# Zaggy1024/RaytracerCore

Hardware: AMD Instinct MI355X
Metric: Mrays/sec (primary+secondary) and samples/sec at 1080p, Cornell box (higher is better)
Workload: dtype f32; 1 GPU; bounce.txt camera 0 1920x1080 x 256 spp per GPU per step; traversal=brute, recursion=10, kernel_build=scene-specialised (hiprtc)

## Files before the change

include/rtcore.h:

```cpp
#ifndef RTCORE_H
#define RTCORE_H

#ifndef __HIPCC_RTC__
#include <stdint.h>
#include <stddef.h>
#endif

#ifdef __cplusplus
extern "C" {
#endif

#define RTCORE_ABI_VERSION 6

typedef enum rt_status {
    RT_OK = 0,
    RT_ERR_ARG = -1,
    RT_ERR_HIP = -2,
    RT_ERR_OOM = -3,
    RT_ERR_NCCL = -4,
    RT_ERR_PARSE = -5,
    RT_ERR_NODEVICE = -6,
    RT_ERR_STATE = -7
} rt_status;

typedef struct rt_vec4d { double x, y, z, w; } rt_vec4d;

typedef struct rt_color { double r, g, b; } rt_color;

typedef enum rt_prim_kind {
    RT_PRIM_TRIANGLE = 0,
    RT_PRIM_SPHERE = 1,
    RT_PRIM_PLANE = 2
} rt_prim_kind;

typedef enum rt_prim_flags {
    RT_FLAG_MIRROR = 1,
    RT_FLAG_TWOSIDED = 2,
    RT_FLAG_INVERT = 4,
    RT_FLAG_HASNORMALS = 8,
    RT_FLAG_TRANSFORMED = 16
} rt_prim_flags;

typedef struct rt_prim {
    int32_t kind;
    int32_t flags;
    rt_vec4d p[3];
    rt_vec4d n[3];
    double radius;
    double to_obj[16];
    double to_world[16];
    double to_normal[16];
    rt_color emission, diffuse, specular, refraction;
    double shininess;
    double refractive_index;
} rt_prim;

typedef enum rt_camera_kind {
    RT_CAMERA_FRUSTUM = 0,
    RT_CAMERA_ORTHO = 1
} rt_camera_kind;

typedef struct rt_camera {
    int32_t kind;
    int32_t reserved;
    rt_vec4d position, look_at, up;
    double fov_y;
    double size_mult;
    double image_plane, dof_amount, focal_length;
} rt_camera;

typedef struct rt_scene_params {
    int32_t width, height;
    int32_t recursion;
    int32_t debug_geom;
    double air_ior;
    rt_color ambient;
} rt_scene_params;

typedef struct rt_scene rt_scene;

typedef enum rt_traversal {
    RT_TRAVERSAL_AUTO = 0,
    RT_TRAVERSAL_BRUTE = 1,
    RT_TRAVERSAL_BVH = 2,
    RT_TRAVERSAL_BVH2 = 3,
    RT_TRAVERSAL_GROUPED = 4
} rt_traversal;

typedef struct rt_scene_info {
    int32_t n_prims;
    int32_t ref_bvh_nodes;
    int32_t ref_bvh_depth;
    int32_t sah_bvh_nodes;
    int32_t sah_bvh_depth;
    int32_t traversal;
    int32_t device;
    int32_t bvh_builder;
    uint64_t device_bytes;
} rt_scene_info;

typedef enum rt_bvh_builder {
    RT_BVH_BUILDER_AUTO = 0,
    RT_BVH_BUILDER_HOST = 1,
    RT_BVH_BUILDER_GPU = 2
} rt_bvh_builder;

#define RT_BUILD_STATS_COUNT 22

int rt_abi_version(void);
const char* rt_build_info(void);
int rt_device_count(void);
int rt_last_error(char* buf, int32_t cap);

int rt_scene_create(const rt_scene_params* params, const rt_prim* prims, int32_t n_prims,
                    int32_t device, rt_scene** out_scene);
int rt_scene_set_camera(rt_scene* scene, const rt_camera* camera);
int rt_scene_set_traversal(rt_scene* scene, int32_t traversal);
int rt_scene_get_info(const rt_scene* scene, rt_scene_info* info);
void rt_scene_destroy(rt_scene* scene);
int rt_set_bvh_builder(int32_t builder);
int rt_scene_get_build_stats(const rt_scene* scene, double* out, int32_t n);
int rt_set_jit(int32_t on);
int rt_scene_get_jit_error(const rt_scene* scene, char* buf, int32_t cap);
int rt_debug_jit_compile(const char* arch, int32_t grouped, char* log, int32_t cap);
int rt_debug_jit_header(const rt_scene_params* params, const rt_prim* prims, int32_t n_prims, const rt_camera* camera,
                        int32_t grouped, char* buf, int64_t cap);
int rt_scene_check_bvh(rt_scene* scene);
#define RT_LAYOUT_COUNT 10
int rt_debug_brute_layout(const rt_prim* prims, int32_t n_prims, int32_t* out, int32_t n_out);
int rt_debug_item_order(int32_t w, int32_t h, int32_t spp, int32_t chunks, int32_t pool, int32_t band,
                        int32_t band_stride, int32_t band_offset, uint32_t* out, int64_t cap_words, int32_t* info);
int rt_debug_pixels_plan(int32_t kernel, int64_t n, int32_t spp, int32_t* info);
int rt_debug_scene_bound(const rt_prim* prims, int32_t n_prims, float* lo, float* hi, float* info);
int rt_debug_block_cull(const rt_prim* prims, int32_t n_prims, const rt_camera* camera, int32_t width, int32_t height,
                        int32_t x0, int32_t y0, int32_t w, int32_t h, int32_t band, int32_t band_stride,
                        int32_t band_offset, uint8_t* dead, int64_t cap, int32_t* info);
int rt_debug_start_rows(int32_t kernel, const rt_camera* camera, int32_t w, int32_t h, int32_t spp, int32_t chunks,
                        int32_t grid_blocks, int32_t flags, int64_t* info);
int rt_debug_ray_log(rt_scene* scene, void* d_log, uint32_t cap, void* d_count);
int rt_debug_vn_rehit(const double* v0, const double* e01, const double* e02, int32_t mirror, double u, double v,
                      const float* dir, int32_t* inside, double* t, double* origin);
int rt_debug_trace_rays(rt_scene* scene, const void* d_rays, uint32_t n, void* d_hits, int32_t waves_per_simd,
                        void* d_stats, void* stream, float* ms);

int rt_render_tile(rt_scene* scene, int32_t x0, int32_t y0, int32_t w, int32_t h, int32_t spp,
                   uint64_t seed, uint64_t sample_base, rt_color* sum_rgb, uint32_t* samples,
                   uint32_t* misses, uint64_t* rays_out);

int rt_render_tile_1spp(rt_scene* scene, int32_t x0, int32_t y0, int32_t w, int32_t h,
                        uint64_t seed, uint64_t sample_index, rt_color* out);

int rt_primary_ids(rt_scene* scene, int32_t x0, int32_t y0, int32_t w, int32_t h, int32_t* ids_out);

int rt_bvh_counts(rt_scene* scene, int32_t x0, int32_t y0, int32_t w, int32_t h, int32_t* counts_out);

typedef enum rt_bounce_type {
    RT_BOUNCE_SKIPPED = 0,
    RT_BOUNCE_DIFFUSE = 1,
    RT_BOUNCE_SPECULAR = 2,
    RT_BOUNCE_SPECULAR_FAIL = 3,
    RT_BOUNCE_TRANSMITTED = 4,
    RT_BOUNCE_EMISSION = 5,
    RT_BOUNCE_PURE_BLACK = 6,
    RT_BOUNCE_RECURSION_COMPLETE = 7,
    RT_BOUNCE_MISSED = 8,
    RT_BOUNCE_DEBUG = 9
} rt_bounce_type;

typedef struct rt_debug_ray {
    int32_t prim_id;
    int32_t type;
    int32_t inside;
    float distance;
    float fresnel;
    float cos_in;
    int32_t bounce;
    int32_t reserved0;
    float position[3];
    float normal[3];
    float origin[3];
    float direction[3];
    float tint[3];
    int32_t reserved1;
} rt_debug_ray;

#define RT_TRACE_MAX_RECORDS (1 << 20)

int rt_trace_paths(rt_scene* scene, int32_t x0, int32_t y0, int32_t w, int32_t h, int32_t spp,
                   uint64_t seed, uint64_t sample_base, rt_debug_ray* rays_out, int32_t* n_rays_out,
                   rt_color* colors_out);

typedef struct rt_ray { rt_vec4d origin, direction; } rt_ray;

typedef struct rt_hit { int32_t prim_id, inside; double distance; float position[3], normal[3]; int32_t reserved[2]; } rt_hit;

typedef enum rt_query_mode {
    RT_QUERY_FAST = 0,
    RT_QUERY_EXACT = 1
} rt_query_mode;

int rt_query_rays(rt_scene* scene, int32_t mode, const rt_ray* rays, int64_t n, rt_hit* hits_out);
int rt_query_rays_device(rt_scene* scene, int32_t mode, const rt_ray* d_rays, int64_t n, rt_hit* d_hits, void* stream);
int rt_camera_rays(const rt_camera* camera, int32_t width, int32_t height, int32_t x0, int32_t y0, int32_t w,
                   int32_t h, rt_ray* out);

int rt_occluded_rays(rt_scene* scene, int32_t mode, const rt_ray* rays, const double* t_max, int64_t n,
                     uint8_t* occluded_out);
int rt_occluded_rays_device(rt_scene* scene, int32_t mode, const rt_ray* d_rays, const double* d_t_max, int64_t n,
                            uint8_t* d_occluded, void* stream);

typedef enum rt_select_kind { RT_SELECT_PRIM = 0, RT_SELECT_NODE = 1 } rt_select_kind;
typedef struct rt_select_item { int32_t kind, index; } rt_select_item;
typedef struct rt_selection { int32_t item, reserved; double distance; } rt_selection;
#define RT_SELECT_MAX_TESTS (1ull << 32)

int rt_select_pixels(rt_scene* scene, const rt_select_item* items, int32_t n_items, int32_t x0, int32_t y0, int32_t w,
                     int32_t h, rt_selection* out);
int rt_select_pixels_device(rt_scene* scene, const rt_select_item* items, int32_t n_items, int32_t x0, int32_t y0,
                            int32_t w, int32_t h, rt_selection* d_out, void* stream);
int rt_select_rays(rt_scene* scene, const rt_select_item* items, int32_t n_items, const rt_ray* rays, int64_t n,
                   rt_selection* out);
int rt_select_rays_device(rt_scene* scene, const rt_select_item* items, int32_t n_items, const rt_ray* d_rays, int64_t n,
                          rt_selection* d_out, void* stream);
int rt_debug_select_rays(const rt_prim* prims, int32_t n_prims, const rt_select_item* items, int32_t n_items,
                         const rt_ray* rays, int64_t n, rt_selection* out);

int rt_render_device(rt_scene* scene, int32_t x0, int32_t y0, int32_t w, int32_t h, int32_t spp,
                     uint64_t seed, uint64_t sample_base, double* d_sum, uint32_t* d_samples,
                     uint32_t* d_misses, unsigned long long* d_rays, void* stream);

int rt_render_rays(rt_scene* scene, const rt_ray* rays, int64_t n, int32_t spp, uint64_t seed, uint64_t sample_base,
                   uint64_t stream_base, rt_color* sum_rgb, uint32_t* samples, uint32_t* misses, uint64_t* rays_out);
int rt_render_rays_device(rt_scene* scene, const rt_ray* d_rays, int64_t n, int32_t spp, uint64_t seed,
                          uint64_t sample_base, uint64_t stream_base, double* d_sum, uint32_t* d_samples,
                          uint32_t* d_misses, unsigned long long* d_rays_count, void* stream);

typedef struct rt_beam {
    rt_vec4d origin, direction;
    rt_vec4d origin_du, origin_dv;
    rt_vec4d direction_du, direction_dv;
} rt_beam;
int rt_render_beams(rt_scene* scene, const rt_beam* beams, int64_t n, int32_t spp, uint64_t seed, uint64_t sample_base,
                    uint64_t stream_base, rt_color* sum_rgb, uint32_t* samples, uint32_t* misses, uint64_t* rays_out);
int rt_render_beams_device(rt_scene* scene, const rt_beam* d_beams, int64_t n, int32_t spp, uint64_t seed,
                           uint64_t sample_base, uint64_t stream_base, double* d_sum, uint32_t* d_samples,
                           uint32_t* d_misses, unsigned long long* d_rays_count, void* stream);
int rt_debug_beam_rays(const rt_beam* beams, int64_t n, int32_t spp, uint64_t seed, uint64_t sample_base,
                       uint64_t stream_base, rt_ray* rays_out, double* uv_out);
int rt_camera_beams(const rt_camera* camera, int32_t width, int32_t height, int32_t x0, int32_t y0, int32_t w,
                    int32_t h, rt_beam* out);

int rt_render_pixels(rt_scene* scene, const uint32_t* pixels, int64_t n, int32_t spp, uint64_t seed, uint64_t sample_base,
                     rt_color* sum_rgb, uint32_t* samples, uint32_t* misses, double* q, uint32_t* batches,
                     uint64_t* rays_out);
int rt_render_pixels_device(rt_scene* scene, const uint32_t* d_pixels, int64_t n, int32_t spp, uint64_t seed,
                            uint64_t sample_base, double* d_sum, uint32_t* d_samples, uint32_t* d_misses, double* d_q,
                            uint32_t* d_batches, uint64_t plane, unsigned long long* d_rays, void* stream);

typedef struct rt_adaptive_params {
    double   rel_tol;
    double   lum_floor;
    uint32_t min_samples;
    uint32_t max_samples;
    uint32_t reserved[2];
} rt_adaptive_params;
int rt_adaptive_select_device(const rt_adaptive_params* params, const double* d_sum, const uint32_t* d_samples,
                              const uint32_t* d_misses, const double* d_q, const uint32_t* d_batches, uint64_t plane,
                              int32_t width, int32_t height, uint32_t* d_pixels, uint32_t cap, uint32_t* d_count,
                              void* stream);
int64_t rt_debug_adaptive_select(const rt_adaptive_params* params, const double* sum, const uint32_t* samples,
                                 const uint32_t* misses, const double* q, const uint32_t* batches, uint64_t plane,
                                 int32_t width, int32_t height, uint32_t* pixels, uint32_t cap);

int rt_primary_hits_device(rt_scene* scene, int32_t x0, int32_t y0, int32_t w, int32_t h, rt_hit* d_hits, void* stream);

#define RT_DENOISE_SAME_PRIM 1u
typedef struct rt_denoise_params {
    float    sigma_l;
    float    sigma_z;
    float    lum_eps;
    int32_t  normal_pow_log2;
    int32_t  iterations;
    uint32_t flags;
    uint32_t reserved[2];
} rt_denoise_params;
int rt_denoise_device(const rt_denoise_params* params, const double* d_sum, const uint32_t* d_samples,
                      const uint32_t* d_misses, const double* d_q, const uint32_t* d_batches, uint64_t plane,
                      const rt_hit* d_hits, int32_t width, int32_t height, double* d_out_sum, float* d_out_var,
                      void* stream);
// ... 87 lines not shown
```

raytracercore_amd/__init__.py:

```python
from __future__ import annotations

import ctypes as C
import enum
import os
from dataclasses import dataclass
from typing import List, Optional, Sequence, Tuple

import numpy as np

_HERE = os.path.dirname(os.path.abspath(__file__))
LIB_PATH = os.path.join(_HERE, "librtcore_hip.so")
REPO_ROOT = os.path.dirname(_HERE)

RT_OK = 0
ABI_VERSION = 6
RT_PRIM_TRIANGLE, RT_PRIM_SPHERE, RT_PRIM_PLANE = 0, 1, 2
RT_FLAG_MIRROR, RT_FLAG_TWOSIDED, RT_FLAG_INVERT, RT_FLAG_HASNORMALS, RT_FLAG_TRANSFORMED = 1, 2, 4, 8, 16
RT_CAMERA_FRUSTUM, RT_CAMERA_ORTHO = 0, 1
RT_TRAVERSAL_AUTO, RT_TRAVERSAL_BRUTE, RT_TRAVERSAL_BVH, RT_TRAVERSAL_BVH2, RT_TRAVERSAL_GROUPED = 0, 1, 2, 3, 4
RT_BVH_BUILDER_AUTO, RT_BVH_BUILDER_HOST, RT_BVH_BUILDER_GPU = 0, 1, 2
(RT_BOUNCE_SKIPPED, RT_BOUNCE_DIFFUSE, RT_BOUNCE_SPECULAR, RT_BOUNCE_SPECULAR_FAIL, RT_BOUNCE_TRANSMITTED,
 RT_BOUNCE_EMISSION, RT_BOUNCE_PURE_BLACK, RT_BOUNCE_RECURSION_COMPLETE, RT_BOUNCE_MISSED, RT_BOUNCE_DEBUG) = range(10)
BOUNCE_TYPE_NAMES = ("Skipped", "Diffuse", "Specular", "SpecularFail", "Transmitted", "Emission", "PureBlack",
                     "RecursionComplete", "Missed", "Debug")
# ... 110 lines not shown
    _fields_ = [("kind", C.c_int32), ("index", C.c_int32)]


class rt_selection(C.Structure):
    _fields_ = [("item", C.c_int32), ("reserved", C.c_int32), ("distance", C.c_double)]


class rt_adaptive_params(C.Structure):
    _fields_ = [("rel_tol", C.c_double), ("lum_floor", C.c_double), ("min_samples", C.c_uint32),
                ("max_samples", C.c_uint32), ("reserved", C.c_uint32 * 2)]


RT_DENOISE_SAME_PRIM = 1


class rt_denoise_params(C.Structure):
    _fields_ = [("sigma_l", C.c_float), ("sigma_z", C.c_float), ("lum_eps", C.c_float), ("normal_pow_log2", C.c_int32),
                ("iterations", C.c_int32), ("flags", C.c_uint32), ("reserved", C.c_uint32 * 2)]


DENOISE_DEFAULTS = dict(sigma_l=1.5, sigma_z=0.05, lum_eps=1e-4, normal_pow_log2=6, iterations=5, flags=0)


def denoise_iterations(width: int, height: int) -> int:
    return max(1, min(5, int(min(width, height)).bit_length() - 6))


def denoise_params(**kw) -> rt_denoise_params:
    v = dict(DENOISE_DEFAULTS)
    unknown = set(kw) - set(v)
    if unknown:
        raise TypeError(f"unknown denoise parameter(s): {sorted(unknown)}")
    v.update(kw)
    return rt_denoise_params(float(v["sigma_l"]), float(v["sigma_z"]), float(v["lum_eps"]), int(v["normal_pow_log2"]),
                             int(v["iterations"]), int(v["flags"]))


RT_REPROJECT_SAME_PRIM = 1


class rt_reproject_params(C.Structure):
    _fields_ = [("sigma_z", C.c_float), ("normal_cos_min", C.c_float), ("max_history", C.c_uint32), ("flags", C.c_uint32),
                ("reserved", C.c_uint32 * 4)]


REPROJECT_DEFAULTS = dict(sigma_z=0.05, normal_cos_min=0.9, max_history=32, flags=RT_REPROJECT_SAME_PRIM)


def reproject_params(**kw) -> rt_reproject_params:
    v = dict(REPROJECT_DEFAULTS)
    unknown = set(kw) - set(v)
    if unknown:
        raise TypeError(f"unknown reproject parameter(s): {sorted(unknown)}")
    v.update(kw)
    return rt_reproject_params(float(v["sigma_z"]), float(v["normal_cos_min"]), int(v["max_history"]), int(v["flags"]))


SELECT_ITEM_DTYPE = np.dtype([("kind", np.int32), ("index", np.int32)])
SELECTION_DTYPE = np.dtype([("item", np.int32), ("reserved", np.int32), ("distance", np.float64)])

RAY_DTYPE = np.dtype([("origin", np.float64, (4,)), ("direction", np.float64, (4,))])
BEAM_DTYPE = np.dtype([(f, np.float64, (4,)) for f in
                       ("origin", "direction", "origin_du", "origin_dv", "direction_du", "direction_dv")])
HIT_DTYPE = np.dtype([
    ("prim_id", np.int32), ("inside", np.int32), ("distance", np.float64),
    ("position", np.float32, (3,)), ("normal", np.float32, (3,)), ("reserved", np.int32, (2,)),
])

_OPTIONAL = ("rt_query_rays", "rt_query_rays_device", "rt_camera_rays", "rt_select_pixels", "rt_select_pixels_device",
             "rt_select_rays", "rt_select_rays_device", "rt_render_rays", "rt_render_rays_device",
             "rt_occluded_rays", "rt_occluded_rays_device", "rt_render_pixels", "rt_render_pixels_device",
             "rt_adaptive_select_device", "rt_primary_hits_device", "rt_denoise_device", "rt_reproject_device",
             "rt_render_beams", "rt_render_beams_device", "rt_camera_beams")

_lib: Optional[C.CDLL] = None


def load_library(path: str = "") -> C.CDLL:
    global _lib
    if _lib is not None:
        return _lib
    path = path or os.environ.get("RTCORE_LIB", "") or LIB_PATH
    if not os.path.exists(path):
        raise RtError(f"{path} is missing: run __graft_entry__.build() (make -C raytracercore_amd/csrc)")
    try:
        import torch
    except ImportError:
        pass
    lib = C.CDLL(path)
    P = C.POINTER
    sig = {
        "rt_abi_version": (C.c_int, []),
        "rt_build_info": (C.c_char_p, []),
        "rt_device_count": (C.c_int, []),
        "rt_last_error": (C.c_int, [C.c_char_p, C.c_int32]),
        "rt_scene_create": (C.c_int, [P(rt_scene_params), P(rt_prim), C.c_int32, C.c_int32, P(C.c_void_p)]),
        "rt_scene_set_camera": (C.c_int, [C.c_void_p, P(rt_camera)]),
        "rt_scene_set_traversal": (C.c_int, [C.c_void_p, C.c_int32]),
        "rt_scene_get_info": (C.c_int, [C.c_void_p, P(rt_scene_info)]),
        "rt_scene_destroy": (None, [C.c_void_p]),
        "rt_set_bvh_builder": (C.c_int, [C.c_int32]),
        "rt_scene_get_build_stats": (C.c_int, [C.c_void_p, P(C.c_double), C.c_int32]),
        "rt_scene_check_bvh": (C.c_int, [C.c_void_p]),
        "rt_set_jit": (C.c_int, [C.c_int32]),
        "rt_scene_get_jit_error": (C.c_int, [C.c_void_p, C.c_char_p, C.c_int32]),
        "rt_debug_jit_compile": (C.c_int, [C.c_char_p, C.c_int32, C.c_char_p, C.c_int32]),
        "rt_debug_jit_header": (C.c_int, [P(rt_scene_params), P(rt_prim), C.c_int32, P(rt_camera), C.c_int32,
                                          C.c_char_p, C.c_int64]),
        "rt_render_tile": (C.c_int, [C.c_void_p] + [C.c_int32] * 5 + [C.c_uint64, C.c_uint64,
                                     P(rt_color), P(C.c_uint32), P(C.c_uint32), P(C.c_uint64)]),
        "rt_render_tile_1spp": (C.c_int, [C.c_void_p] + [C.c_int32] * 4 + [C.c_uint64, C.c_uint64, P(rt_color)]),
        "rt_trace_paths": (C.c_int, [C.c_void_p] + [C.c_int32] * 5 + [C.c_uint64, C.c_uint64, P(rt_debug_ray),
                                     P(C.c_int32), P(rt_color)]),
        "rt_primary_ids": (C.c_int, [C.c_void_p] + [C.c_int32] * 4 + [P(C.c_int32)]),
        "rt_bvh_counts": (C.c_int, [C.c_void_p] + [C.c_int32] * 4 + [P(C.c_int32)]),
        "rt_render_device": (C.c_int, [C.c_void_p] + [C.c_int32] * 5 + [C.c_uint64, C.c_uint64] +
                             [C.c_void_p] * 4 + [C.c_void_p]),
        "rt_primary_ids_device": (C.c_int, [C.c_void_p] + [C.c_int32] * 4 + [C.c_void_p, C.c_void_p]),
        "rt_last_kernel_ms": (C.c_int, [C.c_void_p, P(C.c_float)]),
        "rt_kernel_times": (C.c_int, [C.c_void_p, C.c_int32, P(C.c_float)]),
        "rt_scene_set_stats": (C.c_int, [C.c_void_p, C.c_int32]),
        "rt_scene_get_stats": (C.c_int, [C.c_void_p, P(C.c_uint64), C.c_int32]),
        "rt_render_frame_multi": (C.c_int, [P(rt_scene_params), P(rt_prim), C.c_int32, P(rt_camera), C.c_int32,
                                            C.c_int32, C.c_uint64, C.c_uint64, P(rt_color), P(C.c_uint32),
                                            P(C.c_uint32), P(C.c_uint64)]),
        "rt_render_bands": (C.c_int, [C.c_void_p] + [C.c_int32] * 4 + [C.c_uint64, C.c_uint64, P(rt_color),
                                      P(C.c_uint32), P(C.c_uint32), P(C.c_uint64)]),
        "rt_render_bands_device": (C.c_int, [C.c_void_p] + [C.c_int32] * 4 + [C.c_uint64, C.c_uint64] +
                                   [C.c_void_p] * 3 + [C.c_uint64, C.c_void_p, C.c_void_p]),
        "rt_band_rows": (C.c_int, [C.c_int32] * 4),
        "rt_band_slot_rows": (C.c_int, [C.c_int32] * 3),
        "rt_scatter_band_slot": (C.c_int, [C.c_void_p, C.c_uint64] + [C.c_int32] * 5 + [P(rt_color), P(C.c_uint32),
                                                                                       P(C.c_uint32)]),
        "rt_frame_create": (C.c_int, [P(rt_scene_params), P(rt_prim), C.c_int32, P(rt_camera), C.c_int32,
                                      P(C.c_void_p)]),
        "rt_frame_set_camera": (C.c_int, [C.c_void_p, P(rt_camera)]),
        "rt_frame_render": (C.c_int, [C.c_void_p, C.c_int32, C.c_uint64, C.c_uint64, P(rt_color), P(C.c_uint32),
                                      P(C.c_uint32), P(C.c_uint64)]),
        "rt_frame_submit": (C.c_int, [C.c_void_p, C.c_int32, C.c_uint64, C.c_uint64]),
        "rt_frame_collect": (C.c_int, [C.c_void_p, P(rt_color), P(C.c_uint32), P(C.c_uint32), P(C.c_uint64)]),
        "rt_frame_inject_fault": (C.c_int, [C.c_void_p, C.c_int32]),
        "rt_frame_destroy": (None, [C.c_void_p]),
        "rt_parse_scene": (C.c_int, [C.c_char_p, P(rt_scene_params), P(rt_prim), P(C.c_int32), P(rt_camera),
                                     P(C.c_int32)]),
        "rt_sample_output": (C.c_int32, [rt_color, C.c_uint32, C.c_uint32, rt_color, C.c_double, C.c_double]),
        "rt_tonemap_device": (C.c_int, [C.c_void_p, C.c_void_p, C.c_void_p, C.c_int32, C.c_int32, rt_color, C.c_double,
                                        C.c_double, C.c_void_p, C.c_void_p]),
        "rt_ref_bvh_export": (C.c_int, [P(rt_prim), C.c_int32, P(C.c_int32), P(C.c_double), P(C.c_int32),
                                        P(C.c_int32)]),
        "rt_debug_item_order": (C.c_int, [C.c_int32] * 8 + [P(C.c_uint32), C.c_int64, P(C.c_int32)]),
        "rt_debug_scene_bound": (C.c_int, [P(rt_prim), C.c_int32, P(C.c_float), P(C.c_float), P(C.c_float)]),
        "rt_debug_block_cull": (C.c_int, [P(rt_prim), C.c_int32, P(rt_camera)] + [C.c_int32] * 9 +
                                [P(C.c_uint8), C.c_int64, P(C.c_int32)]),
        "rt_debug_start_rows": (C.c_int, [C.c_int32, P(rt_camera)] + [C.c_int32] * 6 + [P(C.c_int64)]),
        "rt_debug_ray_log": (C.c_int, [C.c_void_p, C.c_void_p, C.c_uint32, C.c_void_p]),
        "rt_debug_vn_rehit": (C.c_int, [P(C.c_double), P(C.c_double), P(C.c_double), C.c_int32, C.c_double,
                                        C.c_double, P(C.c_float), P(C.c_int32), P(C.c_double), P(C.c_double)]),
        "rt_debug_trace_rays": (C.c_int, [C.c_void_p, C.c_void_p, C.c_uint32, C.c_void_p, C.c_int32, C.c_void_p,
                                          C.c_void_p, P(C.c_float)]),
        "rt_query_rays": (C.c_int, [C.c_void_p, C.c_int32, C.c_void_p, C.c_int64, C.c_void_p]),
        "rt_query_rays_device": (C.c_int, [C.c_void_p, C.c_int32, C.c_void_p, C.c_int64, C.c_void_p, C.c_void_p]),
        "rt_camera_rays": (C.c_int, [P(rt_camera)] + [C.c_int32] * 6 + [C.c_void_p]),
        "rt_select_pixels": (C.c_int, [C.c_void_p, C.c_void_p] + [C.c_int32] * 5 + [C.c_void_p]),
        "rt_select_pixels_device": (C.c_int, [C.c_void_p, C.c_void_p] + [C.c_int32] * 5 + [C.c_void_p, C.c_void_p]),
        "rt_select_rays": (C.c_int, [C.c_void_p, C.c_void_p, C.c_int32, C.c_void_p, C.c_int64, C.c_void_p]),
        "rt_select_rays_device": (C.c_int, [C.c_void_p, C.c_void_p, C.c_int32, C.c_void_p, C.c_int64, C.c_void_p,
                                            C.c_void_p]),
        "rt_debug_select_rays": (C.c_int, [P(rt_prim), C.c_int32, C.c_void_p, C.c_int32, C.c_void_p, C.c_int64,
                                           C.c_void_p]),
        "rt_render_rays": (C.c_int, [C.c_void_p, C.c_void_p, C.c_int64, C.c_int32, C.c_uint64, C.c_uint64, C.c_uint64,
                                     P(rt_color), P(C.c_uint32), P(C.c_uint32), P(C.c_uint64)]),
        "rt_render_rays_device": (C.c_int, [C.c_void_p, C.c_void_p, C.c_int64, C.c_int32, C.c_uint64, C.c_uint64,
                                            C.c_uint64] + [C.c_void_p] * 4 + [C.c_void_p]),
        "rt_render_beams": (C.c_int, [C.c_void_p, C.c_void_p, C.c_int64, C.c_int32, C.c_uint64, C.c_uint64, C.c_uint64,
                                      P(rt_color), P(C.c_uint32), P(C.c_uint32), P(C.c_uint64)]),
        "rt_render_beams_device": (C.c_int, [C.c_void_p, C.c_void_p, C.c_int64, C.c_int32, C.c_uint64, C.c_uint64,
                                             C.c_uint64] + [C.c_void_p] * 4 + [C.c_void_p]),
        "rt_debug_beam_rays": (C.c_int, [C.c_void_p, C.c_int64, C.c_int32, C.c_uint64, C.c_uint64, C.c_uint64,
                                         C.c_void_p, C.c_void_p]),
        "rt_camera_beams": (C.c_int, [P(rt_camera)] + [C.c_int32] * 6 + [C.c_void_p]),
        "rt_occluded_rays": (C.c_int, [C.c_void_p, C.c_int32, C.c_void_p, C.c_void_p, C.c_int64, C.c_void_p]),
        "rt_occluded_rays_device": (C.c_int, [C.c_void_p, C.c_int32, C.c_void_p, C.c_void_p, C.c_int64, C.c_void_p,
                                              C.c_void_p]),
        "rt_render_pixels": (C.c_int, [C.c_void_p, C.c_void_p, C.c_int64, C.c_int32, C.c_uint64, C.c_uint64,
                                       P(rt_color), P(C.c_uint32), P(C.c_uint32), P(C.c_double), P(C.c_uint32),
                                       P(C.c_uint64)]),
        "rt_render_pixels_device": (C.c_int, [C.c_void_p, C.c_void_p, C.c_int64, C.c_int32, C.c_uint64, C.c_uint64] +
                                    [C.c_void_p] * 5 + [C.c_uint64, C.c_void_p, C.c_void_p]),
        "rt_adaptive_select_device": (C.c_int, [P(rt_adaptive_params)] + [C.c_void_p] * 5 + [C.c_uint64, C.c_int32,
                                                C.c_int32, C.c_void_p, C.c_uint32, C.c_void_p, C.c_void_p]),
        "rt_debug_adaptive_select": (C.c_int64, [P(rt_adaptive_params)] + [C.c_void_p] * 5 + [C.c_uint64, C.c_int32,
                                                 C.c_int32, C.c_void_p, C.c_uint32]),
        "rt_debug_pixels_plan": (C.c_int, [C.c_int32, C.c_int64, C.c_int32, P(C.c_int32)]),
        "rt_primary_hits_device": (C.c_int, [C.c_void_p] + [C.c_int32] * 4 + [C.c_void_p, C.c_void_p]),
        "rt_denoise_device": (C.c_int, [P(rt_denoise_params)] + [C.c_void_p] * 5 + [C.c_uint64, C.c_void_p, C.c_int32,
                                        C.c_int32, C.c_void_p, C.c_void_p, C.c_void_p]),
        "rt_debug_denoise": (C.c_int, [P(rt_denoise_params)] + [C.c_void_p] * 5 + [C.c_uint64, C.c_void_p, C.c_int32,
                                       C.c_int32, C.c_void_p, C.c_void_p]),
        "rt_reproject_device": (C.c_int, [P(rt_reproject_params), P(rt_camera)] + [C.c_void_p] * 7 +
                                [C.c_uint64, C.c_int32, C.c_int32] + [C.c_void_p] * 7),
        "rt_debug_reproject": (C.c_int, [P(rt_reproject_params), P(rt_camera)] + [C.c_void_p] * 7 +
                               [C.c_uint64, C.c_int32, C.c_int32] + [C.c_void_p] * 6),
    }
    for name, (res, args) in sig.items():
        if (name.startswith("rt_debug_") or name in _OPTIONAL) and not hasattr(lib, name):
            continue
        fn = getattr(lib, name)
        fn.restype = res
        fn.argtypes = args
    if lib.rt_abi_version() != ABI_VERSION:
        raise RtError(f"{path}: ABI version {lib.rt_abi_version()}, this module binds {ABI_VERSION} (rebuild)")
    _lib = lib
    return lib


def _check(rc: int) -> None:
    if rc != RT_OK:
        buf = C.create_string_buffer(1024)
        _lib.rt_last_error(buf, 1024)
        raise RtError(f"rtcore error {rc}: {buf.value.decode(errors='replace')}")


@dataclass
class ParsedScene:
    params: rt_scene_params
    prims: "C.Array[rt_prim]"
    cameras: "C.Array[rt_camera]"

    @property
    def n_prims(self) -> int:
        return len(self.prims)


class SceneLoader:

    @staticmethod
    def from_text(text: str) -> ParsedScene:
        lib = load_library()
        n_p, n_c = C.c_int32(0), C.c_int32(0)
        params = rt_scene_params()
        _check(lib.rt_parse_scene(text.encode(), C.byref(params), None, C.byref(n_p), None, C.byref(n_c)))
        prims = (rt_prim * max(1, n_p.value))()
        cams = (rt_camera * max(1, n_c.value))()
        _check(lib.rt_parse_scene(text.encode(), C.byref(params), prims, C.byref(n_p), cams, C.byref(n_c)))
        return ParsedScene(params, (rt_prim * n_p.value).from_buffer(prims), (rt_camera * n_c.value).from_buffer(cams))

    @staticmethod
    def from_file(path: str) -> ParsedScene:
        with open(path, "r", encoding="utf-8") as f:
            return SceneLoader.from_text(f.read())


LAYOUT_NAMES = ("rects", "boxes", "frames", "frame_boxes", "frame_rects", "tris", "spheres", "planes",
                "groups", "grouped_slots")


def jit_header(scene: "SceneLoader", camera: int = 0, size: Optional[Tuple[int, int]] = None,
               grouped: bool = False) -> str:
    lib = load_library()
    params = rt_scene_params.from_buffer_copy(scene.params)
    if size:
        params.width, params.height = size
    n = len(scene.prims)
    arr = (rt_prim * max(1, n))(*scene.prims)
    cam = rt_camera.from_buffer_copy(scene.cameras[camera])
    k = lib.rt_debug_jit_header(C.byref(params), arr, n, C.byref(cam), 1 if grouped else 0, None, 0)
    if k < 0:
        _check(k)
    buf = C.create_string_buffer(k + 1)
    k2 = lib.rt_debug_jit_header(C.byref(params), arr, n, C.byref(cam), 1 if grouped else 0, buf, k + 1)
    if k2 < 0:
        _check(k2)
    return buf.value.decode()


def brute_layout(prims: Sequence[rt_prim]) -> dict:
    lib = load_library()
    n = len(prims)
    arr = (rt_prim * max(1, n))(*prims)
    out = (C.c_int32 * len(LAYOUT_NAMES))()
    _check(lib.rt_debug_brute_layout(arr, n, out, len(LAYOUT_NAMES)))
    return dict(zip(LAYOUT_NAMES, (int(v) for v in out)))


def item_order(w: int, h: int, spp: int, chunks: int = 0, pool: int = 0,
               bands: Optional[Tuple[int, int, int]] = None) -> Tuple[np.ndarray, dict]:
    lib = load_library()
    b = bands or (0, 0, 0)
    info = (C.c_int32 * 4)()
    n = lib.rt_debug_item_order(w, h, spp, chunks, pool, b[0], b[1], b[2], None, 0, info)
    if n < 0:
        _check(n)
    out = np.zeros((max(1, n), 3), np.uint32)
    n2 = lib.rt_debug_item_order(w, h, spp, chunks, pool, b[0], b[1], b[2],
                                 out.ctypes.data_as(C.POINTER(C.c_uint32)), 3 * n, info)
    if n2 < 0:
        _check(n2)
    return out[:n], dict(zip(("n_chunks", "chunk", "pool", "n_split"), (int(v) for v in info)))


def scene_bound(prims: Sequence[rt_prim]) -> dict:
    lib = load_library()
    n = len(prims)
    arr = (rt_prim * max(1, n))(*prims)
    lo, hi, info = (C.c_float * 3)(), (C.c_float * 3)(), (C.c_float * 2)()
    state = lib.rt_debug_scene_bound(arr, n, lo, hi, info)
    if state < 0:
        _check(state)
    return {"lo": np.array(lo, np.float32), "hi": np.array(hi, np.float32), "limit": np.float32(info[0]),
            "pad": np.float32(info[1]), "state": int(state)}


def block_cull(prims: Sequence[rt_prim], camera: rt_camera, size: Tuple[int, int],
               window: Optional[Tuple[int, int, int, int]] = None,
               bands: Optional[Tuple[int, int, int]] = None) -> Tuple[np.ndarray, int]:
    lib = load_library()
    n = len(prims)
    arr = (rt_prim * max(1, n))(*prims)
    cam = rt_camera.from_buffer_copy(camera)
    b = bands or (0, 0, 0)
    W, H = size
    rows = lib.rt_band_rows(H, b[0], b[1], b[2]) if bands else H
    x0, y0, w, h = window or (0, 0, W, rows)
    bx, by = (w + 7) // 8, (h + 7) // 8
    dead = np.zeros(max(1, bx * by), np.uint8)
    info = (C.c_int32 * 2)()
    live = lib.rt_debug_block_cull(arr, n, C.byref(cam), W, H, x0, y0, w, h, b[0], b[1], b[2],
                                   dead.ctypes.data_as(C.POINTER(C.c_uint8)), bx * by, info)
    if live < 0:
        _check(live)
    return dead[:bx * by].reshape(by, bx).astype(bool), int(live)


def start_rows(kernel: int, camera: rt_camera, w: int, h: int, spp: int, chunks: int = 0, grid_blocks: int = 1792,
               instrumented: bool = False, vertex_normals: bool = False) -> dict:
    lib = load_library()
    cam = rt_camera.from_buffer_copy(camera)
    info = (C.c_int64 * 3)()
    on = lib.rt_debug_start_rows(kernel, C.byref(cam), w, h, spp, chunks, grid_blocks,
                                 int(bool(instrumented)) | int(bool(vertex_normals)) << 1, info)
    if on < 0:
        _check(on)
    return {"on": bool(on), "rows": int(info[0]), "bytes": int(info[1]), "chunk": int(info[2])}


def ref_bvh_export(prims: Sequence[rt_prim]) -> Tuple[np.ndarray, np.ndarray, int, int]:
    lib = load_library()
    n = len(prims)
    arr = (rt_prim * max(1, n))(*prims)
    order = np.zeros(max(1, n), np.int32)
    boxes = np.zeros((max(1, 2 * n), 8), np.float64)
    nodes, depth = C.c_int32(0), C.c_int32(0)
    _check(lib.rt_ref_bvh_export(arr, n, order.ctypes.data_as(C.POINTER(C.c_int32)),
                                 boxes.ctypes.data_as(C.POINTER(C.c_double)), C.byref(nodes), C.byref(depth)))
    return order[:n], boxes[:nodes.value], nodes.value, depth.value


def sample_output(sum_rgb: Tuple[float, float, float], samples: int, misses: int,
                  background=(0.0, 0.0, 0.0), background_alpha: float = 0.0, exposure: float = 1.0) -> int:
    lib = load_library()
    return lib.rt_sample_output(rt_color(*sum_rgb), samples, misses, rt_color(*background), background_alpha, exposure)


def device_count() -> int:
    return load_library().rt_device_count()


def camera_rays(camera: rt_camera, size: Tuple[int, int], x0: int = 0, y0: int = 0, w: Optional[int] = None,
                h: Optional[int] = None) -> np.ndarray:
    lib = load_library()
    if not hasattr(lib, "rt_camera_rays"):
        raise RtError("this build of the library has no rt_camera_rays")
    W, H = int(size[0]), int(size[1])
    w = W - x0 if w is None else w
    h = H - y0 if h is None else h
    out = np.zeros((max(w, 0), max(h, 0)), RAY_DTYPE)
    cam = rt_camera.from_buffer_copy(camera)
    _check(lib.rt_camera_rays(C.byref(cam), W, H, x0, y0, w, h, out.ctypes.data_as(C.c_void_p)))
    return out


def _pack_rays(origins, directions) -> np.ndarray:
    o = np.asarray(origins, np.float64)
    d = np.asarray(directions, np.float64)
    if o.ndim != 2 or d.ndim != 2 or o.shape[0] != d.shape[0] or o.shape[1] not in (3, 4) or d.shape[1] not in (3, 4):
        raise ValueError("origins and directions must be (n, 3) or (n, 4) arrays of the same n")
    rays = np.zeros(o.shape[0], RAY_DTYPE)
    rays["origin"][:, 3] = 1.0
    rays["origin"][:, :o.shape[1]] = o
    rays["direction"][:, :d.shape[1]] = d
    return rays


def _pack_beams(origins, directions, origin_du, origin_dv, direction_du, direction_dv) -> np.ndarray:
    rest = (directions, origin_du, origin_dv, direction_du, direction_dv)
    if all(a is None for a in rest):
        return np.ascontiguousarray(origins, BEAM_DTYPE).reshape(-1)
    if any(a is None for a in rest):
        raise ValueError("beams: six arrays, or one BEAM_DTYPE array and None for the other five")
    parts = [np.asarray(a, np.float64) for a in (origins,) + rest]
    n = parts[0].shape[0] if parts[0].ndim == 2 else -1
    if any(a.ndim != 2 or a.shape[0] != n or a.shape[1] not in (3, 4) for a in parts):
        raise ValueError("origins, directions and the four footprint arrays must be (n, 3) or (n, 4) arrays of the same n")
    beams = np.zeros(n, BEAM_DTYPE)
    beams["origin"][:, 3] = 1.0
    for name, a in zip(BEAM_DTYPE.names, parts):
        beams[name][:, :a.shape[1]] = a
    return beams


def beam_rays_host(origins, directions, origin_du, origin_dv, direction_du, direction_dv, spp: int, seed: int,
                   sample_base: int = 0, stream_base: int = 0) -> Tuple[np.ndarray, np.ndarray]:
    lib = load_library()
    if not hasattr(lib, "rt_debug_beam_rays"):
        raise RtError("this build of the library has no rt_debug_beam_rays")
    beams = _pack_beams(origins, directions, origin_du, origin_dv, direction_du, direction_dv)
    n = beams.shape[0]
    rays = np.zeros((n, max(spp, 0)), RAY_DTYPE)
    uv = np.zeros((n, max(spp, 0), 2), np.float64)
    _check(lib.rt_debug_beam_rays(beams.ctypes.data_as(C.c_void_p), n, spp, seed, sample_base, stream_base,
                                  rays.ctypes.data_as(C.c_void_p), uv.ctypes.data_as(C.c_void_p)))
    return rays, uv


def camera_beams(camera: rt_camera, size: Tuple[int, int], x0: int = 0, y0: int = 0, w: Optional[int] = None,
                 h: Optional[int] = None) -> np.ndarray:
    lib = load_library()
    if not hasattr(lib, "rt_camera_beams"):
        raise RtError("this build of the library has no rt_camera_beams")
    W, H = int(size[0]), int(size[1])
    w = W - x0 if w is None else w
    h = H - y0 if h is None else h
    out = np.zeros((max(w, 0), max(h, 0)), BEAM_DTYPE)
    cam = rt_camera.from_buffer_copy(camera)
    _check(lib.rt_camera_beams(C.byref(cam), W, H, x0, y0, w, h, out.ctypes.data_as(C.c_void_p)))
    return out


def _pack_items(items) -> np.ndarray:
    if isinstance(items, np.ndarray) and items.dtype == SELECT_ITEM_DTYPE:
        return np.ascontiguousarray(items.reshape(-1))
    a = np.asarray(items, np.int64)
    if a.size == 0:
        return np.zeros(0, SELECT_ITEM_DTYPE)
    if a.ndim != 2 or a.shape[1] != 2:
        raise ValueError("items must be an (n, 2) int array or a sequence of (kind, index) pairs")
    if a.min() < -2 ** 31 or a.max() >= 2 ** 31:
        raise ValueError("items: kind and index must fit in int32")
    out = np.zeros(a.shape[0], SELECT_ITEM_DTYPE)
    out["kind"], out["index"] = a[:, 0], a[:, 1]
    return out


def _rays_arg(origins, directions) -> np.ndarray:
    return np.ascontiguousarray(origins, RAY_DTYPE) if directions is None else _pack_rays(origins, directions)


def segment_rays(points_a, points_b) -> Tuple[np.ndarray, np.ndarray]:
    a = np.asarray(points_a, np.float64)
    b = np.asarray(points_b, np.float64)
    if a.shape != b.shape or a.ndim < 1 or a.shape[-1] != 3:
        raise ValueError("points_a and points_b must be (..., 3) arrays of the same shape")
    v = b - a
    scale = np.max(np.abs(v), axis=-1)
    safe = np.where(scale > 0, scale, 1.0)
    u = v / safe[..., None]
    norm = np.sqrt(np.sum(u * u, axis=-1))
    t_max = np.where(scale > 0, norm * safe, 0.0)
    d = u / np.where(scale > 0, norm, 1.0)[..., None]
    d = d / np.where(scale > 0, np.sqrt(np.sum(d * d, axis=-1)), 1.0)[..., None]
    rays = np.zeros(a.shape[:-1], RAY_DTYPE)
    rays["origin"][..., :3] = a
    rays["origin"][..., 3] = 1.0
    rays["direction"][..., :3] = d
    return rays, t_max


def select_rays_host(prims: Sequence[rt_prim], items, origins, directions=None) -> np.ndarray:
    lib = load_library()
    if not hasattr(lib, "rt_debug_select_rays"):
        raise RtError("this build of the library has no rt_debug_select_rays")
    n = len(prims)
    arr = prims if isinstance(prims, C.Array) and n > 0 else (rt_prim * max(1, n))(*prims)
    it = _pack_items(items)
    rays = _rays_arg(origins, directions)
    out = np.zeros(rays.shape, SELECTION_DTYPE)
# ... 680 lines not shown
```

raytracercore_amd/csrc/api_debug.hip:

```cpp
#include <cstdlib>
#include <cstring>

#include "rt_scene.h"

namespace {

int n_bvh_prims(const std::vector<HostPrim>& H)
{
    int nb = 0;
    for (const HostPrim& p : H) nb += p.kind != RT_PRIM_PLANE;
    return nb;
}

HostRecords report_records(const std::vector<HostPrim>& H)
{
    const bool host_tree = builder_for(n_bvh_prims(H)) == RT_BVH_BUILDER_HOST;
    return make_host_records(H, host_tree ? grouping_max_leaf(GroupingTree::LayoutReport, (int)H.size(), false) : 0,
                             group_max_default());
}

}

extern "C" {

// ... 333 lines not shown
        if (ref >= (int)n4.size()) {
            err = "wide child index out of range";
            return u;
        }
        const Node4Q& q = n4[ref];
        uint32_t ex, ql[3], qh[3];
        int refs[4], nc;
        std::memcpy(&ex, &q.a.w, 4);
        std::memcpy(&ql[0], &q.b.x, 4);
        std::memcpy(&qh[0], &q.b.y, 4);
        std::memcpy(&ql[1], &q.b.z, 4);
        std::memcpy(&qh[1], &q.b.w, 4);
        std::memcpy(&ql[2], &q.c.x, 4);
        std::memcpy(&qh[2], &q.c.y, 4);
        std::memcpy(&refs[0], &q.c.z, 4);
        std::memcpy(&refs[1], &q.c.w, 4);
        std::memcpy(&refs[2], &q.d.x, 4);
        std::memcpy(&refs[3], &q.d.y, 4);
        std::memcpy(&nc, &q.d.z, 4);
        if (nc < 1 || nc > 4) {
            err = "wide node with a bad child count";
            return u;
        }
        max_stack = std::max(max_stack, pushes + nc - 1);
        const double org[3] = {q.a.x, q.a.y, q.a.z};
        for (int k = 0; k < nc; k++) {
            const B sub = walk4(refs[k], pushes + nc - 1);
            B box;
            for (int a = 0; a < 3; a++) {
                const double sc = std::ldexp(1.0, (int)((ex >> (8 * a)) & 255u) - 128);
                box.lo[a] = org[a] + ((ql[a] >> (8 * k)) & 255u) * sc;
                box.hi[a] = org[a] + ((qh[a] >> (8 * k)) & 255u) * sc;
            }
            if (err.empty() && !contains(box, sub)) err = "wide child box misses a primitive below it";
            grow(u, sub);
        }
        return u;
    };
    if (err.empty() && nb > 0) walk4(s->bvh.root4, 0);
    for (int i = 0; i < n && err.empty(); i++)
        if (seen[i] != (outside(i) ? 0 : 1))
            err = "wide tree: primitive " + std::to_string(i) + " referenced " + std::to_string(seen[i]) + " times";
    if (err.empty() && max_stack > s->bvh.stack4) err = "wide tree needs more stack than recorded";
    if (!err.empty()) {
        set_error("rt_scene_check_bvh: " + err);
        return RT_ERR_STATE;
    }
    return RT_OK;
}

int rt_debug_item_order(int32_t w, int32_t h, int32_t spp, int32_t chunks, int32_t pool, int32_t band,
                        int32_t band_stride, int32_t band_offset, uint32_t* out, int64_t cap_words, int32_t* info)
{
    const bool banded = band > 0;
    if (w <= 0 || h <= 0 || spp <= 0 || chunks < 0 || pool < 0 || pool % 64 != 0 || cap_words < 0 ||
        (cap_words > 0 && !out) || (banded && (band_stride <= 0 || band_offset < 0 || band_offset >= band_stride))) {
        set_error("rt_debug_item_order: bad argument");
        return RT_ERR_ARG;
    }
    const int rows = banded ? band_set_rows(h, band, band_stride, band_offset) : h;
    if (rows <= 0) return 0;
    PathParams p = make_params_for(pool > 64 ? 1 : 0, chunks, pool, 0, 0, w, rows, spp, 0, 0, 0.0);
    if (banded) set_band(p, band, band_stride, band_offset);
    if ((uint64_t)p.n_chunks * (uint64_t)p.n_pad > 0xF0000000ull) {
        set_error("rt_debug_item_order: tile x spp too large for one launch");
        return RT_ERR_ARG;
    }
    if (info) {
        info[0] = p.n_chunks;
        info[1] = p.chunk;
        info[2] = p.pool;
        info[3] = p.n_split;
    }
    const int64_t n = list_tickets(p, out, cap_words);
    if (n > INT32_MAX) {
        set_error("rt_debug_item_order: too many tickets");
        return RT_ERR_ARG;
    }
    return (int)n;
}

int rt_debug_pixels_plan(int32_t kernel, int64_t n, int32_t spp, int32_t* info)
{
    if (kernel < 0 || kernel > 3 || kernel == 2 || n <= 0 || n > ((int64_t)1 << 30) || spp <= 0 || !info) {
        set_error("rt_debug_pixels_plan: bad argument");
        return RT_ERR_ARG;
    }
    const PathParams p = make_params_pixels(kernel, n, spp, 0, 0, 1920, 1080);
    info[0] = p.n_chunks;
    info[1] = p.chunk;
    info[2] = (p.spp + p.chunk - 1) / p.chunk;
    info[3] = p.n_pad / 64;
    return RT_OK;
}

int rt_debug_scene_bound(const rt_prim* prims, int32_t n_prims, float* lo, float* hi, float* info)
{
    if (n_prims < 0 || (n_prims > 0 && !prims) || !lo || !hi) {
        set_error("rt_debug_scene_bound: bad argument");
        return RT_ERR_ARG;
    }
    for (int i = 0; i < n_prims; i++)
        if (prims[i].kind < 0 || prims[i].kind > 2) {
            set_error("rt_debug_scene_bound: unknown primitive kind at index " + std::to_string(i));
            return RT_ERR_ARG;
        }
    const SceneBound b = make_scene_bound(prepare_prims(prims, n_prims));
    for (int k = 0; k < 3; k++) {
        lo[k] = b.lo[k];
        hi[k] = b.hi[k];
    }
    if (info) {
        info[0] = b.limit;
        info[1] = b.pad;
    }
    return b.empty ? 1 : (b.limit < 0.0f ? 2 : 0);
}

int rt_debug_block_cull(const rt_prim* prims, int32_t n_prims, const rt_camera* camera, int32_t width, int32_t height,
                        int32_t x0, int32_t y0, int32_t w, int32_t h, int32_t band, int32_t band_stride,
                        int32_t band_offset, uint8_t* dead, int64_t cap, int32_t* info)
{
    const bool banded = band > 0;
    if (n_prims < 0 || (n_prims > 0 && !prims) || !camera || width <= 0 || height <= 0 || w <= 0 || h <= 0 || x0 < 0 ||
        y0 < 0 || x0 + w > width || cap < 0 || (cap > 0 && !dead) || band < 0 ||
        (camera->kind != RT_CAMERA_FRUSTUM && camera->kind != RT_CAMERA_ORTHO) ||
        (banded && (band_stride <= 0 || band_offset < 0 || band_offset >= band_stride)) || (!banded && y0 + h > height)) {
        set_error("rt_debug_block_cull: bad argument");
        return RT_ERR_ARG;
    }
    int n_planes = 0;
    for (int i = 0; i < n_prims; i++) {
        if (prims[i].kind < 0 || prims[i].kind > 2) {
            set_error("rt_debug_block_cull: unknown primitive kind at index " + std::to_string(i));
            return RT_ERR_ARG;
        }
        n_planes += prims[i].kind == RT_PRIM_PLANE ? 1 : 0;
    }
    const SceneBound b = make_scene_bound(prepare_prims(prims, n_prims));
    CameraD camd;
    CameraF camf;
    camera_init(*camera, width, height, camd, camf);
    const CullWindow win{x0, y0, w, h, banded ? band : 0, banded ? band_stride : 0, banded ? band_offset : 0};
    std::vector<unsigned char> flags;
    const int live = cull_blocks(camf, b, n_planes, win, flags);
    for (size_t i = 0; i < flags.size() && (int64_t)i < cap; i++) dead[i] = flags[i];
    if (info) {
        info[0] = (w + 7) / 8;
        info[1] = (h + 7) / 8;
    }
    return live;
}

int rt_debug_start_rows(int32_t kernel, const rt_camera* camera, int32_t w, int32_t h, int32_t spp, int32_t chunks,
                        int32_t grid_blocks, int32_t flags, int64_t* info)
{
    if (kernel < 0 || kernel > 3 || !camera || w <= 0 || h <= 0 || spp <= 0 || chunks < 0 || grid_blocks <= 0 || !info ||
        (camera->kind != RT_CAMERA_FRUSTUM && camera->kind != RT_CAMERA_ORTHO)) {
        set_error("rt_debug_start_rows: bad argument");
        return RT_ERR_ARG;
    }
    CameraD camd;
    CameraF camf;
    camera_init(*camera, w, h, camd, camf);
    const PathParams p = make_params_for(kernel, chunks, 0, 0, 0, w, h, spp, 0, 0, 0.0);
    const StartRowsPlan sr = plan_start_rows(kernel, (flags & 1) != 0, (flags & 2) != 0, camf.kind, camf.dof != 0.0f, p.chunk, grid_blocks);
    info[0] = sr.rows;
    info[1] = (int64_t)sr.bytes;
    info[2] = p.chunk;
    return sr.on ? 1 : 0;
}

int rt_parse_scene(const char* text, rt_scene_params* params, rt_prim* prims, int32_t* n_prims, rt_camera* cameras,
                   int32_t* n_cameras)
{
    if (!text || !n_prims || !n_cameras) {
        set_error("rt_parse_scene: bad argument");
        return RT_ERR_ARG;
    }
    ParsedScene ps;
    std::string err;
    if (!parse_scene_text(text, ps, err)) {
        set_error(err);
        return RT_ERR_PARSE;
    }
    const int cap_p = *n_prims, cap_c = *n_cameras;
    *n_prims = (int32_t)ps.prims.size();
    *n_cameras = (int32_t)ps.cameras.size();
    if (params) *params = ps.params;
    if (prims) {
        if (cap_p < (int)ps.prims.size()) {
            set_error("rt_parse_scene: primitive array too small");
            return RT_ERR_ARG;
        }
        std::copy(ps.prims.begin(), ps.prims.end(), prims);
    }
    if (cameras) {
        if (cap_c < (int)ps.cameras.size()) {
            set_error("rt_parse_scene: camera array too small");
            return RT_ERR_ARG;
        }
        std::copy(ps.cameras.begin(), ps.cameras.end(), cameras);
    }
    return RT_OK;
}

int rt_ref_bvh_export(const rt_prim* prims, int32_t n, int32_t* leaf_order, double* boxes, int32_t* n_nodes,
                      int32_t* depth)
{
    if (n < 0 || (n > 0 && !prims)) {
        set_error("rt_ref_bvh_export: bad argument");
        return RT_ERR_ARG;
    }
    std::vector<HostPrim> host = prepare_prims(prims, n);
    RefBvh ref = build_ref_bvh(host);
    int k = 0;
    for (size_t i = 0; i < ref.nodes.size(); i++) {
        const RefNode& r = ref.nodes[i];
        if (r.prim >= 0 && leaf_order) leaf_order[k++] = r.prim;
        if (boxes) {
            double* b = boxes + 8 * i;
            b[0] = r.mn.x; b[1] = r.mn.y; b[2] = r.mn.z; b[3] = r.mn.w;
            b[4] = r.mx.x; b[5] = r.mx.y; b[6] = r.mx.z; b[7] = r.mx.w;
        }
    }
    if (n_nodes) *n_nodes = (int32_t)ref.nodes.size();
    if (depth) *depth = ref.depth;
    return RT_OK;
}

}
```

raytracercore_amd/csrc/block_cull.cpp:

```cpp
#include "block_cull.h"

#include <algorithm>
#include <cmath>

namespace rtc {

namespace {

constexpr double kMargin = 0.25;
constexpr double kAhead = 1e-3;

struct P2 {
    double x, y;
};

struct Hull {
    std::vector<P2> v;
    double xmin, xmax, ymin, ymax;
};

double cross2(P2 o, P2 a, P2 b) { return (a.x - o.x) * (b.y - o.y) - (a.y - o.y) * (b.x - o.x); }

void convex_hull(std::vector<P2> pts, Hull& h)
{
    std::sort(pts.begin(), pts.end(), [](P2 a, P2 b) { return a.x < b.x || (a.x == b.x && a.y < b.y); });
    std::vector<P2> v(2 * pts.size());
    size_t k = 0;
    for (size_t i = 0; i < pts.size(); i++) {
        while (k >= 2 && cross2(v[k - 2], v[k - 1], pts[i]) <= 0.0) k--;
        v[k++] = pts[i];
    }
    for (size_t i = pts.size() - 1, t = k + 1; i > 0; i--) {
        while (k >= t && cross2(v[k - 2], v[k - 1], pts[i - 1]) <= 0.0) k--;
        v[k++] = pts[i - 1];
    }
    v.resize(k > 1 ? k - 1 : k);
    h.v = v;
    h.xmin = h.ymin = INFINITY;
    h.xmax = h.ymax = -INFINITY;
    for (P2 p : pts) {
        h.xmin = std::min(h.xmin, p.x);
        h.xmax = std::max(h.xmax, p.x);
        h.ymin = std::min(h.ymin, p.y);
        h.ymax = std::max(h.ymax, p.y);
    }
}

bool separated(const Hull& h, double xa, double xb, double ya, double yb)
{
    if (xb < h.xmin || xa > h.xmax || yb < h.ymin || ya > h.ymax) return true;
    const size_t n = h.v.size();
    if (n < 3) return false;
    for (size_t i = 0; i < n; i++) {
        const P2 p = h.v[i], q = h.v[i + 1 == n ? 0 : i + 1];
        const double nx = q.y - p.y, ny = -(q.x - p.x);
        const double cx = nx > 0.0 ? xa : xb, cy = ny > 0.0 ? ya : yb;
        if (nx * (cx - p.x) + ny * (cy - p.y) > 0.0) return true;
    }
    return false;
}

struct V3d {
    double x, y, z;
};
V3d crs(V3d a, V3d b) { return {a.y * b.z - a.z * b.y, a.z * b.x - a.x * b.z, a.x * b.y - a.y * b.x}; }
double dot(V3d a, V3d b) { return a.x * b.x + a.y * b.y + a.z * b.z; }
V3d v3d(const float4& f) { return {(double)f.x, (double)f.y, (double)f.z}; }

bool project_bound(const CameraF& c, const SceneBound& b, int frame_w, Hull& hull)
{
    const bool frustum = c.kind == RT_CAMERA_FRUSTUM;
    const double vals[] = {c.position.x, c.position.y, c.position.z, c.look.x, c.look.y, c.look.z, c.side.x,
                           c.side.y, c.side.z, c.up.x, c.up.y, c.up.z, c.w2, c.h2, c.tan_x, c.tan_y,
                           c.h_mult, c.v_mult, c.image_plane, c.dof, c.focal_length, c.tan_x_per_px, c.tan_y_per_px};
    for (double v : vals)
        if (!std::isfinite(v)) return false;
    if (c.dof != 0.0f) return false;
    const V3d pos = v3d(c.position), look = v3d(c.look), side = v3d(c.side), up = v3d(c.up);
    const double apos = std::fabs(pos.x) + std::fabs(pos.y) + std::fabs(pos.z);
    const V3d da = crs(up, look), db = crs(look, side), dc = crs(side, up);
    const double det = dot(side, da);
    if (!(std::fabs(det) > 0.5 && std::fabs(det) < 2.0)) return false;
    const double sxa = frustum ? c.tan_x_per_px : c.h_mult, sya = frustum ? c.tan_y_per_px : c.v_mult;
    if (sxa == 0.0 || sya == 0.0) return false;
    const double scale = std::min(std::fabs(sxa), std::fabs(sya));
    if (frustum) {
        if (!(apos <= (double)b.limit)) return false;
    } else {
        const double reach = std::fabs((double)c.w2 * c.h_mult) * (std::fabs(side.x) + std::fabs(side.y) + std::fabs(side.z)) +
                             std::fabs((double)c.h2 * c.v_mult) * (std::fabs(up.x) + std::fabs(up.y) + std::fabs(up.z));
        if (!(apos + 2.0 * reach + std::fabs((double)c.image_plane) <= (double)b.limit)) return false;
    }
    std::vector<P2> pts;
    double c_min = INFINITY, c_max = 0.0;
    for (int k = 0; k < 8; k++) {
        const V3d P = {(k & 1) ? (double)b.hi[0] + b.pad : (double)b.lo[0] - b.pad,
                       (k & 2) ? (double)b.hi[1] + b.pad : (double)b.lo[1] - b.pad,
                       (k & 4) ? (double)b.hi[2] + b.pad : (double)b.lo[2] - b.pad};
        const V3d v = {P.x - pos.x, P.y - pos.y, P.z - pos.z};
        const double a = dot(v, da) / det, bb = dot(v, db) / det, cc = dot(v, dc) / det;
        if (!(cc > kAhead * std::sqrt(dot(v, v))) || !(cc > 0.0)) return false;
        c_min = std::min(c_min, cc);
        c_max = std::max(c_max, cc);
        if (frustum) pts.push_back({(a / cc + (double)c.tan_x) / sxa, (bb / cc + (double)c.tan_y) / sya});
        else pts.push_back({a / sxa + (double)c.w2, bb / sya + (double)c.h2});
    }
    double err;
    if (frustum) {
        const double L = 1.0 + std::fabs((double)c.tan_x) + std::fabs((double)c.tan_y);
        err = std::ldexp(L * L, -20) / scale +
              std::ldexp(apos + std::fabs((double)c.image_plane), -22) / (c_min * scale);
    } else {
        const double R = apos + std::fabs((double)c.w2 * c.h_mult) + std::fabs((double)c.h2 * c.v_mult) +
                         std::fabs((double)c.image_plane);
        err = std::ldexp(R + c_max, -22) / scale + std::ldexp((double)std::max(frame_w, 1), -22);
    }
    if (!(err <= kMargin / 8.0)) return false;
    for (P2 p : pts)
        if (!(std::isfinite(p.x) && std::isfinite(p.y))) return false;
    convex_hull(pts, hull);
    return true;
}

}

int cull_blocks(const CameraF& cam, const SceneBound& bound, int n_planes, const CullWindow& win,
                std::vector<unsigned char>& dead)
{
    const int bxn = (win.w + 7) / 8, byn = (win.h + 7) / 8;
    const int n = bxn * byn;
    dead.assign((size_t)n, 0);
    if (n_planes > 0) return n;
    if (bound.empty) {
        dead.assign((size_t)n, 1);
        return 0;
    }
    if (!(bound.limit >= 0.0f)) return n;
    Hull hull;
    if (!project_bound(cam, bound, (int)(2.0f * cam.w2), hull)) return n;
    int live = 0;
    for (int by = 0; by < byn; by++) {
        int run_a[8], run_b[8], runs = 0;
        for (int py = by * 8; py < std::min(win.h, by * 8 + 8); py++) {
            int fy = win.y0 + py;
            if (win.band > 0) fy = win.y0 + ((py / win.band) * win.band_stride + win.band_offset) * win.band + py % win.band;
            if (runs > 0 && fy == run_b[runs - 1] + 1) run_b[runs - 1] = fy;
            else {
                run_a[runs] = run_b[runs] = fy;
                runs++;
            }
        }
        for (int bx = 0; bx < bxn; bx++) {
            const double xa = (double)(win.x0 + bx * 8) - kMargin;
            const double xb = (double)(win.x0 + std::min(win.w, bx * 8 + 8)) + kMargin;
            bool is_dead = true;
            for (int r = 0; r < runs && is_dead; r++)
                is_dead = separated(hull, xa, xb, (double)run_a[r] - kMargin, (double)(run_b[r] + 1) + kMargin);
            dead[(size_t)by * bxn + bx] = is_dead ? 1 : 0;
            live += is_dead ? 0 : 1;
        }
    }
    return live;
}

uint64_t dead_pixels(const CullWindow& win, const std::vector<unsigned char>& dead)
{
    const int bxn = (win.w + 7) / 8, byn = (win.h + 7) / 8;
    uint64_t n = 0;
    for (int by = 0; by < byn; by++)
        for (int bx = 0; bx < bxn; bx++)
            if (dead[(size_t)by * bxn + bx])
                n += (uint64_t)(std::min(win.w, bx * 8 + 8) - bx * 8) * (uint64_t)(std::min(win.h, by * 8 + 8) - by * 8);
    return n;
}

}
```

raytracercore_amd/csrc/block_cull.h:

```cpp
#pragma once
#include <cstdint>
#include <vector>

#include "rt_internal.h"

namespace rtc {

struct CullWindow {
    int x0, y0, w, h;
    int band, band_stride, band_offset;
};

int cull_blocks(const CameraF& cam, const SceneBound& bound, int n_planes, const CullWindow& win,
                std::vector<unsigned char>& dead);

uint64_t dead_pixels(const CullWindow& win, const std::vector<unsigned char>& dead);

}
```

raytracercore_amd/csrc/kernels_path.hip:

```cpp
#include "../../include/rtcore_rng.h"
#include "rt_kernels.h"
#include "rt_beam.h"
#ifdef RT_SCENE_CONST
#include "rt_scene_const.h"
#endif

namespace rtc {
namespace {

struct V3 {
    float x, y, z;
};
__device__ __forceinline__ V3 v3(float x, float y, float z) { return V3{x, y, z}; }
__device__ __forceinline__ V3 xyz(float4 a) { return V3{a.x, a.y, a.z}; }
__device__ __forceinline__ V3 operator+(V3 a, V3 b) { return {a.x + b.x, a.y + b.y, a.z + b.z}; }
__device__ __forceinline__ V3 operator-(V3 a, V3 b) { return {a.x - b.x, a.y - b.y, a.z - b.z}; }
__device__ __forceinline__ V3 operator*(V3 a, float s) { return {a.x * s, a.y * s, a.z * s}; }
__device__ __forceinline__ V3 operator*(V3 a, V3 b) { return {a.x * b.x, a.y * b.y, a.z * b.z}; }
__device__ __forceinline__ V3 operator-(V3 a) { return {-a.x, -a.y, -a.z}; }
__device__ __forceinline__ float dot(V3 a, V3 b) { return fmaf(a.x, b.x, fmaf(a.y, b.y, a.z * b.z)); }
__device__ __forceinline__ bool known_zero(float c)
{
#if defined(RT_SCENE_CONST)
    return __builtin_constant_p(c) && c == 0.0f;
// ... 191 lines not shown

template <bool SUB>
__device__ __forceinline__ void hit_box(const BoxRec& B, V3 o, V3 d, V3 id, V3 oi, int prev, Best& b)
{
    const float lx = SUB ? (B.lo.x - oi.x) * id.x : fmaf(B.lo.x, id.x, -oi.x);
    const float hx = SUB ? (B.hi.x - oi.x) * id.x : fmaf(B.hi.x, id.x, -oi.x);
    const float ly = SUB ? (B.lo.y - oi.y) * id.y : fmaf(B.lo.y, id.y, -oi.y);
    const float hy = SUB ? (B.hi.y - oi.y) * id.y : fmaf(B.hi.y, id.y, -oi.y);
    const float lz = SUB ? (B.lo.z - oi.z) * id.z : fmaf(B.lo.z, id.z, -oi.z);
    const float hz = SUB ? (B.hi.z - oi.z) * id.z : fmaf(B.hi.z, id.z, -oi.z);
    const float nx = vmin(lx, hx), ny = vmin(ly, hy), nz = vmin(lz, hz);
    const float fx = vmax(lx, hx), fy = vmax(ly, hy), fz = vmax(lz, hz);
    const float te = vmax3(nx, ny, nz), tx = vmin3(fx, fy, fz);
    const bool meet = te <= tx;
    if (RT_BOX_WAVE_SKIP && !__any(meet & (tx >= 0.0f))) return;
    const int sx = (int)(__float_as_uint(d.x) >> 31), sy = (int)(__float_as_uint(d.y) >> 31),
              sz = (int)(__float_as_uint(d.z) >> 31);
    const uint32_t keep = B.keep;
    const uint32_t rel_prev = (uint32_t)(prev - (B.sg0 >> 1));
    bool ok_e = false, ok_x = false;
    int fe = 0, fo = 0;
    if (keep & 0x3Fu) {
        fe = te == nx ? sx : (te == ny ? 2 + sy : 4 + sz);
        ok_e = meet & (__float_as_uint(te) < __float_as_uint(b.t)) & ((uint32_t)fe != rel_prev) &
               (((keep >> fe) & 1u) != 0);
    }
    if (keep & 0x3F00u) {
        fo = tx == fx ? 1 - sx : (tx == fy ? 3 - sy : 5 - sz);
        ok_x = meet & (__float_as_uint(tx) < __float_as_uint(b.t)) & ((uint32_t)fo != rel_prev) &
               (((keep >> (8 + fo)) & 1u) != 0);
    }
    const bool ok = ok_e | ok_x;
    b.t = ok ? (ok_e ? te : tx) : b.t;
    b.sg = ok ? B.sg0 + 2 * (ok_e ? fe : fo) : b.sg;
}

__device__ __forceinline__ float slab_rcp(float d)
{
    return rcp(fabsf(d) >= 5.421010862e-20f ? d : __builtin_copysignf(5.421010862e-20f, d));
}
__device__ __forceinline__ float slab_rcp_lean(float d)
{
    return __builtin_amdgcn_fmed3f(rcp(d), -0x1p64f, 0x1p64f);
}

template <bool BARE = false>
__device__ __forceinline__ bool slab(float4 lo, float4 hi, V3 oi, V3 id, float tmax, float& tnear)
{
    const float tx0 = fmaf(lo.x, id.x, -oi.x), tx1 = fmaf(hi.x, id.x, -oi.x);
    const float ty0 = fmaf(lo.y, id.y, -oi.y), ty1 = fmaf(hi.y, id.y, -oi.y);
    const float tz0 = fmaf(lo.z, id.z, -oi.z), tz1 = fmaf(hi.z, id.z, -oi.z);
    const float nx = BARE ? vmin(tx0, tx1) : fminf(tx0, tx1), fx = BARE ? vmax(tx0, tx1) : fmaxf(tx0, tx1);
    const float ny = BARE ? vmin(ty0, ty1) : fminf(ty0, ty1), fy = BARE ? vmax(ty0, ty1) : fmaxf(ty0, ty1);
    const float nz = BARE ? vmin(tz0, tz1) : fminf(tz0, tz1), fz = BARE ? vmax(tz0, tz1) : fmaxf(tz0, tz1);
    const float tmin = BARE ? vmax3(nx, ny, vmax0(nz)) : fmaxf(fmaxf(nx, ny), fmaxf(nz, 0.0f));
    const float tmx = BARE ? vmin3(fx, fy, vmin(fz, tmax)) : fminf(fminf(fx, fy), fminf(fz, tmax));
    tnear = tmin;
    return tmin <= tmx * 1.00000024f;
}

template <class SceneT>
__device__ __forceinline__ bool scene_meets(const SceneT& s, V3 o, V3 d)
{
    const V3 id = v3(slab_rcp_lean(d.x), slab_rcp_lean(d.y), slab_rcp_lean(d.z));
    const V3 oi = o * id;
    const float tx0 = fmaf(s.bound_lo[0], id.x, -oi.x), tx1 = fmaf(s.bound_hi[0], id.x, -oi.x);
    const float ty0 = fmaf(s.bound_lo[1], id.y, -oi.y), ty1 = fmaf(s.bound_hi[1], id.y, -oi.y);
    const float tz0 = fmaf(s.bound_lo[2], id.z, -oi.z), tz1 = fmaf(s.bound_hi[2], id.z, -oi.z);
    const float tmin = fmaxf(fmaxf(fminf(tx0, tx1), fminf(ty0, ty1)), fmaxf(fminf(tz0, tz1), 0.0f));
    const float tmx = fminf(fminf(fmaxf(tx0, tx1), fmaxf(ty0, ty1)), fmaxf(tz0, tz1));
    const bool near = fabsf(o.x) + fabsf(o.y) + fabsf(o.z) <= s.bound_limit;
    const bool finite = fabsf(d.x + d.y + d.z) < __builtin_huge_valf();
    return (!(tmin > tmx) | !near | !finite) & (s.bound_empty == 0);
}

template <bool CULL, bool STATS, bool ANY = false, class SceneT, class GroupP, class TestP, class RectP, class FrameP,
          class BoxP, class XfP>
__device__ __forceinline__ void trace_brute(const SceneT& s, GroupP groups, TestP tests, RectP rects, FrameP frames,
                                            BoxP boxes, XfP xf, V3 o, V3 d, int prev, Best& b, unsigned& n_flat,
                                            unsigned& n_sph, unsigned& n_node)
{
    const V3 id = v3(slab_rcp_lean(d.x), slab_rcp_lean(d.y), slab_rcp_lean(d.z));
    const V3 oi = o * id;
    const int n_groups = CULL ? s.n_groups : 1;
    int skip_to = 0;
#ifdef RT_SCENE_CONST
#pragma unroll
#endif
    for (int g = 0; g < n_groups; g++) {
        if (CULL && g < skip_to) continue;
        const GroupRec G = groups[g];
        if (CULL) {
            if (STATS) n_node++;
            float tn;
            if (!__any((!ANY || b.sg < 0) && slab<true>(G.lo, G.hi, oi, id, b.t, tn))) {
                skip_to = g + 1 + G.skip;
                continue;
            }
        }
        if (STATS) {
            n_flat += G.n_rect[0] + G.n_rect[1] + G.n_rect[2] + G.n_flat_extra + (G.n_tri_sph & 0xFFFF);
            n_sph += G.n_tri_sph >> 16;
        }
        RectP r = rects + __float_as_int(G.lo.w);
        rect_group<0>(r, G.n_rect[0], o, d, id, oi, prev, b);
        r += G.n_rect[0];
        rect_group<1>(r, G.n_rect[1], o, d, id, oi, prev, b);
        r += G.n_rect[1];
        rect_group<2>(r, G.n_rect[2], o, d, id, oi, prev, b);
        for (int j = G.frame_first + G.n_frames; j < G.frame_first + G.n_frames + G.n_boxes; j++) {
            const BoxRec B = boxes[j];
            hit_box<false>(B, o, d, id, oi, prev, b);
        }
        if (ANY && !CULL && !__any(b.sg < 0)) return;
        for (int f = G.frame_first; f < G.frame_first + G.n_frames; f++) {
            const FrameRec F = frames[f];
            const V3 lo = v3(dot4(F.r0, o), dot4(F.r1, o), dot4(F.r2, o));
            const V3 ld = v3(dot3(F.r0, d), dot3(F.r1, d), dot3(F.r2, d));
            const V3 lid = v3(rcp(ld.x), rcp(ld.y), rcp(ld.z));
            RectP fr = rects + F.rect_first;
            rect_group<0, true>(fr, F.n_rect[0], lo, ld, lid, lo, prev, b);
            fr += F.n_rect[0];
            rect_group<1, true>(fr, F.n_rect[1], lo, ld, lid, lo, prev, b);
            fr += F.n_rect[1];
            rect_group<2, true>(fr, F.n_rect[2], lo, ld, lid, lo, prev, b);
            if (F.box >= 0) {
                const BoxRec B = boxes[F.box];
                hit_box<true>(B, lo, ld, lid, lo, prev, b);
            }
        }
        if (ANY && !CULL && !__any(b.sg < 0)) return;
        int i = __float_as_int(G.hi.w);
        int end = i + (G.n_tri_sph & 0xFFFF);
        if (i < end) {
            TestRec cur = tests[i];
            for (; i < end; i++) {
                const TestRec nxt = tests[i + 1];
                hit_tri<true>(cur, i, o, d, prev, b);
                cur = nxt;
            }
        }
        if (ANY && !CULL && !__any(b.sg < 0)) return;
        end = i + (G.n_tri_sph >> 16);
        if (i < end) {
            TestRec cur = tests[i];
            for (; i < end; i++) {
                const TestRec nxt = tests[i + 1];
                hit_sph<true, RT_SPH_WAVE_SKIP < 0 ? CULL : RT_SPH_WAVE_SKIP != 0>(cur, i, o, d, prev, xf, b);
                cur = nxt;
            }
        }
        if (ANY && CULL && !__any(b.sg < 0)) return;
    }
}

template <bool SLOT = false, class XfP>
__device__ __forceinline__ void hit_any(const TestRec& R, int slot, V3 o, V3 d, int prev, XfP xf, Best& b)
{
    switch (__float_as_uint(R.meta.y) & KIND_MASK) {
    case RT_PRIM_TRIANGLE: hit_tri<SLOT>(R, slot, o, d, prev, b); break;
    case RT_PRIM_SPHERE: hit_sph<SLOT>(R, slot, o, d, prev, xf, b); break;
    default: hit_plane<SLOT>(R, slot, o, d, prev, b); break;
    }
}

constexpr uint32_t kLeafGeneric = 0xFFFFFFFFu;
__device__ __forceinline__ void leaf_decode(int pend, int& k, int& kend, uint32_t& lfl)
{
    const bool compact = (pend & kLeafCompact) != 0;
    k = compact ? (pend >> 2) & (kLeafCompactMaxFirst - 1) : pend >> 3;
    kend = k + (pend & (compact ? 3 : 7)) + 1;
    lfl = compact ? leaf_flags(((uint32_t)pend >> 25) & 31u) : kLeafGeneric;
}
__device__ __forceinline__ int leaf_advance(int pend, int n)
{
    const bool compact = (pend & kLeafCompact) != 0;
    const int left = pend & (compact ? 3 : 7);
    return left >= n ? pend + (compact ? (n << 2) - n : (n << 3) - n) : -1;
}



__device__ __forceinline__ float ubyte(uint32_t v, int k) { return (float)((v >> (8 * k)) & 255u); }
__device__ __forceinline__ void cswap(float& da, int& ra, float& db, int& rb)
{
    const bool sw = db < da;
    const float t = da;
    const int r = ra;
    da = sw ? db : da;
    ra = sw ? rb : ra;
    db = sw ? t : db;
    rb = sw ? r : rb;
}
#define RT_STACK_OVF 44
typedef __attribute__((address_space(3))) int LdsInt;
typedef __attribute__((address_space(1))) int GlobalInt;
struct TravStack {
    LdsInt* lds;
    GlobalInt* ovf;
};
__device__ __forceinline__ TravStack make_stack(int* lds_base, int* ovf_base)
{
    return TravStack{(LdsInt*)lds_base, (GlobalInt*)ovf_base};
}
__device__ __forceinline__ unsigned ovf_slot(int e)
{
    return (unsigned)e * (gridDim.x * 256u) + blockIdx.x * 256u + threadIdx.x;
}
template <int STACK>
__device__ __forceinline__ void push(const TravStack& st, int& sp, int v)
{
    if (sp < STACK) st.lds[sp * 256 + (int)threadIdx.x] = v;
    else st.ovf[ovf_slot(sp - STACK)] = v;
    sp++;
}
template <int STACK>
__device__ __forceinline__ int pop_ref(const TravStack& st, int& sp)
{
    --sp;
    return sp < STACK ? st.lds[sp * 256 + (int)threadIdx.x] : st.ovf[ovf_slot(sp - STACK)];
}

__device__ __forceinline__ void pin4(float4& f)
{
    typedef float F4 __attribute__((ext_vector_type(4)));
    F4 v = {f.x, f.y, f.z, f.w};
    asm volatile("" : "+v"(v));
    f = make_float4(v.x, v.y, v.z, v.w);
}
__device__ __forceinline__ void pin_rec(TestRec& t)
{
    pin4(t.r0);
    pin4(t.r1);
    pin4(t.r2);
    pin4(t.meta);
}
template <int STACK>
__device__ __forceinline__ void wide_visit(const Node4Q& q, V3 id, V3 oi, float best, int& ref, int& sp,
                                           const TravStack& stk, bool& pop)
{
    const uint32_t ex = __float_as_uint(q.a.w);
    const float ax = __builtin_amdgcn_ldexpf(id.x, (int)(ex & 255u) - 128);
    const float ay = __builtin_amdgcn_ldexpf(id.y, (int)((ex >> 8) & 255u) - 128);
    const float az = __builtin_amdgcn_ldexpf(id.z, (int)((ex >> 16) & 255u) - 128);
    const float bx = fmaf(q.a.x, id.x, -oi.x), by = fmaf(q.a.y, id.y, -oi.y), bz = fmaf(q.a.z, id.z, -oi.z);
    const uint32_t lx = __float_as_uint(q.b.x), hx = __float_as_uint(q.b.y);
    const uint32_t ly = __float_as_uint(q.b.z), hy = __float_as_uint(q.b.w);
    const uint32_t lz = __float_as_uint(q.c.x), hz = __float_as_uint(q.c.y);
    const uint32_t nx = id.x >= 0.0f ? lx : hx, fx = id.x >= 0.0f ? hx : lx;
    const uint32_t ny = id.y >= 0.0f ? ly : hy, fy = id.y >= 0.0f ? hy : ly;
    const uint32_t nz = id.z >= 0.0f ? lz : hz, fz = id.z >= 0.0f ? hz : lz;
    const int nc = __float_as_int(q.d.z);
    float d0, d1, d2, d3;
    int r0 = __float_as_int(q.c.z), r1 = __float_as_int(q.c.w), r2 = __float_as_int(q.d.x), r3 = __float_as_int(q.d.y);
    const float tmax_best = best * 1.00000024f;
#define RT_WIDE_CHILD(K, D)                                                                                       \
    {                                                                                                             \
        const float tmin = fmaxf(fmaxf(fmaxf(fmaf(ubyte(nx, K), ax, bx), fmaf(ubyte(ny, K), ay, by)),              \
                                       fmaf(ubyte(nz, K), az, bz)), 0.0f);                                         \
        const float tmax = fminf(fminf(fmaf(ubyte(fx, K), ax, bx), fmaf(ubyte(fy, K), ay, by)),                   \
                                 fmaf(ubyte(fz, K), az, bz));                                                      \
        D = ((K < nc) & (tmin <= fminf(tmax * 1.00000024f, tmax_best))) ? tmin : __builtin_huge_valf();         \
    }
    RT_WIDE_CHILD(0, d0)
    RT_WIDE_CHILD(1, d1)
    RT_WIDE_CHILD(2, d2)
    RT_WIDE_CHILD(3, d3)
#undef RT_WIDE_CHILD
    cswap(d0, r0, d1, r1);
    cswap(d2, r2, d3, r3);
    cswap(d0, r0, d2, r2);
    cswap(d1, r1, d3, r3);
    cswap(d1, r1, d2, r2);
    const float inf = __builtin_huge_valf();
    if (d0 < inf) {
        if (d3 < inf) push<STACK>(stk, sp, r3);
        if (d2 < inf) push<STACK>(stk, sp, r2);
        if (d1 < inf) push<STACK>(stk, sp, r1);
        ref = r0;
        pop = false;
    }
}

template <int STACK>
__device__ __forceinline__ void any_visit(const Node4Q& q, V3 id, V3 oi, float best, int& ref, int& sp,
                                          const TravStack& stk, bool& pop)
{
    const uint32_t ex = __float_as_uint(q.a.w);
    const float ax = __builtin_amdgcn_ldexpf(id.x, (int)(ex & 255u) - 128);
    const float ay = __builtin_amdgcn_ldexpf(id.y, (int)((ex >> 8) & 255u) - 128);
    const float az = __builtin_amdgcn_ldexpf(id.z, (int)((ex >> 16) & 255u) - 128);
    const float bx = fmaf(q.a.x, id.x, -oi.x), by = fmaf(q.a.y, id.y, -oi.y), bz = fmaf(q.a.z, id.z, -oi.z);
    const uint32_t lx = __float_as_uint(q.b.x), hx = __float_as_uint(q.b.y);
    const uint32_t ly = __float_as_uint(q.b.z), hy = __float_as_uint(q.b.w);
    const uint32_t lz = __float_as_uint(q.c.x), hz = __float_as_uint(q.c.y);
    const bool px = id.x >= 0.0f, py = id.y >= 0.0f, pz = id.z >= 0.0f;
    const uint32_t nx = px ? lx : hx, fx = px ? hx : lx;
    const uint32_t ny = py ? ly : hy, fy = py ? hy : ly;
    const uint32_t nz = pz ? lz : hz, fz = pz ? hz : lz;
    const int nc = __float_as_int(q.d.z);
    const int r0 = __float_as_int(q.c.z), r1 = __float_as_int(q.c.w), r2 = __float_as_int(q.d.x), r3 = __float_as_int(q.d.y);
    const float tmax_best = best * 1.00000024f;
    bool h0, h1, h2, h3;
#define RT_ANY_CHILD(K, H)                                                                                        \
    {                                                                                                             \
        const float tmin = fmaxf(fmaxf(fmaxf(fmaf(ubyte(nx, K), ax, bx), fmaf(ubyte(ny, K), ay, by)),              \
// ... 761 lines not shown
            S.rng = rt_rng_from_pixel_key(L.pkey, p.sample_base + (unsigned long long)item_sample<NT>(L, p));
            const float u = (float)rt_rng_next24(&S.rng) * 0x1p-24f;
            const float v = (float)rt_rng_next24(&S.rng) * 0x1p-24f;
            BeamV o, d;
            const BeamSample r = beam_sample(p.beam_list + (size_t)kBeamRows * (size_t)bi, u, v, o, d);
            if (r == BEAM_RAY) {
                S.o = v3(o.x, o.y, o.z);
                S.d = v3(d.x, d.y, d.z);
                S.tint = v3(1.0f, 1.0f, 1.0f);
                S.bounce = 0;
                S.prev = -1;
                L.live = true;
            } else {
                const unsigned left = r == BEAM_INVALID ? L.cnt >> 16 : 1u;
                L.cnt += left * (256u - 65536u);
                if (!NT) L.s_next += (int)left;
            }
        }
        return;
    }
    if (go && L.active && L.item_open && !L.live && L.cnt >= 65536u) {
        if (start_rows_on<NT, SRC, ROWS>(p, cam)) {
            const unsigned r = (L.cnt & 0xFFu) + ((L.cnt >> 8) & 0xFFu);
            const row_g1* const rows = (const row_g1*)(unsigned long long)p.starts;
            const row_f4 v = *(const row_g4*)(rows + start_row_offset(p, r, lane));
            const V3 d = v3(v.x, v.y, v.z);
            S.rng.x = __float_as_uint(v.w);
            S.o = madd(d, cam.image_plane, xyz(cam.position));
            S.d = d;
            S.tint = v3(1.0f, 1.0f, 1.0f);
            S.bounce = 0;
            S.prev = -1;
            L.live = true;
            return;
        }
        int fx = L.fx, fy = L.fy;
        if (NT && SRC == ITEMS_PIXELS) {
            const unsigned pix = p.pixel_list[item_ray(L.item, p)];
            list_pixel(pix, p, fx, fy);
            L.pkey = rt_rng_pixel_key(p.seed_key, (unsigned long long)pix);
        } else if (NT) {
            int px, py, c;
            item_pixel(L.item, p, px, py, c, fx, fy);
            L.pkey = rt_rng_pixel_key(p.seed_key, (unsigned long long)fy * (unsigned long long)p.scene.width +
                                                      (unsigned long long)fx);
        }
        S.rng = rt_rng_from_pixel_key(L.pkey, p.sample_base + (unsigned long long)item_sample<NT>(L, p));
        start_sample<!NT>(cam, fx, fy, S);
        L.live = true;
    }
}

template <bool VN, bool PIN = false, bool SLOT = false, bool REC = false, class SceneT, class VnP, class TestP, class ParT>
__device__ __forceinline__ void bounce(Lane& L, Sample& S, const SceneT& s, const ShadeRecs& R, VnP vnormals, TestP tests,
                                       const PrimD* prims_d, const Best& b, [[maybe_unused]] const ParT& p)
{
    V3 col;
    [[maybe_unused]] BounceRec rec;
    [[maybe_unused]] const V3 ro = S.o, rd = S.d, rtint = S.tint;
    [[maybe_unused]] const int rbounce = S.bounce;
    [[maybe_unused]] unsigned rsample = 0;
    if constexpr (REC) {
        if (p.rec_rays) {
            int px, py, c, fx, fy;
            item_pixel(L.item, p, px, py, c, fx, fy);
            rsample = ((unsigned)py * (unsigned)p.w + (unsigned)px) * (unsigned)p.spp + (unsigned)item_sample<SLOT>(L, p);
        }
    }
    const int r = shade<VN, PIN, SLOT, REC>(s, R.prims, R.mats, R.xfs, vnormals, tests, prims_d, b, S, col, &rec);
    if constexpr (REC) {
        const unsigned slot = rsample * (unsigned)(s.recursion + 1) + (unsigned)rbounce;
        if (p.rec_rays && slot < p.rec_max && rbounce <= s.recursion) {
            float4* q = p.rec_rays + (size_t)kRecRows * slot;
            q[0] = make_float4(__int_as_float(rec.prim_id), __int_as_float(rec.type), __int_as_float(rec.inside), rec.distance);
            q[1] = make_float4(rec.fresnel, rec.cos_in, __int_as_float(rbounce), 0.0f);
            q[2] = make_float4(rec.pos.x, rec.pos.y, rec.pos.z, rec.nrm.x);
            q[3] = make_float4(rec.nrm.y, rec.nrm.z, ro.x, ro.y);
            q[4] = make_float4(ro.z, rd.x, rd.y, rd.z);
            q[5] = make_float4(rtint.x, rtint.y, rtint.z, 0.0f);
            if (r != 0)
                p.rec_samples[rsample] = r == 1 ? make_float4(0.0f + col.x, 0.0f + col.y, 0.0f + col.z, __int_as_float(rbounce + 1))
                                                : make_float4(-1.0f, -1.0f, -1.0f, __int_as_float(rbounce + 1));
        }
    }
    if (r != 0) {
        const bool hit = r == 1;
        L.ar += hit ? col.x : 0.0f;
        L.ag += hit ? col.y : 0.0f;
        L.ab += hit ? col.z : 0.0f;
        L.cnt += hit ? 1u - 65536u : 256u - 65536u;
        if (!SLOT) L.s_next++;
        L.live = false;
        if (!SLOT) {
            asm volatile("" : "=v"(S.o.x), "=v"(S.o.y), "=v"(S.o.z), "=v"(S.d.x), "=v"(S.d.y), "=v"(S.d.z),
                         "=v"(S.tint.x), "=v"(S.tint.y), "=v"(S.tint.z), "=v"(S.bounce), "=v"(S.prev),
                         "=v"(S.rng.x));
        }
    }
}

template <bool STATS, class ParT>
__device__ __forceinline__ void flush_counts(unsigned long long wave_rays, const Counters& cnt, const ParT& p,
                                             int lane)
{
    if (lane == 0) atomicAdd(p.rays, wave_rays);
    if (STATS) {
        unsigned long long a = cnt.nodes, t = cnt.tris, q = cnt.sphs;
        for (int off = 32; off > 0; off >>= 1) {
            a += __shfl_down(a, off);
            t += __shfl_down(t, off);
            q += __shfl_down(q, off);
        }
        if (lane == 0) {
            atomicAdd(p.stats + 0, a);
            atomicAdd(p.stats + 1, t);
            atomicAdd(p.stats + 2, q);
            atomicAdd(p.stats + 3, cnt.cyc_start);
            atomicAdd(p.stats + 4, cnt.cyc_trace);
            atomicAdd(p.stats + 5, cnt.cyc_shade);
            atomicAdd(p.stats + 6, cnt.iters);
        }
        unsigned long long mx = cnt.max_steps, ov = cnt.ovf_pushes, ms = cnt.max_sp, ot = cnt.outer;
        for (int off = 32; off > 0; off >>= 1) {
            mx = max(mx, (unsigned long long)__shfl_down(mx, off));
            ov += __shfl_down(ov, off);
            ms = max(ms, (unsigned long long)__shfl_down(ms, off));
            ot += __shfl_down(ot, off);
        }
        if (lane == 0) {
            atomicMax(p.stats + 7, mx);
            atomicAdd(p.stats + 8, ov);
            atomicMax(p.stats + 9, ms);
            atomicAdd(p.stats + 10, ot);
        }
    }
}

#ifdef __HIP_DEVICE_COMPILE__
#define RT_AS_CONST __attribute__((address_space(4)))
#else
#define RT_AS_CONST
#endif
typedef RT_AS_CONST const CameraF CameraC;
typedef RT_AS_CONST const PathParams ParamsC;

template <bool CULL, bool LDS, bool STATS, bool VN, int SRC = ITEMS_TILE>
__device__ __forceinline__ void path_body(const CameraF* __restrict__ camp, const PathParams* __restrict__ pp)
{
    const ParamsC& P0 = *(const ParamsC*)pp;
    extern __shared__ float4 lds_scene[];
    const ShadeRecs R = stage_scene<LDS>(P0.scene, P0.prims, P0.mats, P0.xf, lds_scene);
    const int lane = threadIdx.x & 63;
    const unsigned total = (unsigned)P0.n_chunks * (unsigned)P0.n_pad;
    Lane L;
    lane_init(L);
    Sample S;
    S.prev = -1;
    S.bounce = 0;
    Counters cnt{};
    unsigned long long wave_rays = 0;
    const unsigned long long bound_off = P0.scene_bound != 0 ? 0ull : ~0ull;

    while (true) {
        unsigned long long t0 = 0, t1 = 0, t2 = 0;
        if (STATS) t0 = __builtin_readcyclecounter();
        const CameraC* cp = (const CameraC*)camp;
        asm volatile("" : "+s"(cp));
        const ParamsC* pq = (const ParamsC*)pp;
        asm volatile("" : "+s"(pq));
#ifdef RT_SCENE_CONST
        const PathScene& sc = *(const PathScene*)kSceneW;
#else
        const auto& sc = pq->scene;
#endif
#if defined(RT_SCENE_CONST) && RT_SCENE_CONST_CAMERA
        refill<false, ITEMS_TILE, !STATS && !VN, !STATS && !VN>(L, S, *pq, sc, *(const CameraF*)kCameraW, lane, total,
                                                         (unsigned)wave_rays);
#else
        refill<false, SRC, !STATS && !VN, !STATS && !VN && SRC == ITEMS_TILE>(L, S, *pq, sc, *cp, lane, total,
                                                                              (unsigned)wave_rays);
#endif
        if (!__any(L.active)) break;
        if (STATS) t1 = __builtin_readcyclecounter();
        wave_rays += (unsigned)__popcll(__ballot(L.live));
        if (L.live) {
#ifdef RT_SCENE_CONST
            const auto tests = (const TestRec*)kTestsW;
            const auto rects = (const RectRec*)kRectsW;
            const auto frames = (const FrameRec*)kFramesW;
            const auto boxes = (const BoxRec*)kFramesW;
            const auto groups = (const GroupRec*)kGroupsW;
            const auto xf = (const XformF*)kXfW;
#else
            const auto tests = (const RT_AS_CONST TestRec*)pq->tests;
            const auto rects = (const RT_AS_CONST RectRec*)pq->rects;
            const auto frames = (const RT_AS_CONST FrameRec*)pq->frames;
            const auto boxes = (const RT_AS_CONST BoxRec*)pq->frames;
            const auto groups = (const RT_AS_CONST GroupRec*)pq->groups;
            const auto xf = (const RT_AS_CONST XformF*)pq->xf;
#endif
            const auto vnormals = (const RT_AS_CONST float4*)pq->vnormals;
            Best b = query_start<VN>(sc, S.prev);
            bool query = true;
            if (!STATS && (!CULL || RT_BOUND_GROUPED) &&
                __builtin_expect((__ballot(L.live && S.bounce != 0) | bound_off) == 0ull, 0))
                query = __any(L.live && scene_meets(sc, S.o, S.d));
            if (query)
                trace_brute<CULL, STATS>(sc, groups, tests, rects, frames, boxes, xf, S.o, S.d, S.prev, b, cnt.tris,
                                         cnt.sphs, cnt.nodes);
            test_planes(sc, tests, S.o, S.d, S.prev, b);
            if (VN && __builtin_isnan(S.d.x + S.d.y + S.d.z)) b = Best{__builtin_huge_valf(), -1};
            if (STATS) t2 = __builtin_readcyclecounter();
            bounce<VN, false, false, STATS>(L, S, sc, R, vnormals, tests, pq->prims_d, b, *pq);
        } else if (STATS) {
            t2 = __builtin_readcyclecounter();
        }
        if (STATS) {
            const unsigned long long t3 = __builtin_readcyclecounter();
            cnt.cyc_start += t1 - t0;
            cnt.cyc_trace += t2 - t1;
            cnt.cyc_shade += t3 - t2;
            cnt.iters++;
        }
    }
    if (!STATS && SRC == ITEMS_TILE && P0.cull != nullptr && blockIdx.x == 0 && threadIdx.x < 64)
        wave_rays += ((unsigned long long)P0.cull[0] | (unsigned long long)P0.cull[1] << 32) * (unsigned long long)P0.spp;
    flush_counts<STATS>(wave_rays, cnt, *(const ParamsC*)pp, lane);
}

template <bool CULL, bool LDS, bool STATS, bool VN, int SRC = ITEMS_TILE>
__global__ void __launch_bounds__(256, CULL ? RT_GROUPED_WAVES : RT_PATH_WAVES)
    path_kernel(PathScene, const CameraF* __restrict__ camp, const PathParams* __restrict__ pp, const TestRec*,
                const RectRec*, const FrameRec*, const PrimF*, const NodeF*, const Node4Q*, const GroupRec*,
                const XformF*, const MatF*, const float4*)
{
    path_body<CULL, LDS, STATS, VN, SRC>(camp, pp);
}

template <bool STATS, class GroupP, class RectP, class BoxP>
__device__ __forceinline__ void test_outer(GroupP groups, RectP rects, BoxP boxes, V3 o, V3 d, int prev, Best& b,
                                           unsigned& n_tests)
{
    const V3 id = v3(slab_rcp_lean(d.x), slab_rcp_lean(d.y), slab_rcp_lean(d.z));
    const V3 oi = o * id;
    const GroupRec G = groups[0];
    if (STATS) n_tests += G.n_rect[0] + G.n_rect[1] + G.n_rect[2] + G.n_flat_extra;
    RectP r = rects + __float_as_int(G.lo.w);
    rect_group<0>(r, G.n_rect[0], o, d, id, oi, prev, b);
    r += G.n_rect[0];
    rect_group<1>(r, G.n_rect[1], o, d, id, oi, prev, b);
    r += G.n_rect[1];
    rect_group<2>(r, G.n_rect[2], o, d, id, oi, prev, b);
    for (int j = G.frame_first + G.n_frames; j < G.frame_first + G.n_frames + G.n_boxes; j++) {
        const BoxRec B = boxes[j];
        hit_box<false>(B, o, d, id, oi, prev, b);
    }
}

template <bool STATS, class TestP, class RowP, class XfP>
__device__ __forceinline__ void test_leaf(TestP tests, RowP rows, XfP xf, int pend, V3 o, V3 d, int prev, Best& b,
                                          unsigned& n_tri, unsigned& n_sph)
{
    int k, kend;
    uint32_t lfl;
    leaf_decode(pend, k, kend, lfl);
    float4 r[RT_SPEC_PRIMS][3];
    uint32_t fl[RT_SPEC_PRIMS];
#pragma unroll
    for (int j = 0; j < RT_SPEC_PRIMS; j++) {
        r[j][0] = rows[3 * (k + j)];
        r[j][1] = rows[3 * (k + j) + 1];
        r[j][2] = rows[3 * (k + j) + 2];
    }
    if (lfl == kLeafGeneric) {
#pragma unroll
        for (int j = 0; j < RT_SPEC_PRIMS; j++) fl[j] = __float_as_uint(tests[k + j].meta.y);
    } else {
#pragma unroll
        for (int j = 0; j < RT_SPEC_PRIMS; j++) fl[j] = lfl;
    }
#pragma unroll
    for (int j = 0; j < RT_SPEC_PRIMS; j++) {
        pin4(r[j][0]);
        pin4(r[j][1]);
        pin4(r[j][2]);
    }
#pragma unroll
    for (int j = 0; j < RT_SPEC_PRIMS; j++) {
        if (j == 0 || k + j < kend) {
            const bool sph = (fl[j] & KIND_MASK) == RT_PRIM_SPHERE;
            if (STATS) {
                if (sph) n_sph++;
                else n_tri++;
            }
            if (sph) hit_sph_rows(r[j][0], r[j][1], fl[j], k + j, k + j, o, d, prev, xf, b);
            else hit_tri_rows(r[j][0], r[j][1], r[j][2], fl[j], k + j, k + j, o, d, prev, b);
        }
    }
}

struct Walk {
    bool more;
    int ref;
    int sp;
    int pend;
};
__device__ __forceinline__ void walk_start(Walk& w, int root, bool tree)
{
    w.ref = root;
    w.sp = 0;
    w.pend = -1;
    w.more = tree;
    if (root < 0) {
        w.pend = ~root;
        w.more = false;
    }
}
struct WalkStep {
    bool ended;
    bool leaf_step, can_node;
    int sp_visit;
};
template <int STACK, bool ANY, bool STATS = false, int WIDTH = 4, class FetchT, class TestP, class RowP, class XfP>
__device__ __forceinline__ WalkStep walk_step(Walk& w, bool trav, int spec, FetchT fetch, V3 id, V3 oi, const TravStack& stk,
                                              TestP tests, RowP rows, XfP xf, V3 o, V3 d, int prev, Best& b,
                                              unsigned& n_tri, unsigned& n_sph)
{
    WalkStep st;
    st.can_node = trav && w.more && w.ref >= 0;
    const bool blocked = trav && w.pend >= 0 && !st.can_node;
    st.leaf_step = __ballot(st.can_node) == 0 || __popcll(__ballot(blocked)) >= spec;
    st.ended = false;
    st.sp_visit = w.sp;
    if (trav) {
        if (st.leaf_step) {
            if (w.pend >= 0) {
                test_leaf<STATS>(tests, rows, xf, w.pend, o, d, prev, b, n_tri, n_sph);
                w.pend = leaf_advance(w.pend, RT_SPEC_PRIMS);
                if (ANY && b.sg >= 0) {
                    w.pend = -1;
                    w.more = false;
                }
            }
        } else if (st.can_node) {
            bool pop = true;
            const auto node = fetch(w.ref);
            if constexpr (WIDTH == 2) bvh2_visit<STACK>(node, id, oi, b.t, w.ref, w.sp, stk, pop);
            else if constexpr (ANY) any_visit<STACK>(node, id, oi, b.t, w.ref, w.sp, stk, pop);
            else wide_visit<STACK>(node, id, oi, b.t, w.ref, w.sp, stk, pop);
            st.sp_visit = w.sp;
            if (pop) {
                if (w.sp > 0) w.ref = pop_ref<STACK>(stk, w.sp);
                else w.more = false;
            }
        }
        if (w.more && w.ref < 0 && w.pend < 0) {
            w.pend = ~w.ref;
            if (w.sp > 0) w.ref = pop_ref<STACK>(stk, w.sp);
            else w.more = false;
// ... 1106 lines not shown
```

raytracercore_amd/csrc/launch_params.cpp:

```cpp
#include "launch_params.h"

#include <algorithm>
#include <cmath>
#include <cstdlib>

#include "host_scene.h"

namespace rtc {

void set_item_order(PathParams& p)
{
    const char* e = getenv("RTCORE_ITEM_ORDER");
    bool dense = !(e && e[0] == '0');
    const unsigned slots = (unsigned)p.pool / 64u;
    const unsigned used = (unsigned)((p.spp + p.chunk - 1) / p.chunk);
    const unsigned n_blocks = (unsigned)(p.n_pad / 64);
    for (;; dense = false) {
        const unsigned n_real = dense ? used : (unsigned)p.n_chunks;
        const unsigned n_full = dense && p.spp % p.chunk != 0 ? used - 1 : n_real;
        p.tpb = n_full / slots;
        p.tail_first = p.tpb * (unsigned)p.pool;
        p.tail_len = (n_real - p.tpb * slots) * 64u;
        p.magic_tpb = 0;
        if (p.tpb <= 1) break;
        const uint64_t M = ((1ull << 32) + p.tpb - 1) / p.tpb;
        const uint64_t err = M * p.tpb - (1ull << 32);
        if (M < (1ull << 32) && (uint64_t)n_blocks * p.tpb * err < (1ull << 32)) {
            p.magic_tpb = (unsigned)M;
            break;
        }
    }
    p.linear = p.tail_len == 0 && p.tpb * slots == (unsigned)p.n_chunks;
    for (int g = 0; g < kMaxSplit; g++) {
        const unsigned b = g < p.n_split ? (p.split_start[g + 1] - p.split_start[g]) >> (p.log2_chunks + 6) : 0u;
        p.split_full[g] = b * p.tpb;
        p.split_tickets[g] = p.split_full[g] + (p.tail_len ? b : 0u);
    }
}

void set_blocks(PathParams& p, int n_blocks)
{
    p.n_pad = n_blocks * 64;
    p.n_split = 1;
    int want = kMaxSplit;
    if (const char* e = getenv("RTCORE_XCD_SPLIT")) want = atoi(e) > 0 ? kMaxSplit : 1;
    if (want > 1 && n_blocks >= 4 * kMaxSplit) p.n_split = kMaxSplit;
    for (int g = 0; g <= p.n_split; g++)
        p.split_start[g] = (unsigned)((int64_t)n_blocks * g / p.n_split) * (unsigned)(p.n_chunks * 64);
    set_item_order(p);
}

PathParams make_params_for(int kernel, int chunks_over, int pool_over, int x0, int y0, int w, int h, int spp,
                           uint64_t seed, uint64_t base, double chunk_npix)
{
    PathParams p{};
    p.x0 = x0;
    p.y0 = y0;
    p.w = w;
    p.h = h;
    p.band = 0;
    p.spp = spp;
    const int base_chunks = kernel >= 2 ? 64 : 24;
    int chunks = base_chunks;
    const double npix = chunk_npix > 0.0 ? chunk_npix : (double)w * (double)h;
    if (npix > 0 && npix < 2073600.0)
        chunks = (int)std::min(8.0 * base_chunks, base_chunks * std::ceil(2073600.0 / npix));
    else if (npix > 2073600.0)
        chunks = (int)std::max(base_chunks / 4.0, std::ceil(base_chunks * 2073600.0 / npix));
    if (const char* e = getenv("RTCORE_PATH_CHUNKS")) chunks = std::max(1, atoi(e));
    if (chunks_over > 0) chunks = chunks_over;
    p.chunk = std::max(1, std::min(64, (spp + chunks - 1) / chunks));
    const int used = (spp + p.chunk - 1) / p.chunk;
    p.log2_chunks = 0;
    while ((1 << p.log2_chunks) < used) p.log2_chunks++;
    p.n_chunks = 1 << p.log2_chunks;
    p.blocks_x = (w + 7) / 8;
    p.n_pad = p.blocks_x * ((h + 7) / 8) * 64;
    p.inv_blocks_x = 1.0f / (float)p.blocks_x;
    p.magic_bx = 0;
    if (p.blocks_x > 1 && !getenv("RTCORE_NO_MAGIC_DIV")) {
        const uint64_t M = ((1ull << 32) + (uint64_t)p.blocks_x - 1) / (uint64_t)p.blocks_x;
        const uint64_t err = M * (uint64_t)p.blocks_x - (1ull << 32);
        const uint64_t max_blk = (uint64_t)(p.n_pad / 64);
        if (M < (1ull << 32) && max_blk * err < (1ull << 32)) p.magic_bx = (unsigned)M;
    }
    int pool_mul = kernel == 0 ? 1 : 2;
    if (const char* e = getenv("RTCORE_POOL_MUL")) pool_mul = std::max(1, std::min(64, atoi(e)));
    if (pool_over > 0) pool_mul = std::max(1, std::min(64, pool_over / 64));
    p.pool = 64;
    while (p.pool < 64 * pool_mul && p.pool < 64 * p.n_chunks) p.pool *= 2;
    p.batch = kernel < 2 ? 64 : 0;
    if (const char* e = getenv("RTCORE_ITEM_BATCH")) p.batch = std::max(0, std::min(64, atoi(e)));
    p.scene_bound = 1;
    if (const char* e = getenv("RTCORE_SCENE_BOUND")) p.scene_bound = atoi(e) != 0 ? 1 : 0;
    p.sample_rounds = 1;
    if (const char* e = getenv("RTCORE_SAMPLE_ROUNDS")) p.sample_rounds = std::max(0, std::min(2, atoi(e)));
    p.refill = 28;
    if (const char* e = getenv("RTCORE_BVH_REFILL")) p.refill = std::max(1, std::min(64, atoi(e)));
    p.spec = 12;
    if (const char* e = getenv("RTCORE_BVH_SPEC")) p.spec = std::max(1, std::min(64, atoi(e)));
    set_blocks(p, p.n_pad / 64);
    p.seed = seed;
    p.seed_key = rt_rng_seed_key(seed);
    p.sample_base = base;
    return p;
}

PathParams make_params_rays(int kernel, int64_t n, int spp, uint64_t seed, uint64_t base, uint64_t stream_base)
{
    PathParams p = make_params_for(kernel, 0, 0, 0, 0, 8, (int)((n + 7) / 8), spp, seed, base, 2073600.0);
    p.n_rays = (unsigned)n;
    p.stream_base = stream_base;
    return p;
}

PathParams make_params_pixels(int kernel, int64_t n, int spp, uint64_t seed, uint64_t base, int width, int height)
{
    PathParams p = make_params_for(kernel, 0, 0, 0, 0, 8, (int)((n + 7) / 8), spp, seed, base, 2073600.0);
    p.n_rays = (unsigned)n;
    p.n_frame_px = (unsigned)((uint64_t)width * (uint64_t)height);
    p.inv_frame_w = 1.0f / (float)width;
    return p;
}

int64_t render_rays_max_n(int kernel, int spp)
{
    const PathParams p = make_params_for(kernel, 0, 0, 0, 0, 8, 8, spp, 0, 0, 2073600.0);
    const int64_t blocks = (int64_t)(0xF0000000ull / ((uint64_t)p.n_chunks * 64u));
    return std::min<int64_t>(blocks * 64, (int64_t)1 << 30);
}

StartRowsPlan plan_start_rows(int kernel, bool instrumented, bool vertex_normals, int camera_kind, bool dof, int chunk,
                              int grid_blocks)
{
    const StartRowsPlan off{false, 0, 0};
    if (kernel < 0 || kernel >= 2 || instrumented || vertex_normals || camera_kind != RT_CAMERA_FRUSTUM || dof) return off;
    if (chunk < 1 || chunk > kStartRowsMaxChunk || grid_blocks < 1) return off;
    if (const char* e = getenv("RTCORE_START_ROWS"))
        if (atoi(e) == 0) return off;
    const size_t bytes = (size_t)grid_blocks * 4u * (size_t)chunk * 64u * 16u;
    if (bytes > kStartRowsCap) return off;
    return StartRowsPlan{true, chunk, bytes};
}

void set_band(PathParams& p, int band, int stride, int offset)
{
    p.band = band;
    p.band_stride = stride;
    p.band_offset = offset;
    p.band_log2 = -1;
    for (int k = 0; k < 31; k++)
        if (band == (1 << k)) p.band_log2 = k;
    p.inv_band = 1.0f / (float)band;
}

int band_set_rows(int H, int band, int stride, int offset)
{
    int rows = 0;
    for (int b = offset; b * band < H; b += stride) rows += std::min(band, H - b * band);
    return rows;
}

int band_slot_rows(int H, int band, int stride)
{
    int m = 0;
    for (int o = 0; o < stride; o++) m = std::max(m, band_set_rows(H, band, stride, o));
    return m;
}

void scatter_band_set(const unsigned char* slot, size_t plane, int W, int H, int band, int stride, int offset,
                      rt_color* sum_rgb, uint32_t* samples, uint32_t* misses)
{
    const double* hs = reinterpret_cast<const double*>(slot);
    const uint32_t* hn = reinterpret_cast<const uint32_t*>(hs + 3 * plane);
    const uint32_t* hm = hn + plane;
    parallel_ranges((size_t)W, 64, [&](size_t xa, size_t xb) {
        int tr = 0;
        for (int b = offset; b * band < H; b += stride)
            for (int y = b * band; y < std::min(H, (b + 1) * band); y++, tr++)
                for (size_t x = xa; x < xb; x++) {
                    const size_t i = (size_t)tr * W + x, o = x * H + y;
                    sum_rgb[o].r += hs[i];
                    sum_rgb[o].g += hs[plane + i];
                    sum_rgb[o].b += hs[2 * plane + i];
                    samples[o] += hn[i];
                    misses[o] += hm[i];
                }
    });
}

int64_t list_tickets(const PathParams& p, uint32_t* out, int64_t cap_words)
{
    int64_t n = 0;
    for (int g = 0; g < p.n_split; g++)
        for (unsigned t = 0; t < p.split_tickets[g]; t++, n++) {
            unsigned first = 0, len = 0;
            ticket_items(p, (unsigned)g, t, first, len);
            if (3 * (n + 1) <= cap_words) {
                out[3 * n] = (uint32_t)g;
                out[3 * n + 1] = first;
                out[3 * n + 2] = len;
            }
        }
    return n;
}

}
```

raytracercore_amd/csrc/rt_kernels.h:

```cpp
#pragma once
#include "../../include/rtcore_rng.h"
#include "rt_internal.h"

namespace rtc {

constexpr int kMaxSplit = 8;
constexpr int kSplitStride = 32;

enum ItemSource : int { ITEMS_TILE = 0, ITEMS_RAYS = 1, ITEMS_PIXELS = 2, ITEMS_BEAMS = 3 };

struct PathParams {
    int x0, y0, w, h;
    int band, band_stride, band_offset;
    int band_log2;
    float inv_band;
    int spp;
    int chunk;
    int n_chunks;
    int log2_chunks;
    int blocks_x;
    int n_pad;
    int refill;
    int spec;
    int pool;
    float inv_blocks_x;
    unsigned magic_bx;
    unsigned long long seed;
    rt_key2 seed_key;
    unsigned long long sample_base;
    const rt_key2* pkeys;
    unsigned int* counter;
    int n_split;
    unsigned split_start[9];
    unsigned tpb;
    unsigned magic_tpb;
    unsigned tail_first;
    unsigned tail_len;
    int linear;
    int batch;
    unsigned split_full[8];
    unsigned split_tickets[8];
    float4* partial;
    unsigned long long* rays;
    int* stack_ovf;
    unsigned long long* stats;
    PathScene scene;
    const TestRec* tests;
    const float4* rows;
    const RectRec* rects;
    const FrameRec* frames;
    const PrimF* prims;
    const GroupRec* groups;
    const NodeF* nodes;
    const Node4Q* nodes4;
    const XformF* xf;
    const MatF* mats;
    const float4* vnormals;
    const PrimD* prims_d;
    float4* ray_log;
    unsigned int* ray_log_n;
    unsigned int ray_log_cap;
    float4* rec_rays;
    float4* rec_samples;
    unsigned int rec_max;
    union {
        const double2* ray_list;
        const uint32_t* pixel_list;
        const double2* beam_list;
        float4* starts;
    };
    unsigned int n_rays;
    int start_rows;
    union {
        unsigned long long stream_base;
        struct {
            unsigned int n_frame_px;
            float inv_frame_w;
        };
    };
    int scene_bound;
    int sample_rounds;
    const unsigned int* cull;
};
static_assert(__builtin_offsetof(PathParams, start_rows) == __builtin_offsetof(PathParams, n_rays) + 4 &&
                  __builtin_offsetof(PathParams, scene_bound) == __builtin_offsetof(PathParams, n_rays) + 16,
              "start_rows takes the padding after n_rays");
static_assert(__builtin_offsetof(PathParams, sample_rounds) == __builtin_offsetof(PathParams, scene_bound) + 4 &&
                  __builtin_offsetof(PathParams, cull) == __builtin_offsetof(PathParams, scene_bound) + 8,
              "sample_rounds takes the padding after scene_bound");
constexpr int kCullTable = 4;
constexpr int kRecRows = 6;

template <class ParT>
__host__ __device__ inline void ticket_items(const ParT& p, unsigned g, unsigned t, unsigned& first, unsigned& len)
{
    const unsigned full = p.split_full[g];
    unsigned blk, off;
    if (t < full) {
        blk = p.magic_tpb ? (unsigned)(((unsigned long long)t * p.magic_tpb) >> 32) : t;
        off = (t - blk * p.tpb) * (unsigned)p.pool;
        len = (unsigned)p.pool;
    } else {
        blk = t - full;
        off = p.tail_first;
        len = p.tail_len;
    }
    first = p.split_start[g] + (blk << (p.log2_chunks + 6)) + off;
}

constexpr unsigned kRoundsNum = 4, kRoundsDen = 5;
template <class ParT>
__host__ __device__ inline bool ticket_rounds(const ParT& p, int recursion, bool first, unsigned prev_rays)
{
    if (p.sample_rounds != 1) return p.sample_rounds == 2;
    if (first) return false;
    const unsigned long long samples = (unsigned long long)(unsigned)p.pool * (unsigned long long)(unsigned)p.chunk;
    return (unsigned long long)prev_rays * kRoundsDen >= samples * (unsigned long long)(unsigned)(recursion + 1) * kRoundsNum;
}

struct TraceRaysParams {
    const float4* rays;
    float2* hits;
    unsigned int n;
    unsigned int* counter;
    int* stack_ovf;
    const TestRec* tests;
    const float4* rows;
    const Node4Q* nodes4;
    const XformF* xf;
    int root4;
    int spec;
    const GroupRec* outer;
    const RectRec* outer_rects;
    const FrameRec* outer_boxes;
    unsigned long long* stats;
};

#ifndef __HIPCC_RTC__
struct QueryParams {
    const double2* rays;
    float4* hits;
    unsigned int n;
    unsigned int* counter;
    int* stack_ovf;
    PathScene scene;
    const TestRec* tests;
    const float4* rows;
    const RectRec* rects;
    const FrameRec* frames;
    const PrimF* prims;
    const GroupRec* groups;
    const Node4Q* nodes4;
    const XformF* xf;
    const float4* vnormals;
    int root4;
    int n_nodes4;
    int spec;
};
constexpr int kHitRows = 3;

int query_blocks_per_cu(int kernel);
hipError_t launch_query(const QueryParams& p, int kernel, int grid_blocks, hipStream_t stream);
hipError_t launch_query_exact(const DevScene& s, const rt_ray* d_rays, unsigned n, rt_hit* d_hits, hipStream_t stream);
struct OccludedParams {
    QueryParams q;
    const double* t_max;
    unsigned char* out;
    int early;
};
int occluded_blocks_per_cu(int kernel);
hipError_t launch_occluded(const OccludedParams& p, int kernel, int grid_blocks, hipStream_t stream);
hipError_t launch_occluded_exact(const DevScene& s, const rt_ray* d_rays, const double* d_t_max, unsigned n,
                                 unsigned char* d_out, hipStream_t stream);
void fill_launch(const DevScene& s, int variant, PathParams& p);

hipError_t launch_primary_ids(const DevScene& s, const CameraD& cam, int x0, int y0, int w, int h, int mode,
                              int32_t* d_ids, hipStream_t stream);

hipError_t launch_select_pixels(const DevScene& s, const CameraD& cam, const rt_select_item* d_items, int n_items, int x0,
                                int y0, int w, int h, rt_selection* d_out, hipStream_t stream);
hipError_t launch_select_rays(const DevScene& s, const rt_select_item* d_items, int n_items, const rt_ray* d_rays,
                              unsigned n, rt_selection* d_out, hipStream_t stream);

int path_variant(int kernel, bool lds);
constexpr int kStackOverflow = 44;
constexpr int kTestSpares = 3;
int path_wide_stack();
size_t path_lds_bytes(const DevScene& s);
size_t path_dyn_lds(const DevScene& s, int variant);
hipError_t launch_path(const DevScene& s, const CameraF* d_cam, const PathParams* d_params, int variant,
                       int grid_blocks, hipStream_t stream, bool stats, ItemSource src = ITEMS_TILE);
int path_blocks_per_cu(int variant, size_t dyn_lds, bool stats, bool vn, ItemSource src = ITEMS_TILE);
int trace_rays_blocks_per_cu(int waves);
int debug_vn_rehit(const double v0[3], const double e01[3], const double e02[3], int mirror, double u, double v,
                   const float dir[3], int* inside, double* t, double o[3]);
hipError_t launch_trace_rays(const TraceRaysParams& p, int waves, int grid_blocks, hipStream_t stream);
hipError_t launch_pixel_keys(rt_key2 seed_key, int w, int h, rt_key2* out, hipStream_t stream);
hipError_t compact_leaves(const TestRec* d_tests, int n_records, float4* d_rows, NodeF* d_nodes, int n_nodes,
                          Node4Q* d_nodes4, int n_nodes4, bool rewrite, hipStream_t stream);

hipError_t launch_accumulate(const PathParams& p, double* d_sum, uint32_t* d_samples, uint32_t* d_misses,
                             hipStream_t stream, size_t plane = 0);
hipError_t launch_tonemap(int w, int h, const double* d_sum, const uint32_t* d_samples, const uint32_t* d_misses,
                          rt_color back, double back_alpha, double exposure, int32_t* d_argb, hipStream_t stream);
struct TileRec {
    double r, g, b;
    uint32_t samples, misses;
};
hipError_t launch_accumulate_rays(const PathParams& p, double* d_sum, uint32_t* d_samples, uint32_t* d_misses,
                                  TileRec* d_recs, hipStream_t stream);
hipError_t launch_accumulate_pixels(const PathParams& p, double* d_sum, uint32_t* d_samples, uint32_t* d_misses,
                                    double* d_q, uint32_t* d_batches, size_t plane, hipStream_t stream);
struct PixelRec {
    double r, g, b, q;
    uint32_t samples, misses, batches, pad;
};
hipError_t launch_accumulate_pixels_recs(const PathParams& p, PixelRec* d_recs, hipStream_t stream);
hipError_t launch_tile_host_layout(int w, int h, const double* d_sum, const uint32_t* d_samples,
                                  const uint32_t* d_misses, TileRec* d_out, hipStream_t stream);
hipError_t launch_trace_host_layout(int w, int h, int spp, int recursion, const float4* d_rays, const float4* d_samples,
                                    float4* d_rays_out, float4* d_samples_out, hipStream_t stream);
hipError_t launch_colors_1spp(const PathParams& p, float* d_out, hipStream_t stream);

#endif

}
```

raytracercore_amd/csrc/rt_scene.h:

```cpp
#pragma once
#include <algorithm>
#include <array>
#include <functional>
#include <string>
#include <vector>

#include "block_cull.h"
#include "host_scene.h"
#include "launch_params.h"
#include "rt_jit.h"
#include "rt_kernels.h"
#include "scene_records.h"

using namespace rtc;

#define HIP_TRY(expr)                                                                                  \
    do {                                                                                                \
        hipError_t e_ = (expr);                                                                         \
        if (e_ != hipSuccess) {                                                                         \
            set_error(std::string(#expr) + ": " + hipGetErrorString(e_));                               \
            return e_ == hipErrorOutOfMemory ? RT_ERR_OOM : RT_ERR_HIP;                                 \
        }                                                                                               \
    } while (0)

// ... 29 lines not shown
        return hipMemcpy(p, v.data(), v.size() * sizeof(T), hipMemcpyHostToDevice);
    }
};

template <class T>
struct HostBuf {
    T* p = nullptr;
    size_t n = 0;
    ~HostBuf() { release(); }
    void release()
    {
        if (p) (void)hipHostFree(p);
        p = nullptr;
        n = 0;
    }
    hipError_t reserve(size_t count)
    {
        if (count <= n) return hipSuccess;
        release();
        hipError_t e = hipHostMalloc((void**)&p, std::max<size_t>(count, 1) * sizeof(T), hipHostMallocDefault);
        if (e == hipSuccess) n = count;
        return e;
    }
};

struct BruteDev {
    DevBuf<PrimF> prims;
    DevBuf<TestRec> tests;
    DevBuf<RectRec> rects;
    DevBuf<FrameRec> frames;
    DevBuf<GroupRec> groups;
    hipError_t upload(const BruteOrder& o)
    {
        hipError_t e = prims.upload(o.prims);
        if (e == hipSuccess) e = tests.upload(o.tests);
        if (e == hipSuccess) e = rects.upload(o.rects);
        if (e == hipSuccess) e = frames.upload(o.frames);
        if (e == hipSuccess) e = groups.upload(o.groups);
        return e;
    }
};

struct rt_scene {
    int device = 0;
    int n_cu = 256;
    rt_scene_params params{};
    std::vector<HostPrim> host;
    int traversal = RT_TRAVERSAL_AUTO, resolved = RT_TRAVERSAL_BRUTE;
    int variant = 0;
    int blocks_per_cu = 1;
    RefBvh ref;
    bool ref_built = false;
    SahBvh sah;
    Bvh4 bvh4;
    struct {
        int builder = RT_BVH_BUILDER_HOST;
        int n_nodes2 = 0, n_nodes4 = 0, root2 = 0, root4 = 0, depth2 = 0, stack4 = 0, rounds = 0;
        int leaves4 = 0, compact4 = 0;
        float gpu_ms = 0.0f;
    } bvh;
    DevBuf<int32_t> order_d;
    std::vector<char> bvh_outer;
    double ms_prepare = 0, ms_bvh = 0, ms_upload = 0;
    BruteLayout layout;
    int group_max = 0;
    DevScene dev{};
    BruteDev flat_d, grouped_d, bvh_d;
    DevBuf<float4> rows_bvh;
    std::vector<GroupRec> groups_gr_host;
    struct BruteHost {
        std::vector<GroupRec> groups;
        std::vector<RectRec> rects;
        std::vector<FrameRec> frames;
        std::vector<TestRec> tests;
    } flat_h, grouped_h;
    std::vector<XformF> xf_h;
    unsigned jit_gen = 0;
    struct {
        int variant = -1;
        unsigned gen = 0;
        hipFunction_t fn = nullptr;
        int blocks_per_cu = 0;
        int status = 0;
        double compile_ms = 0;
        bool from_cache = false;
        std::string error;
        std::string header;
    } jit;
    double grouped_measured = 0;
    DevBuf<NodeF> nodes;
    DevBuf<Node4Q> nodes4;
    DevBuf<Node4Q> hot4;
    DevBuf<XformF> xf;
    DevBuf<MatF> mats;
    DevBuf<float4> vnormals;
    DevBuf<PrimD> prims_d;
    DevBuf<XformD> xf_d;
    DevBuf<RefNode> ref_nodes;
    DevBuf<unsigned int> counter;
    DevBuf<rt_key2> pkeys;
    bool pkeys_valid = false;
    uint64_t pkeys_seed = 0;
    DevBuf<float4> starts;
    DevBuf<int> stack_ovf;
    DevBuf<unsigned long long> rays;
    DevBuf<float4> partial;
    DevBuf<double> sum, colors;
    DevBuf<float> colors32;
    HostBuf<unsigned char> stage;
    HostBuf<unsigned long long> rays_h;
    static constexpr int kCopyChunks = 8;
    std::array<hipEvent_t, kCopyChunks> copy_ev{};
    hipStream_t copy_stream = nullptr;
    std::array<hipEvent_t, kCopyChunks> band_ev{};
    DevBuf<uint32_t> samples, misses;
    DevBuf<int32_t> ids;
    DevBuf<rt_ray> query_rays;
    DevBuf<rt_hit> query_hits;
    std::array<hipEvent_t, 2> query_up_ev{};
    DevBuf<rt_ray> primary_rays;
    DevBuf<double> occluded_t_max;
    DevBuf<unsigned char> occluded_out;
    DevBuf<TileRec> render_rays_recs;
    int rays_variant = -1, rays_blocks_per_cu = 1;
    int beams_variant = -1, beams_blocks_per_cu = 1;
    DevBuf<uint32_t> pixel_list;
    DevBuf<PixelRec> pixel_recs;
    int pixels_variant = -1, pixels_blocks_per_cu = 1;
    DevBuf<rt_select_item> select_items;
    DevBuf<rt_ray> select_rays;
    DevBuf<rt_selection> select_out;
    bool stats_on = false;
    float4* ray_log = nullptr;
    unsigned int* ray_log_n = nullptr;
    unsigned int ray_log_cap = 0;
    int stats_blocks_per_cu = 1;
    DevBuf<unsigned long long> stats_buf;
    bool tracing = false;
    DevBuf<unsigned long long> trace_stats;
    DevBuf<float4> trace_rays, trace_samples, trace_out;
    CameraD camd{};
    CameraF camf{};
    DevBuf<CameraF> camf_d;
    static constexpr int kParamRing = 256;
    DevBuf<PathParams> params_d;
    PathParams* params_h = nullptr;
    std::array<hipEvent_t, kParamRing> slot_ev{};
    unsigned params_next = 0;
    struct CullEntry {
        bool valid = false;
        unsigned cam_gen = 0;
        CullWindow win{};
        int n_live = 0, n_blocks = 0;
        uint64_t dead_px = 0, used = 0;
        DevBuf<unsigned int> dev;
        HostBuf<unsigned int> host;
        hipEvent_t up = nullptr;
    };
    static constexpr int kCullEntries = 4;
    std::array<CullEntry, kCullEntries> cull_cache;
    uint64_t cull_clock = 0;
    unsigned cam_gen = 0;
    bool has_camera = false;
    bool flat_overflow = false;
    hipStream_t stream = nullptr;
    static constexpr int kTimeRing = 64;
    std::array<hipEvent_t, kTimeRing> t_start{}, t_end{};
    uint64_t launches = 0;
    hipEvent_t done_ev = nullptr;
    hipStream_t last_stream = nullptr;
    bool any_op = false;
    uint64_t device_bytes = 0;

    ~rt_scene()
    {
        if (jit.fn) jit_release(device, jit.fn);
        if (params_h) (void)hipHostFree(params_h);
        for (hipEvent_t e : slot_ev)
            if (e) (void)hipEventDestroy(e);
        if (done_ev) (void)hipEventDestroy(done_ev);
        for (CullEntry& c : cull_cache)
            if (c.up) (void)hipEventDestroy(c.up);
        for (hipEvent_t e : copy_ev)
            if (e) (void)hipEventDestroy(e);
        for (hipEvent_t e : band_ev)
            if (e) (void)hipEventDestroy(e);
        for (hipEvent_t e : query_up_ev)
            if (e) (void)hipEventDestroy(e);
        if (copy_stream) {
            (void)hipStreamSynchronize(copy_stream);
            (void)hipStreamDestroy(copy_stream);
        }
        for (int i = 0; i < kTimeRing; i++) {
            if (t_start[i]) (void)hipEventDestroy(t_start[i]);
            if (t_end[i]) (void)hipEventDestroy(t_end[i]);
        }
        if (stream) (void)hipStreamDestroy(stream);
    }
};

struct CopyPlan {
    size_t a[rt_scene::kCopyChunks], b[rt_scene::kCopyChunks];
    int n = 0;
};

namespace rtc {

int builder_for(int n_bvh);
int group_max_default();
int build_bvhs(rt_scene* s);
int upload_scene(rt_scene* s);
int ensure_ref_bvh(rt_scene* s);
int resolve_traversal(rt_scene* s);
int calibrate_grouping(rt_scene* s);
int prepare_jit(rt_scene* s);
int check_tile(rt_scene* s, int x0, int y0, int w, int h);
PathParams make_params(rt_scene* s, int x0, int y0, int w, int h, int spp, uint64_t seed, uint64_t base,
                       double chunk_npix = 0.0);
int run_path(rt_scene* s, PathParams& p, unsigned long long* d_rays, hipStream_t stream, bool timed = true);
int upload_params(rt_scene* s, const PathParams& p, hipStream_t stream, const PathParams** d_out);
int end_op(rt_scene* s, hipStream_t stream);
int queue_copy(rt_scene* s, CopyPlan& plan, const void* d_src, size_t a, size_t b, size_t rec_bytes, int k,
               hipStream_t stream);
int consume_copies(rt_scene* s, const CopyPlan& plan, const std::function<void(const unsigned char*, size_t, size_t)>& consume);
struct RenderList {
    ItemSource src;
    size_t rec_bytes;
    int64_t chunk;
    const char* what;
};
int render_list_device(rt_scene* s, const RenderList& kind, const char* name, const void* d_list, int64_t n, int32_t spp,
                       uint64_t seed, uint64_t sample_base, uint64_t stream_base, double* d_sum, uint32_t* d_samples,
                       uint32_t* d_misses, unsigned long long* d_count, void* stream);
int render_list_host(rt_scene* s, const RenderList& kind, const char* name, const void* list, int64_t n, int32_t spp,
                     uint64_t seed, uint64_t sample_base, uint64_t stream_base, rt_color* sum_rgb, uint32_t* samples,
                     uint32_t* misses, uint64_t* rays_out);
const char* check_pixel_list(const uint32_t* pixels, int64_t n, uint64_t npix, int64_t* at);
int copy_consume(rt_scene* s, const void* d_src, size_t n_items, size_t rec_bytes,
                 const std::function<void(const unsigned char*, size_t, size_t)>& consume);

}
```

raytracercore_amd/csrc/scene_records.cpp:

```cpp
#include "scene_records.h"

#include <algorithm>
#include <array>
#include <cmath>
#include <cstdlib>
#include <cstring>
#include <functional>
#include <string>
#include <unordered_map>

namespace rtc {

float4 f4(Vec4d v, float w) { return make_float4((float)v.x, (float)v.y, (float)v.z, w); }
float as_f(int v)
{
    float f;
    std::memcpy(&f, &v, 4);
    return f;
}
float as_f(uint32_t v)
{
    float f;
    std::memcpy(&f, &v, 4);
    return f;
}

void make_exact_records(const std::vector<HostPrim>& H, std::vector<PrimD>& pd, std::vector<XformD>& xd)
{
    const int n = (int)H.size();
    pd.resize(n);
    xd.clear();
    for (int i = 0; i < n; i++) {
        const HostPrim& p = H[i];
        PrimD& d = pd[i];
        std::memset(&d, 0, sizeof d);
        d.flags = p.flags;
        d.xf = -1;
        if (p.kind == RT_PRIM_TRIANGLE) {
            d.a = p.v[0];
            d.b = p.e01;
            d.c = p.e02;
            d.d = p.n;
            for (int k = 0; k < 3; k++) d.vn[k] = p.vn[k];
        } else if (p.kind == RT_PRIM_SPHERE) {
            d.a = p.center;
            d.b = v4d(p.radius, p.radius_sqr, 0, 0);
            if (p.flags & F_TRANSFORMED) {
                d.xf = (int)xd.size();
                XformD X;
                std::memcpy(X.to_world, p.to_world, sizeof X.to_world);
                std::memcpy(X.to_obj, p.to_obj, sizeof X.to_obj);
                std::memcpy(X.to_normal, p.to_normal, sizeof X.to_normal);
                xd.push_back(X);
            }
        } else {
            d.a = p.pn;
            d.b = v4d(p.pd, 0, 0, 0);
        }
    }
}

namespace {

double luminance(rt_color c) { return 0.299 * c.r + 0.587 * c.g + 0.114 * c.b; }
uint32_t p_flags_with_axis(uint32_t flags, int axis) { return flags | ((uint32_t)(axis + 1) << F_AXIS_SHIFT); }
void set_rect_axis(PrimF& f, uint32_t flags, int axis)
{
    const uint32_t fl = p_flags_with_axis(flags, axis);
    std::memcpy(&f.b.w, &fl, 4);
    f.c = make_float4(axis == 0 ? 1.0f : 0.0f, axis == 1 ? 1.0f : 0.0f, axis == 2 ? 1.0f : 0.0f, 0.0f);
}

}

PrimF make_primf(const std::vector<HostPrim>& H, const std::vector<int>& xf_index, int i)
{
    {
        const HostPrim& p = H[i];
        PrimF f;
        std::memset(&f, 0, sizeof f);
        if (p.kind == RT_PRIM_TRIANGLE) {
            f.a = f4(p.v[0], as_f(i));
            f.b = f4(p.e01, as_f(p.flags));
            f.c = make_float4(0.0f, 0.0f, 0.0f, 0.0f);
            f.d = f4(p.n, 0.0f);
        } else if (p.kind == RT_PRIM_SPHERE) {
            f.a = f4(p.center, as_f(i));
            f.b = make_float4((float)p.radius, (float)(1.0 / p.radius), as_f(xf_index[i]), as_f(p.flags));
            if (!(p.flags & F_TRANSFORMED)) {
                const double ir = 1.0 / p.radius;
                f.c = make_float4(0.0f, 0.0f, 0.0f, (float)ir);
                f.d = make_float4((float)(-p.center.x * ir), (float)(-p.center.y * ir), (float)(-p.center.z * ir), 0.0f);
            }
        } else {
            f.a = f4(p.pn, as_f(i));
            f.b = make_float4((float)p.pd, 0.0f, 0.0f, as_f(p.flags));
            f.d = f4(p.pn, 0.0f);
        }
        return f;
    }
}
TestRec make_testrec(const std::vector<HostPrim>& H, const std::vector<int>& xf_index, int i)
{
    {
        const HostPrim& p = H[i];
        TestRec t;
        std::memset(&t, 0, sizeof t);
        t.meta = make_float4(as_f(i), as_f(p.flags), 0.0f, 0.0f);
        if (p.kind == RT_PRIM_TRIANGLE) {
            const Vec4d e1 = p.e01, e2 = p.e02, nn = cross_s(p.e01, p.e02);
            const double D = dot_s(e1, cross_s(e2, nn));
            const Vec4d rows[3] = {cross_s(e2, nn), cross_s(nn, e1), nn};
            float4* out[3] = {&t.r0, &t.r1, &t.r2};
            for (int k = 0; k < 3; k++) {
                const Vec4d r = divs(rows[k], D);
                *out[k] = make_float4((float)r.x, (float)r.y, (float)r.z,
                                      (float)(-(r.x * p.v[0].x + r.y * p.v[0].y + r.z * p.v[0].z)));
            }
        } else if (p.kind == RT_PRIM_SPHERE) {
            t.r0 = f4(p.center, (float)p.radius);
            t.r1 = make_float4((float)p.radius_sqr, as_f(xf_index[i]), 0.0f, 0.0f);
        } else {
            t.r0 = f4(p.pn, (float)p.pd);
        }
        return t;
    }
}

int rect_axis_of(const HostPrim& p)
{
    if (p.kind != RT_PRIM_TRIANGLE || !(p.flags & F_MIRROR) || (p.flags & F_HASNORMALS)) return -1;
    const double e1[3] = {p.e01.x, p.e01.y, p.e01.z}, e2[3] = {p.e02.x, p.e02.y, p.e02.z};
    for (int k = 0; k < 3; k++) {
        const int a = (k + 1) % 3, b = (k + 2) % 3;
        if (e1[k] != 0 || e2[k] != 0) continue;
        const bool e1a = e1[a] != 0 && e1[b] == 0, e1b = e1[b] != 0 && e1[a] == 0;
        const bool e2a = e2[a] != 0 && e2[b] == 0, e2b = e2[b] != 0 && e2[a] == 0;
        if ((e1a && e2b) || (e1b && e2a)) return k;
    }
    return -1;
}

namespace {

struct OrderBuilder {
    const std::vector<HostPrim>& H;
    const std::vector<int>& xf_index;
    const int n;
    std::vector<int> kind_of;
    const bool use_boxes = !getenv("RTCORE_NO_BOXES");

    OrderBuilder(const std::vector<HostPrim>& H_, const std::vector<int>& xf_index_)
        : H(H_), xf_index(xf_index_), n((int)H_.size()), kind_of(H_.size())
// ... 546 lines not shown
    std::vector<int> all;
    for (int i = 0; i < n; i++)
        if (b.kind_of[i] != 5) all.push_back(i);
    out.flat = b.build_order({all}, {0});
    if (!outer.empty()) {
        std::vector<int> ids;
        for (int i = 0; i < n; i++)
            if (outer[i]) ids.push_back(i);
        out.outer = b.build_order({ids}, {0});
    }
    for (int k = 0; k < 3; k++) out.nr[k] = out.flat.nr[k];
    out.nt = out.flat.nt;
    out.ns = out.flat.ns;
    out.layout = layout_of(out.flat);
    for (int i = 0; i < n; i++) out.np += b.kind_of[i] == 5;
    int kGroupMax = group_max;
    if (const char* e = getenv("RTCORE_GROUP_MAX")) kGroupMax = std::max(1, atoi(e));
    out.group_max = kGroupMax;
    int kSuperMin = 3;
    if (const char* e = getenv("RTCORE_GROUP_SUPER")) kSuperMin = std::max(0, atoi(e));
    bool group_boxes = false;
    if (const char* e = getenv("RTCORE_GROUP_BOXES")) group_boxes = atoi(e) != 0;
    GroupCut c{sah, kGroupMax, kSuperMin, std::vector<int>(n, -1), {}, {}, {}, {}};
    if (group_boxes && b.use_boxes) c.find_scene_boxes(b, all);
    if ((int)all.size() <= 4096 && !sah.order.empty()) c.split(sah.root, false);
    if (!c.cut.empty()) out.grouped = b.build_order(c.cut, c.skips);
    return out;
}

int grouping_max_leaf(GroupingTree who, int n_prims, bool has_outer)
{
    switch (who) {
    case GroupingTree::Scene: return n_prims > 256 && !has_outer ? 3 : 2;
    case GroupingTree::LayoutReport: return n_prims > 256 ? 4 : 2;
    case GroupingTree::JitHeader: return n_prims > 256 ? 3 : 2;
    }
    return 2;
}

HostRecords make_host_records(const std::vector<HostPrim>& H, int max_leaf, int group_max, const SahBvh* sah,
                              const std::vector<char>* outer)
{
    HostRecords r;
    const int n = (int)H.size();
    r.xf_index.assign(n, -1);
    for (int i = 0; i < n; i++) {
        const HostPrim& p = H[i];
        r.n_bvh += p.kind != RT_PRIM_PLANE;
        r.n_planes += p.kind == RT_PRIM_PLANE;
        r.n_vn += (p.kind == RT_PRIM_TRIANGLE && (p.flags & F_HASNORMALS)) ? 1 : 0;
        if (p.kind == RT_PRIM_SPHERE && (p.flags & F_TRANSFORMED)) {
            r.xf_index[i] = (int)r.xf.size();
            r.xf.push_back(make_xformf(p));
        }
    }
    SahBvh own;
    if (!sah && max_leaf > 0 && r.n_bvh > 0) own = build_sah_bvh(H, max_leaf);
    const SahBvh& tree = sah ? *sah : own;
    r.sah_root = tree.root;
    r.orders = make_brute_orders(H, r.xf_index, tree, group_max, outer ? *outer : std::vector<char>{});
    return r;
}

MatTable make_materials(const std::vector<HostPrim>& H, double air_ior)
{
    MatTable t;
    const int n = (int)H.size();
    t.mat_of.resize(n);
    std::unordered_map<std::string, int32_t> mat_index;
    for (int i = 0; i < n; i++) {
        const HostPrim& p = H[i];
        const bool refl = p.shininess > 0;
        rt_color spec = refl ? p.specular : rt_color{0, 0, 0};
        rt_color refr = refl ? p.refraction : rt_color{0, 0, 0};
        MatF m;
        std::memset(&m, 0, sizeof m);
        m.emission = make_float4((float)p.emission.r, (float)p.emission.g, (float)p.emission.b, (float)luminance(p.emission));
        m.diffuse = make_float4((float)p.diffuse.r, (float)p.diffuse.g, (float)p.diffuse.b, (float)luminance(p.diffuse));
        m.specular = make_float4((float)spec.r, (float)spec.g, (float)spec.b, (float)luminance(spec));
        m.refraction = make_float4((float)refr.r, (float)refr.g, (float)refr.b, (float)luminance(refr));
        m.shininess = (float)p.shininess;
        m.ior = (float)p.ior;
        m.flags = p.flags;
        m.inv_shininess = (float)(1.0 / p.shininess);
        m.eta_enter = p.ior != 0 ? (float)(air_ior / p.ior) : 0.0f;
        m.eta_exit = p.ior != 0 ? (float)(p.ior / air_ior) : 0.0f;
        m.pad[0] = m.pad[1] = 0.0f;
        const std::string key(reinterpret_cast<const char*>(&m), sizeof m);
        auto it = mat_index.find(key);
        if (it == mat_index.end()) {
            it = mat_index.emplace(key, (int32_t)t.mats.size()).first;
            t.mats.push_back(m);
        }
        t.mat_of[i] = it->second;
    }
    return t;
}

std::vector<GroupRec> groups_nearest_first(const std::vector<GroupRec>& g, const CameraD& cam)
{
    const double px = cam.position.x, py = cam.position.y, pz = cam.position.z;
    auto dist2 = [&](const GroupRec& G) {
        const double dx = std::max({0.0, (double)G.lo.x - px, px - (double)G.hi.x});
        const double dy = std::max({0.0, (double)G.lo.y - py, py - (double)G.hi.y});
        const double dz = std::max({0.0, (double)G.lo.z - pz, pz - (double)G.hi.z});
        return dx * dx + dy * dy + dz * dz;
    };
    std::vector<GroupRec> out;
    std::function<void(size_t, size_t)> emit = [&](size_t a, size_t b) {
        std::vector<std::pair<size_t, size_t>> sib;
        for (size_t i = a; i < b; i += 1 + (size_t)std::max(0, g[i].skip))
            sib.push_back({i, std::min(b, i + 1 + (size_t)std::max(0, g[i].skip))});
        std::stable_sort(sib.begin(), sib.end(), [&](const auto& x, const auto& y) { return dist2(g[x.first]) < dist2(g[y.first]); });
        for (const auto& [i, e] : sib) {
            out.push_back(g[i]);
            emit(i + 1, e);
        }
    };
    emit(0, g.size());
    return out;
}

XformF make_xformf(const HostPrim& p)
{
    XformF F;
    const double c[3] = {p.center.x, p.center.y, p.center.z};
    for (int r = 0; r < 3; r++) {
        F.to_world[r] = make_float4((float)p.to_world[4 * r], (float)p.to_world[4 * r + 1], (float)p.to_world[4 * r + 2],
                                    (float)p.to_world[4 * r + 3]);
        double row[4] = {0, 0, 0, 0};
        for (int k = 0; k < 3; k++) {
            const double nk = p.to_normal[4 * r + k] / p.radius;
            for (int j = 0; j < 3; j++) row[j] += nk * p.to_world[4 * k + j];
            row[3] += nk * (p.to_world[4 * k + 3] - c[k]);
        }
        F.normal[r] = make_float4((float)row[0], (float)row[1], (float)row[2], (float)row[3]);
    }
    return F;
}

uint32_t scene_facts(const std::vector<HostPrim>& H)
{
    uint32_t facts = 0;
    for (const HostPrim& p : H) {
        if (std::isinf(p.shininess) && p.shininess > 0) facts |= FACT_INF_SHININESS;
        if ((float)p.ior != 0.0f) facts |= FACT_IOR;
        if (p.flags & F_TRANSFORMED) facts |= FACT_XF;
        if (p.flags & F_HASNORMALS) facts |= FACT_VN;
        if (p.kind == RT_PRIM_SPHERE) facts |= FACT_SPHERE;
    }
    return facts;
}

SceneBound make_scene_bound(const std::vector<HostPrim>& H)
{
    double lo[3] = {INFINITY, INFINITY, INFINITY}, hi[3] = {-INFINITY, -INFINITY, -INFINITY};
    bool any = false, bad = false;
    auto grow = [&](int k, double a, double b) {
        if (!(std::isfinite(a) && std::isfinite(b))) bad = true;
        lo[k] = std::min(lo[k], a);
        hi[k] = std::max(hi[k], b);
    };
    for (const HostPrim& p : H) {
        if (p.kind == RT_PRIM_TRIANGLE) {
            const Vec4d v3 = add(add(p.v[0], p.e01), p.e02);
            const int nv = (p.flags & F_MIRROR) ? 4 : 3;
            for (int j = 0; j < nv; j++) {
                const Vec4d& v = j < 3 ? p.v[j] : v3;
                const double c[3] = {v.x, v.y, v.z};
                for (int k = 0; k < 3; k++) grow(k, c[k], c[k]);
            }
        } else if (p.kind == RT_PRIM_SPHERE) {
            const double c[3] = {p.center.x, p.center.y, p.center.z};
            for (int k = 0; k < 3; k++) {
                double mid = c[k], half = std::fabs(p.radius);
                if (p.flags & F_TRANSFORMED) {
                    const double* m = p.to_obj + 4 * k;
                    mid = m[0] * c[0] + m[1] * c[1] + m[2] * c[2] + m[3];
                    half = std::fabs(p.radius) * std::sqrt(m[0] * m[0] + m[1] * m[1] + m[2] * m[2]);
                }
                grow(k, mid - half, mid + half);
            }
        } else {
            continue;
        }
        any = true;
    }
    SceneBound b{};
    if (!any) {
        b.empty = 1;
        b.limit = INFINITY;
        return b;
    }
    double M = 0.0;
    for (int k = 0; k < 3; k++) M = std::max(M, std::max(std::fabs(lo[k]), std::fabs(hi[k])));
    const double limit = 1024.0 * M, pad = std::ldexp(limit + M, -18);
    if (bad || !std::isfinite(M) || !((float)(limit + M + pad) < INFINITY)) {
        b.limit = -1.0f;
        return b;
    }
    for (int k = 0; k < 3; k++) {
        const double a = lo[k] - pad, c = hi[k] + pad;
        b.lo[k] = (float)a;
        if ((double)b.lo[k] > a) b.lo[k] = std::nextafterf(b.lo[k], -INFINITY);
        b.hi[k] = (float)c;
        if ((double)b.hi[k] < c) b.hi[k] = std::nextafterf(b.hi[k], INFINITY);
    }
    b.limit = (float)limit;
    if ((double)b.limit > limit) b.limit = std::nextafterf(b.limit, 0.0f);
    b.pad = (float)pad;
    return b;
}

static constexpr int kOuterMax = 64;
static constexpr double kOuterAreaDiv = 1024.0;

void select_outer(const std::vector<HostPrim>& H, std::vector<char>& out)
{
    out.clear();
    const int n = (int)H.size();
    float slo[3] = {INFINITY, INFINITY, INFINITY}, shi[3] = {-INFINITY, -INFINITY, -INFINITY};
    int nb = 0;
    std::vector<std::pair<double, int>> cand;
    for (int i = 0; i < n; i++) {
        if (H[i].kind == RT_PRIM_PLANE) continue;
        nb++;
        float lo[3], hi[3];
        sah_prim_box(H[i], lo, hi);
        for (int k = 0; k < 3; k++) {
            slo[k] = std::min(slo[k], lo[k]);
            shi[k] = std::max(shi[k], hi[k]);
        }
        const int k = rect_axis_of(H[i]);
        if (k < 0) continue;
        const double a = (double)(hi[(k + 1) % 3] - lo[(k + 1) % 3]) * (double)(hi[(k + 2) % 3] - lo[(k + 2) % 3]);
        cand.push_back({a, i});
    }
    double face = 0.0;
    for (int k = 0; k < 3; k++)
        face = std::max(face, (double)(shi[(k + 1) % 3] - slo[(k + 1) % 3]) * (double)(shi[(k + 2) % 3] - slo[(k + 2) % 3]));
    std::sort(cand.begin(), cand.end(), [](const auto& a, const auto& b) { return a.first != b.first ? a.first > b.first : a.second < b.second; });
    std::vector<char> m(n, 0);
    int k = 0;
    for (const auto& c : cand) {
        if (k == kOuterMax || !(c.first * kOuterAreaDiv >= face)) break;
        m[c.second] = 1;
        k++;
    }
    if (k > 0 && k < nb) out = std::move(m);
}

}
```

raytracercore_amd/csrc/scene_records.h:

```cpp
#pragma once
#include <vector>

#include "host_scene.h"

namespace rtc {

PrimF make_primf(const std::vector<HostPrim>& H, const std::vector<int>& xf_index, int i);
TestRec make_testrec(const std::vector<HostPrim>& H, const std::vector<int>& xf_index, int i);
float as_f(int v);
float as_f(uint32_t v);
float4 f4(Vec4d v, float w);
void make_exact_records(const std::vector<HostPrim>& H, std::vector<PrimD>& pd, std::vector<XformD>& xd);

struct BruteLayout {
    int rects = 0, boxes = 0, frames = 0, frame_boxes = 0, frame_rects = 0, tris = 0, sphs = 0;
};
struct BruteOrder {
    std::vector<PrimF> prims;
    std::vector<TestRec> tests;
    std::vector<RectRec> rects;
    std::vector<FrameRec> frames;
    std::vector<GroupRec> groups;
    int nr[3] = {0, 0, 0}, nt = 0, ns = 0;
    bool overflow = false;
    int tris0 = 0, sphs0 = 0;
};
struct BruteOrders {
    BruteOrder flat, grouped;
    BruteOrder outer;
    int nr[3] = {0, 0, 0}, nt = 0, ns = 0, np = 0;
    int group_max = 0;
    BruteLayout layout;
};
int rect_axis_of(const HostPrim& p);

BruteOrders make_brute_orders(const std::vector<HostPrim>& H, const std::vector<int>& xf_index, const SahBvh& sah,
                              int group_max, const std::vector<char>& outer = {});

struct HostRecords {
    std::vector<int> xf_index;
    std::vector<XformF> xf;
    int n_bvh = 0, n_planes = 0, n_vn = 0;
    int sah_root = 0;
    BruteOrders orders;
};
HostRecords make_host_records(const std::vector<HostPrim>& H, int max_leaf, int group_max, const SahBvh* sah = nullptr,
                              const std::vector<char>* outer = nullptr);

enum class GroupingTree {
    Scene,
    LayoutReport,
    JitHeader,
};
int grouping_max_leaf(GroupingTree who, int n_prims, bool has_outer);

struct MatTable {
    std::vector<MatF> mats;
    std::vector<int32_t> mat_of;
};
MatTable make_materials(const std::vector<HostPrim>& H, double air_ior);

std::vector<GroupRec> groups_nearest_first(const std::vector<GroupRec>& g, const CameraD& cam);
XformF make_xformf(const HostPrim& p);
uint32_t scene_facts(const std::vector<HostPrim>& H);
SceneBound make_scene_bound(const std::vector<HostPrim>& H);
void select_outer(const std::vector<HostPrim>& H, std::vector<char>& out);

}
```

raytracercore_amd/csrc/scene_upload.hip:

```cpp
#include <atomic>
#include <cmath>
#include <cstdio>
#include <cstdlib>
#include <cstring>
#include <unordered_map>

#include "bvh_gpu.h"
#include "rt_scene.h"

namespace rtc {

static std::atomic<int> g_builder{RT_BVH_BUILDER_AUTO};
constexpr int kGpuBuildMin = 1 << 22;

int builder_for(int n_bvh)
{
    int b = g_builder.load();
    if (b == RT_BVH_BUILDER_AUTO)
        if (const char* e = getenv("RTCORE_BVH_BUILDER"))
            b = std::strcmp(e, "gpu") == 0 ? RT_BVH_BUILDER_GPU : std::strcmp(e, "host") == 0 ? RT_BVH_BUILDER_HOST : b;
    if (b == RT_BVH_BUILDER_AUTO) b = n_bvh >= kGpuBuildMin ? RT_BVH_BUILDER_GPU : RT_BVH_BUILDER_HOST;
    return n_bvh > 0 ? b : RT_BVH_BUILDER_HOST;
}

// ... 160 lines not shown
            tree[k] = primf(s->sah.order[k]);
            ttree[k] = testrec(s->sah.order[k]);
        });
        set_mats(tree);
        bv.insert(bv.begin(), tree.begin(), tree.end());
        tbv.insert(tbv.begin(), ttree.begin(), ttree.end());
    }
    HIP_TRY(s->prims_d.upload(pd));
    HIP_TRY(s->xf_d.upload(xd));
    HIP_TRY(s->flat_d.upload(flat));
    HIP_TRY(s->grouped_d.upload(grouped));
    s->groups_gr_host = grouped.groups;
    s->flat_h = {flat.groups, flat.rects, flat.frames, flat.tests};
    s->grouped_h = {grouped.groups, grouped.rects, grouped.frames, grouped.tests};
    s->xf_h = xf;
    if (s->bvh.builder != RT_BVH_BUILDER_GPU) {
        HIP_TRY(s->bvh_d.prims.upload(bv));
        tbv.resize(tbv.size() + kTestSpares, TestRec{});
        HIP_TRY(s->bvh_d.tests.upload(tbv));
        HIP_TRY(s->nodes.upload(s->sah.nodes));
        HIP_TRY(s->nodes4.upload(s->bvh4.nodes));
    }
    if (!orders.outer.groups.empty()) {
        HIP_TRY(s->bvh_d.rects.upload(orders.outer.rects));
        HIP_TRY(s->bvh_d.frames.upload(orders.outer.frames));
        HIP_TRY(s->bvh_d.groups.upload(orders.outer.groups));
    }
    HIP_TRY(s->xf.upload(xf));
    HIP_TRY(s->mats.upload(mats));
    HIP_TRY(s->vnormals.upload(vn));
    s->device_bytes = pd.size() * sizeof(PrimD) + xd.size() * sizeof(XformD) +
                      (flat.prims.size() + grouped.prims.size() + n_bvh_records) * sizeof(PrimF) +
                      (flat.tests.size() + grouped.tests.size() + n_bvh_records + 1) * sizeof(TestRec) +
                      (size_t)s->bvh.n_nodes2 * sizeof(NodeF) + (size_t)s->bvh.n_nodes4 * sizeof(Node4Q) +
                      xf.size() * sizeof(XformF) + mats.size() * sizeof(MatF) + vn.size() * sizeof(float4);

    {
        const char* e = getenv("RTCORE_COMPACT_LEAVES");
        const bool rewrite = !(e && e[0] == '0');
        const size_t n_rec = n_bvh_records + kTestSpares;
        HIP_TRY(s->rows_bvh.reserve(3 * n_rec));
        HIP_TRY(compact_leaves(s->bvh_d.tests.p, (int)n_rec, s->rows_bvh.p, s->nodes.p, s->bvh.n_nodes2, s->nodes4.p,
                               s->bvh.n_nodes4, rewrite, s->stream));
        HIP_TRY(hipStreamSynchronize(s->stream));
    }
    std::vector<Node4Q> hot;
    int root4_hot = s->bvh.root4;
    {
        std::vector<Node4Q> all4((size_t)s->bvh.n_nodes4);
        if (!all4.empty())
            HIP_TRY(hipMemcpy(all4.data(), s->nodes4.p, all4.size() * sizeof(Node4Q), hipMemcpyDeviceToHost));
        s->bvh.leaves4 = s->bvh.compact4 = 0;
        for (const Node4Q& nd : all4)
            for (float f : {nd.c.z, nd.c.w, nd.d.x, nd.d.y}) {
                int32_t c;
                std::memcpy(&c, &f, 4);
                if (c < 0 && c != RT_NODE4_EMPTY) {
                    s->bvh.leaves4++;
                    s->bvh.compact4 += ((~c) & kLeafCompact) != 0;
                }
            }
        int k_hot = 64;
        if (const char* e = getenv("RTCORE_HOT_NODES")) k_hot = std::max(0, std::min(1024, atoi(e)));
        if (k_hot > 0 && s->bvh.root4 >= 0 && s->bvh.n_nodes4 > 0) {
            std::vector<int> order{s->bvh.root4};
            std::unordered_map<int, int> slot_of{{s->bvh.root4, 0}};
            for (size_t q = 0; q < order.size() && (int)order.size() < k_hot; q++) {
                const Node4Q& nd = all4[order[q]];
                int32_t ch[4];
                std::memcpy(&ch[0], &nd.c.z, 4);
                std::memcpy(&ch[1], &nd.c.w, 4);
                std::memcpy(&ch[2], &nd.d.x, 4);
                std::memcpy(&ch[3], &nd.d.y, 4);
                for (int c : ch)
                    if (c >= 0 && (int)order.size() < k_hot && !slot_of.count(c)) {
                        slot_of[c] = (int)order.size();
                        order.push_back(c);
                    }
            }
            for (int g : order) {
                Node4Q nd = all4[g];
                float* refs[4] = {&nd.c.z, &nd.c.w, &nd.d.x, &nd.d.y};
                for (float* r : refs) {
                    int32_t c;
                    std::memcpy(&c, r, 4);
                    auto it = c >= 0 ? slot_of.find(c) : slot_of.end();
                    if (it != slot_of.end()) {
                        c = RT_HOT_BIT | it->second;
                        std::memcpy(r, &c, 4);
                    }
                }
                hot.push_back(nd);
            }
            root4_hot = RT_HOT_BIT | 0;
        }
    }
    HIP_TRY(s->hot4.upload(hot));

    DevScene& d = s->dev;
    d.hot4 = s->hot4.p;
    d.n_hot4 = (int)hot.size();
    d.root4_hot = root4_hot;
    d.tests_bf = s->flat_d.tests.p;
    d.tests_bvh = s->bvh_d.tests.p;
    d.rows_bvh = s->rows_bvh.p;
    d.rects_bf = s->flat_d.rects.p;
    d.frames_bf = s->flat_d.frames.p;
    d.prims_bf = s->flat_d.prims.p;
    d.groups_bf = s->flat_d.groups.p;
    d.tests_gr = s->grouped_d.tests.p;
    d.rects_gr = s->grouped_d.rects.p;
    d.frames_gr = s->grouped_d.frames.p;
    d.prims_gr = s->grouped_d.prims.p;
    d.groups_gr = s->grouped_d.groups.p;
    d.n_groups_gr = (int)grouped.groups.size();
    d.pln0_bf = (int)flat.prims.size() - np;
    d.pln0_gr = grouped.prims.empty() ? 0 : (int)grouped.prims.size() - np;
    d.pln0_bvh = (int)n_bvh_records - np;
    d.rects_bvh = s->bvh_d.rects.p;
    d.frames_bvh = s->bvh_d.frames.p;
    d.groups_bvh = s->bvh_d.groups.p;
    d.n_outer = orders.outer.groups.empty() ? 0 : 1;
    for (int k = 0; k < 3; k++) d.n_rect[k] = orders.nr[k];
    d.n_tri = orders.nt;
    d.n_sph = orders.ns;
    d.n_pln = np;
    d.prims_bvh = s->bvh_d.prims.p;
    d.nodes = s->nodes.p;
    d.n_nodes = s->bvh.n_nodes2;
    d.root = s->bvh.root2;
    d.nodes4 = s->nodes4.p;
    d.n_nodes4 = s->bvh.n_nodes4;
    d.root4 = s->bvh.root4;
    d.xf = s->xf.p;
    d.mats = s->mats.p;
    d.vnormals = s->vnormals.p;
    d.n_mats = (int)mats.size();
    d.n_xf = (int)xf.size();
    d.facts = facts;
    d.n_vn = rec.n_vn;
    d.prims_d = s->prims_d.p;
    d.xf_d = s->xf_d.p;
    d.ref_nodes = nullptr;
    d.n_ref_nodes = 0;
    d.width = s->params.width;
    d.height = s->params.height;
    d.recursion = s->params.recursion;
    d.debug_geom = s->params.debug_geom;
    d.air_ior = (float)s->params.air_ior;
    const rt_color& a = s->params.ambient;
    d.ambient = make_float3((float)a.r, (float)a.g, (float)a.b);
    d.ambient_miss = (a.r == -1 && a.g == -1 && a.b == -1) ? 1 : 0;
    d.bound = make_scene_bound(H);
    return RT_OK;
}

int ensure_ref_bvh(rt_scene* s)
{
    if (s->ref_built) return RT_OK;
    s->ref = build_ref_bvh(s->host);
    HIP_TRY(hipSetDevice(s->device));
    HIP_TRY(s->ref_nodes.upload(s->ref.nodes));
    s->dev.ref_nodes = s->ref_nodes.p;
    s->dev.n_ref_nodes = (int)s->ref.nodes.size();
    s->device_bytes += s->ref.nodes.size() * sizeof(RefNode);
    s->ref_built = true;
    return RT_OK;
}

int resolve_traversal(rt_scene* s)
{
    int t = s->traversal;
    if (t == RT_TRAVERSAL_AUTO) {
        const int n_bvh = s->dev.pln0_bvh;
        t = n_bvh <= 48 ? RT_TRAVERSAL_BRUTE : RT_TRAVERSAL_BVH;
    }
    if (s->traversal == RT_TRAVERSAL_AUTO && t == RT_TRAVERSAL_BRUTE && s->grouped_measured > 1.25)
        t = RT_TRAVERSAL_GROUPED;
    if (t == RT_TRAVERSAL_GROUPED && s->dev.n_groups_gr == 0) t = RT_TRAVERSAL_BRUTE;
    if (t == RT_TRAVERSAL_BRUTE && s->flat_overflow) {
        set_error("brute-force traversal: more than 65535 triangles or 32767 spheres in the flat order");
        return RT_ERR_ARG;
    }
    int kernel = t == RT_TRAVERSAL_GROUPED ? 1 : 0;
    if (t == RT_TRAVERSAL_BVH2) {
        if (s->bvh.depth2 >= 24 + kStackOverflow) {
            set_error("BVH2 deeper than the kernel's traversal stack");
            return RT_ERR_ARG;
        }
        kernel = 2;
    } else if (t == RT_TRAVERSAL_BVH) {
        if (s->bvh.stack4 > path_wide_stack() + kStackOverflow) {
            set_error("wide BVH needs a deeper traversal stack than the kernel's");
            return RT_ERR_ARG;
        }
        kernel = 3;
    }
    s->resolved = t;
    const size_t lds = path_lds_bytes(s->dev);
    const int plain = path_variant(kernel, false), staged = path_variant(kernel, true);
    const int occ_plain = path_blocks_per_cu(plain, path_dyn_lds(s->dev, plain), false, s->dev.n_vn > 0);
    const int occ_staged = lds <= 64 * 1024 ? path_blocks_per_cu(staged, path_dyn_lds(s->dev, staged), false, s->dev.n_vn > 0) : 0;
    bool use_lds = occ_staged >= occ_plain || (kernel <= 1 && occ_staged > 0 && jit_enabled());
    if (const char* e = getenv("RTCORE_PATH_LDS")) use_lds = e[0] == '1' && occ_staged > 0;
    s->variant = use_lds ? staged : plain;
    s->blocks_per_cu = use_lds ? occ_staged : occ_plain;
    if (s->stats_on) s->stats_blocks_per_cu = path_blocks_per_cu(s->variant, path_dyn_lds(s->dev, s->variant), true, s->dev.n_vn > 0);
    return RT_OK;
}

int calibrate_grouping(rt_scene* s)
{
    s->grouped_measured = 0;
    if (s->traversal != RT_TRAVERSAL_AUTO || s->dev.n_groups_gr < 2) return RT_OK;
    const int n_bvh = s->dev.pln0_bvh;
    if (n_bvh > 48) return RT_OK;
    const int w = std::min(64, s->params.width), h = std::min(64, s->params.height);
    const int x0 = (s->params.width - w) / 2, y0 = (s->params.height - h) / 2;
    const int saved_variant = s->variant, saved_blocks = s->blocks_per_cu;
    const int variant = path_variant(1, false);
    s->variant = variant;
    s->blocks_per_cu = path_blocks_per_cu(variant, 0, true, s->dev.n_vn > 0);
    HIP_TRY(s->stats_buf.reserve(RT_STATS_COUNT));
    HIP_TRY(s->sum.reserve((size_t)3 * w * h));
    HIP_TRY(s->samples.reserve((size_t)w * h));
    HIP_TRY(s->misses.reserve((size_t)w * h));
    HIP_TRY(hipMemsetAsync(s->stats_buf.p, 0, RT_STATS_COUNT * sizeof(unsigned long long), s->stream));
    HIP_TRY(hipMemsetAsync(s->rays.p, 0, sizeof(unsigned long long), s->stream));
    const bool was_on = s->stats_on;
    const int was_blocks = s->stats_blocks_per_cu;
    s->stats_on = true;
    s->stats_blocks_per_cu = s->blocks_per_cu;
    PathParams p = make_params(s, x0, y0, w, h, 2, 0x5EEDull, 0);
    p.pool = 64;
    set_item_order(p);
    p.batch = 0;
    int rc = run_path(s, p, s->rays.p, s->stream, false);
    if (rc == RT_OK) rc = end_op(s, s->stream);
    s->stats_on = was_on;
    s->stats_blocks_per_cu = was_blocks;
    s->variant = saved_variant;
    s->blocks_per_cu = saved_blocks;
    if (rc != RT_OK) return rc;
    unsigned long long st[RT_STATS_COUNT], rays = 0;
    HIP_TRY(hipMemcpyAsync(st, s->stats_buf.p, sizeof st, hipMemcpyDeviceToHost, s->stream));
    HIP_TRY(hipMemcpyAsync(&rays, s->rays.p, sizeof rays, hipMemcpyDeviceToHost, s->stream));
    HIP_TRY(hipStreamSynchronize(s->stream));
    HIP_TRY(hipMemsetAsync(s->stats_buf.p, 0, RT_STATS_COUNT * sizeof(unsigned long long), s->stream));
    if (rays == 0) return RT_OK;
    const double flat = 20.0 * (n_bvh - s->dev.n_sph) + 30.0 * s->dev.n_sph;
    const double grouped = (15.0 * st[0] + 20.0 * st[1] + 30.0 * st[2]) / (double)rays;
    s->grouped_measured = flat / std::max(grouped, 1e-9);
    return resolve_traversal(s);
}

PathParams make_params(rt_scene* s, int x0, int y0, int w, int h, int spp, uint64_t seed, uint64_t base,
                       double chunk_npix)
{
    return make_params_for(s->variant >> 1, 0, 0, x0, y0, w, h, spp, seed, base, chunk_npix);
}

int check_tile(rt_scene* s, int x0, int y0, int w, int h)
{
    if (!s) {
        set_error("null scene");
        return RT_ERR_ARG;
    }
    if (!s->has_camera) {
        set_error("no camera set (rt_scene_set_camera)");
        return RT_ERR_STATE;
    }
    if (w <= 0 || h <= 0 || x0 < 0 || y0 < 0 || x0 + w > s->params.width || y0 + h > s->params.height) {
        set_error("tile outside the frame");
        return RT_ERR_ARG;
    }
    return RT_OK;
}

int prepare_jit(rt_scene* s)
{
    const char* eg = getenv("RTCORE_JIT_GROUPED");
    const bool grouped_ok = !(eg && eg[0] == '0');
    const bool eligible = jit_enabled() && !s->stats_on &&
                          (s->variant == path_variant(0, true) || (grouped_ok && s->variant == path_variant(1, true)));
    if (!eligible) {
        s->jit.status = 0;
        return 0;
    }
    const bool grouped = s->variant == path_variant(1, true);
    const unsigned gen = s->jit_gen;
    if (s->jit.variant == s->variant && s->jit.gen == gen) {
        s->jit.status = s->jit.fn ? 1 : (s->jit.error.empty() ? 0 : -1);
        return s->jit.fn ? 1 : 0;
    }
    PathParams lp{};
    fill_launch(s->dev, s->variant, lp);
    const auto& B = grouped ? s->grouped_h : s->flat_h;
    static const bool cam_in = getenv("RTCORE_JIT_CAMERA") && getenv("RTCORE_JIT_CAMERA")[0] == '1';
    const std::string header =
        jit_scene_header(lp.scene, s->camf, grouped || cam_in, B.groups, B.rects, B.frames, B.tests, s->xf_h);
    if (s->jit.variant == s->variant && s->jit.fn && header == s->jit.header) {
        s->jit.gen = gen;
        s->jit.status = 1;
        s->jit.compile_ms = 0;
        s->jit.from_cache = true;
        return 1;
    }
    s->jit.error.clear();
    s->jit.variant = s->variant;
    s->jit.gen = gen;
    s->jit.header = header;
    if (s->jit.fn) jit_release(s->device, s->jit.fn);
    s->jit.fn = nullptr;
    if (const char* dump = getenv("RTCORE_JIT_DUMP")) {
        if (FILE* f = fopen(dump, "w")) {
            fwrite(header.data(), 1, header.size(), f);
            fclose(f);
        }
    }
    JitKernel k;
    std::string err;
    if (!jit_kernel(s->device, header, grouped, k, err)) {
        s->jit.status = -1;
        s->jit.error = err;
        return 0;
    }
    int n = 0;
    if (hipModuleOccupancyMaxActiveBlocksPerMultiprocessor(&n, k.fn, 256, path_dyn_lds(s->dev, s->variant)) !=
            hipSuccess ||
        n < 1) {
        jit_release(s->device, k.fn);
        (void)hipGetLastError();
        s->jit.status = -1;
        s->jit.error = "occupancy query of the scene-specialised kernel failed";
        return 0;
    }
    s->jit.fn = k.fn;
    s->jit.blocks_per_cu = n;
    s->jit.status = 1;
    s->jit.compile_ms = k.compile_ms;
    s->jit.from_cache = k.from_cache;
    return 1;
}

int upload_params(rt_scene* s, const PathParams& p, hipStream_t stream, const PathParams** d_out)
{
    if (!s->params_h) {
        HIP_TRY(hipHostMalloc(&s->params_h, sizeof(PathParams) * rt_scene::kParamRing, hipHostMallocDefault));
        HIP_TRY(s->params_d.reserve(rt_scene::kParamRing));
    }
    const unsigned slot = s->params_next++ % rt_scene::kParamRing;
    hipEvent_t& sev = s->slot_ev[slot];
    if (sev) HIP_TRY(hipEventSynchronize(sev));
    else HIP_TRY(hipEventCreateWithFlags(&sev, hipEventDisableTiming));
    s->params_h[slot] = p;
    HIP_TRY(hipMemcpyAsync(s->params_d.p + slot, s->params_h + slot, sizeof(PathParams), hipMemcpyHostToDevice, stream));
    HIP_TRY(hipEventRecord(sev, stream));
    *d_out = s->params_d.p + slot;
    return RT_OK;
}

constexpr int kCullMinBlocks = 4096;
static int plan_block_cull(rt_scene* s, const PathParams& p, rt_scene::CullEntry*& ent, bool& fresh)
{
    ent = nullptr;
    fresh = false;
    if ((s->variant >> 1) >= 2 || s->stats_on || s->tracing) return RT_OK;
    if (const char* e = getenv("RTCORE_BLOCK_CULL"))
        if (atoi(e) == 0) return RT_OK;
    int min_blocks = kCullMinBlocks;
    if (const char* e = getenv("RTCORE_BLOCK_CULL_MIN")) min_blocks = std::max(1, atoi(e));
    const int n_blocks = p.n_pad / 64;
    if (n_blocks < min_blocks || p.blocks_x > 0xFFFF || n_blocks / p.blocks_x > 0xFFFF) return RT_OK;
    const CullWindow win{p.x0, p.y0, p.w, p.h, p.band > 0 ? p.band : 0, p.band > 0 ? p.band_stride : 0,
                         p.band > 0 ? p.band_offset : 0};
    auto same = [](const CullWindow& a, const CullWindow& b) {
        return a.x0 == b.x0 && a.y0 == b.y0 && a.w == b.w && a.h == b.h && a.band == b.band &&
               a.band_stride == b.band_stride && a.band_offset == b.band_offset;
    };
    rt_scene::CullEntry* c = nullptr;
    for (rt_scene::CullEntry& e : s->cull_cache)
        if (e.valid && e.cam_gen == s->cam_gen && same(e.win, win)) c = &e;
    if (!c) {
        auto age = [&](const rt_scene::CullEntry& e) { return e.valid && e.cam_gen == s->cam_gen ? e.used : 0; };
        c = &s->cull_cache[0];
        for (rt_scene::CullEntry& e : s->cull_cache)
            if (age(e) < age(*c)) c = &e;
        c->valid = false;
        if (c->up) HIP_TRY(hipEventSynchronize(c->up));
        else HIP_TRY(hipEventCreateWithFlags(&c->up, hipEventDisableTiming));
        std::vector<unsigned char> dead;
        c->n_live = cull_blocks(s->camf, s->dev.bound, s->dev.n_pln, win, dead);
        c->n_blocks = n_blocks;
        c->dead_px = dead_pixels(win, dead);
        c->cam_gen = s->cam_gen;
        c->win = win;
        if (c->n_live < n_blocks) {
            const size_t words = (size_t)kCullTable + (size_t)c->n_live + (size_t)n_blocks;
            HIP_TRY(c->host.reserve(words));
            HIP_TRY(c->dev.reserve(words));
            unsigned int* h = c->host.p;
            h[0] = (unsigned)(c->dead_px & 0xFFFFFFFFull);
            h[1] = (unsigned)(c->dead_px >> 32);
            h[2] = (unsigned)c->n_live;
            h[3] = (unsigned)n_blocks;
            unsigned live = 0;
            for (int b = 0; b < n_blocks; b++) {
                if (!dead[(size_t)b]) h[kCullTable + live] = (unsigned)(b % p.blocks_x) | (unsigned)(b / p.blocks_x) << 16;
                h[kCullTable + c->n_live + b] = dead[(size_t)b] ? 0xFFFFFFFFu : live;
                live += dead[(size_t)b] ? 0u : 1u;
            }
            fresh = true;
        } else {
            c->valid = true;
        }
    }
    c->used = ++s->cull_clock;
    if (c->n_live < c->n_blocks) ent = c;
    return RT_OK;
}

int run_path(rt_scene* s, PathParams& p, unsigned long long* d_rays, hipStream_t stream, bool timed)
{
    rt_scene::CullEntry* cull = nullptr;
    bool cull_fresh = false;
    p.cull = nullptr;
    const int crc = plan_block_cull(s, p, cull, cull_fresh);
    if (crc != RT_OK) return crc;
    if (cull) {
        set_blocks(p, cull->n_live);
        p.cull = cull->dev.p;
    }
    const size_t need = (size_t)p.n_chunks * (size_t)p.n_pad;
    uint64_t tickets = 0;
    for (int g = 0; g < p.n_split; g++) tickets += p.split_tickets[g];
    if (need > 0xF0000000ull || tickets > need / 64) {
        set_error("tile x spp too large for one launch; split the tile");
        return RT_ERR_ARG;
    }
    HIP_TRY(s->partial.reserve(need));
    HIP_TRY(s->counter.reserve(kMaxSplit * kSplitStride));
    p.partial = s->partial.p;
    p.counter = s->counter.p;
    p.rays = d_rays;
    p.stats = s->stats_on ? (s->tracing ? s->trace_stats.p : s->stats_buf.p) : nullptr;
    p.ray_log = (s->stats_on && !s->tracing && s->variant >= 4) ? s->ray_log : nullptr;
    p.ray_log_n = s->ray_log_n;
    p.ray_log_cap = s->ray_log_cap;
    if (p.ray_log) s->ray_log = nullptr;
    if (s->any_op && stream != s->last_stream) HIP_TRY(hipStreamWaitEvent(stream, s->done_ev, 0));
    if (cull && cull_fresh) {
        const size_t words = (size_t)kCullTable + (size_t)cull->n_live + (size_t)cull->n_blocks;
        HIP_TRY(hipMemcpyAsync(cull->dev.p, cull->host.p, words * sizeof(unsigned int), hipMemcpyHostToDevice, stream));
        HIP_TRY(hipEventRecord(cull->up, stream));
        cull->valid = true;
    }
    HIP_TRY(hipMemsetAsync(p.counter, 0, sizeof(unsigned int) * kSplitStride * p.n_split, stream));
    int grid = s->n_cu * (s->stats_on ? s->stats_blocks_per_cu : s->blocks_per_cu);
    p.stack_ovf = nullptr;
    if (s->variant >= 4) {
        HIP_TRY(s->stack_ovf.reserve((size_t)grid * 256 * kStackOverflow));
        p.stack_ovf = s->stack_ovf.p;
    }
    const int jit = s->tracing ? 0 : prepare_jit(s);
    int jit_grid = jit ? s->n_cu * s->jit.blocks_per_cu : 0;
    if ((s->variant >> 1) < 2 && !s->stats_on) {
        constexpr double kSamplesPerLane = 6.0;
        const double samples = ((double)p.w * (double)p.h - (cull ? (double)cull->dead_px : 0.0)) * (double)p.spp;
        int cap = (int)std::ceil(samples / ((double)s->n_cu * 256.0 * kSamplesPerLane));
        if (const char* e = getenv("RTCORE_GRID_BPC")) cap = atoi(e);
        cap = std::max(1, cap);
        if (jit) jit_grid = s->n_cu * std::min(s->jit.blocks_per_cu, cap);
        else grid = s->n_cu * std::min(s->blocks_per_cu, cap);
    }
    const int tslot = (int)(s->launches % rt_scene::kTimeRing);
    if (timed) HIP_TRY(hipEventRecord(s->t_start[tslot], stream));
    fill_launch(s->dev, s->variant, p);
    p.pkeys = nullptr;
    static const bool pkeys_on = !(getenv("RTCORE_PIXEL_KEYS") && getenv("RTCORE_PIXEL_KEYS")[0] == '0');
    if ((s->variant >> 1) < 2 && !s->stats_on && pkeys_on) {
        if (!s->pkeys_valid || s->pkeys_seed != p.seed) {
            HIP_TRY(s->pkeys.reserve((size_t)s->params.width * (size_t)s->params.height));
            HIP_TRY(launch_pixel_keys(p.seed_key, s->params.width, s->params.height, s->pkeys.p, stream));
            s->pkeys_valid = true;
            s->pkeys_seed = p.seed;
        }
        p.pkeys = s->pkeys.p;
    }
    p.starts = nullptr;
    p.start_rows = 0;
    const StartRowsPlan sr = plan_start_rows(s->variant >> 1, s->stats_on || s->tracing, s->dev.n_vn > 0, s->camf.kind,
                                             s->camf.dof != 0.0f, p.chunk, jit ? jit_grid : grid);
    if (sr.on) {
        HIP_TRY(s->starts.reserve(sr.bytes / sizeof(float4)));
        p.starts = s->starts.p;
        p.start_rows = sr.rows;
    }
    const PathParams* pa = nullptr;
    const int urc = upload_params(s, p, stream, &pa);
    if (urc != RT_OK) return urc;
    if (jit) {
        const CameraF* ca = s->camf_d.p;
        void* args[] = {&ca, &pa};
        HIP_TRY(hipModuleLaunchKernel(s->jit.fn, jit_grid, 1, 1, 256, 1, 1,
                                      (unsigned)path_dyn_lds(s->dev, s->variant), stream, args, nullptr));
    } else {
        HIP_TRY(launch_path(s->dev, s->camf_d.p, pa, s->variant, grid, stream, s->stats_on));
    }
    if (timed) {
        HIP_TRY(hipEventRecord(s->t_end[tslot], stream));
        s->launches++;
    }
    return RT_OK;
}

int end_op(rt_scene* s, hipStream_t stream)
{
    HIP_TRY(hipEventRecord(s->done_ev, stream));
    s->last_stream = stream;
    s->any_op = true;
    return RT_OK;
}

int queue_copy(rt_scene* s, CopyPlan& plan, const void* d_src, size_t a, size_t b, size_t rec_bytes, int k,
               hipStream_t stream)
{
    k = std::max(1, std::min(k, rt_scene::kCopyChunks - plan.n));
    const size_t per = (b - a + k - 1) / k;
    for (int c = 0; c < k; c++) {
        const size_t ca = std::min(b, a + c * per), cb = std::min(b, a + (c + 1) * per);
        hipEvent_t& ev = s->copy_ev[plan.n];
        if (!ev) HIP_TRY(hipEventCreateWithFlags(&ev, hipEventDisableTiming));
        if (cb > ca)
            HIP_TRY(hipMemcpyAsync(s->stage.p + ca * rec_bytes, static_cast<const unsigned char*>(d_src) + ca * rec_bytes,
                                   (cb - ca) * rec_bytes, hipMemcpyDeviceToHost, stream));
        HIP_TRY(hipEventRecord(ev, stream));
        plan.a[plan.n] = ca;
        plan.b[plan.n] = cb;
        plan.n++;
    }
    return RT_OK;
}

int consume_copies(rt_scene* s, const CopyPlan& plan, const std::function<void(const unsigned char*, size_t, size_t)>& consume)
{
    constexpr size_t kMinItems = 65536;
    size_t longest = 0;
    for (int k = 0; k < plan.n; k++) longest = std::max(longest, plan.b[k] - plan.a[k]);
    const size_t S = std::max<size_t>(1, std::min<size_t>((size_t)host_threads(), longest / kMinItems));
    std::atomic<int> failed{0};
    host_run((size_t)plan.n * S, [&](size_t t) {
        const size_t k = t / S, j = t % S;
        const size_t a0 = plan.a[k], b0 = plan.b[k];
        const size_t sl = (b0 - a0 + S - 1) / S;
        const size_t a = std::min(b0, a0 + j * sl), b = std::min(b0, a + sl);
        if (hipEventSynchronize(s->copy_ev[k]) != hipSuccess) {
            failed = 1;
            return;
        }
        if (b > a) consume(s->stage.p, a, b);
    });
    if (failed) {
        set_error("device -> host copy failed");
        return RT_ERR_HIP;
    }
    return RT_OK;
}

int copy_consume(rt_scene* s, const void* d_src, size_t n_items, size_t rec_bytes,
                 const std::function<void(const unsigned char*, size_t, size_t)>& consume)
{
    const size_t bytes = n_items * rec_bytes;
    HIP_TRY(s->stage.reserve(bytes));
    CopyPlan plan;
    const int K = (int)std::max<size_t>(1, std::min<size_t>(rt_scene::kCopyChunks, bytes >> 20));
    int rc = queue_copy(s, plan, d_src, 0, n_items, rec_bytes, K, s->stream);
    if (rc != RT_OK) return rc;
    return consume_copies(s, plan, consume);
}

}

extern "C" int rt_set_bvh_builder(int32_t builder)
{
    if (builder < RT_BVH_BUILDER_AUTO || builder > RT_BVH_BUILDER_GPU) {
        set_error("rt_set_bvh_builder: bad argument");
        return RT_ERR_ARG;
    }
    g_builder.store(builder);
    return RT_OK;
}
```

Before: 131,300 Mrays/s.

## Add per-block primitive unit masks to skip unreachable primitives on camera rays

Splits the flat brute-force primitive list into units (rects, boxes, frames, triangles, spheres), computes a padded world bound per unit, and projects each into screen space to build a 64-bit mask per live 8x8 pixel block. The masks are uploaded with the block-cull table, and a new trace_units path lets first-bounce camera rays test only the primitives whose projection can overlap their block. This aims to cut intersection work for primary rays in brute traversal, at the cost of host-side mask computation, a larger cull upload, and extra mask branching in the kernel. It only applies when there are no planes or vertex normals and at most 64 units.

```diff
diff --git a/include/rtcore.h b/include/rtcore.h
--- a/include/rtcore.h
+++ b/include/rtcore.h
@@ -135,6 +135,10 @@
 int rt_debug_block_cull(const rt_prim* prims, int32_t n_prims, const rt_camera* camera, int32_t width, int32_t height,
                         int32_t x0, int32_t y0, int32_t w, int32_t h, int32_t band, int32_t band_stride,
                         int32_t band_offset, uint8_t* dead, int64_t cap, int32_t* info);
+int rt_debug_block_units(const rt_prim* prims, int32_t n_prims, const rt_camera* camera, int32_t width, int32_t height,
+                         int32_t x0, int32_t y0, int32_t w, int32_t h, int32_t band, int32_t band_stride,
+                         int32_t band_offset, int32_t* unit_first, int32_t* unit_ids, int64_t cap_ids, float* unit_box,
+                         uint8_t* dead, uint64_t* masks, int64_t cap_blocks, int32_t* info);
 int rt_debug_start_rows(int32_t kernel, const rt_camera* camera, int32_t w, int32_t h, int32_t spp, int32_t chunks,
                         int32_t grid_blocks, int32_t flags, int64_t* info);
 int rt_debug_ray_log(rt_scene* scene, void* d_log, uint32_t cap, void* d_count);
diff --git a/raytracercore_amd/__init__.py b/raytracercore_amd/__init__.py
--- a/raytracercore_amd/__init__.py
+++ b/raytracercore_amd/__init__.py
@@ -286,6 +286,9 @@
         "rt_debug_scene_bound": (C.c_int, [P(rt_prim), C.c_int32, P(C.c_float), P(C.c_float), P(C.c_float)]),
         "rt_debug_block_cull": (C.c_int, [P(rt_prim), C.c_int32, P(rt_camera)] + [C.c_int32] * 9 +
                                 [P(C.c_uint8), C.c_int64, P(C.c_int32)]),
+        "rt_debug_block_units": (C.c_int, [P(rt_prim), C.c_int32, P(rt_camera)] + [C.c_int32] * 9 +
+                                 [P(C.c_int32), P(C.c_int32), C.c_int64, P(C.c_float), P(C.c_uint8), P(C.c_uint64),
+                                  C.c_int64, P(C.c_int32)]),
         "rt_debug_start_rows": (C.c_int, [C.c_int32, P(rt_camera)] + [C.c_int32] * 6 + [P(C.c_int64)]),
         "rt_debug_ray_log": (C.c_int, [C.c_void_p, C.c_void_p, C.c_uint32, C.c_void_p]),
         "rt_debug_vn_rehit": (C.c_int, [P(C.c_double), P(C.c_double), P(C.c_double), C.c_int32, C.c_double,
@@ -466,6 +469,40 @@
     return dead[:bx * by].reshape(by, bx).astype(bool), int(live)
 
 
+def block_units(prims: Sequence[rt_prim], camera: rt_camera, size: Tuple[int, int],
+                window: Optional[Tuple[int, int, int, int]] = None,
+                bands: Optional[Tuple[int, int, int]] = None) -> dict:
+    lib = load_library()
+    n = len(prims)
+    arr = (rt_prim * max(1, n))(*prims)
+    cam = rt_camera.from_buffer_copy(camera)
+    b = bands or (0, 0, 0)
+    W, H = size
+    rows = lib.rt_band_rows(H, b[0], b[1], b[2]) if bands else H
+    x0, y0, w, h = window or (0, 0, W, rows)
+    bx, by = (w + 7) // 8, (h + 7) // 8
+    dead = np.zeros(max(1, bx * by), np.uint8)
+    masks = np.zeros(max(1, bx * by), np.uint64)
+    cap_ids = 8 * max(1, n) + 64
+    first = np.zeros(65, np.int32)
+    ids = np.zeros(cap_ids, np.int32)
+    box = np.zeros((64, 2, 3), np.float32)
+    info = (C.c_int32 * 6)()
+    nu = lib.rt_debug_block_units(arr, n, C.byref(cam), W, H, x0, y0, w, h, b[0], b[1], b[2],
+                                  first.ctypes.data_as(C.POINTER(C.c_int32)), ids.ctypes.data_as(C.POINTER(C.c_int32)),
+                                  cap_ids, box.ctypes.data_as(C.POINTER(C.c_float)),
+                                  dead.ctypes.data_as(C.POINTER(C.c_uint8)),
+                                  masks.ctypes.data_as(C.POINTER(C.c_uint64)), bx * by, info)
+    if nu < 0:
+        _check(nu)
+    live = int(info[2])
+    per_unit = [ids[first[u]:first[u + 1]].tolist() for u in range(nu)] if nu <= 64 and info[4] <= cap_ids else []
+    return {"n_units": int(nu), "ids": per_unit, "box": box[:nu] if nu <= 64 else box[:0],
+            "pad": float(np.array([info[5]], np.int32).view(np.float32)[0]),
+            "dead": dead[:bx * by].reshape(by, bx).astype(bool), "live": live, "masks": masks[:live].copy(),
+            "on": bool(info[3])}
+
+
 def start_rows(kernel: int, camera: rt_camera, w: int, h: int, spp: int, chunks: int = 0, grid_blocks: int = 1792,
                instrumented: bool = False, vertex_normals: bool = False) -> dict:
     lib = load_library()
diff --git a/raytracercore_amd/csrc/api_debug.hip b/raytracercore_amd/csrc/api_debug.hip
--- a/raytracercore_amd/csrc/api_debug.hip
+++ b/raytracercore_amd/csrc/api_debug.hip
@@ -509,6 +509,65 @@
     return live;
 }
 
+int rt_debug_block_units(const rt_prim* prims, int32_t n_prims, const rt_camera* camera, int32_t width, int32_t height,
+                         int32_t x0, int32_t y0, int32_t w, int32_t h, int32_t band, int32_t band_stride,
+                         int32_t band_offset, int32_t* unit_first, int32_t* unit_ids, int64_t cap_ids, float* unit_box,
+                         uint8_t* dead, uint64_t* masks, int64_t cap_blocks, int32_t* info)
+{
+    const bool banded = band > 0;
+    if (n_prims < 0 || (n_prims > 0 && !prims) || !camera || width <= 0 || height <= 0 || w <= 0 || h <= 0 || x0 < 0 ||
+        y0 < 0 || x0 + w > width || cap_ids < 0 || (cap_ids > 0 && !unit_ids) || cap_blocks < 0 ||
+        (cap_blocks > 0 && (!dead || !masks)) || band < 0 ||
+        (camera->kind != RT_CAMERA_FRUSTUM && camera->kind != RT_CAMERA_ORTHO) ||
+        (banded && (band_stride <= 0 || band_offset < 0 || band_offset >= band_stride)) || (!banded && y0 + h > height)) {
+        set_error("rt_debug_block_units: bad argument");
+        return RT_ERR_ARG;
+    }
+    for (int i = 0; i < n_prims; i++)
+        if (prims[i].kind < 0 || prims[i].kind > 2) {
+            set_error("rt_debug_block_units: unknown primitive kind at index " + std::to_string(i));
+            return RT_ERR_ARG;
+        }
+    const std::vector<HostPrim> H = prepare_prims(prims, n_prims);
+    const HostRecords rec = report_records(H);
+    const SceneBound b = make_scene_bound(H);
+    const FlatUnits U = make_flat_units(H, rec.orders.flat, b, rec.n_planes, rec.n_vn);
+    CameraD camd;
+    CameraF camf;
+    camera_init(*camera, width, height, camd, camf);
+    const CullWindow win{x0, y0, w, h, banded ? band : 0, banded ? band_stride : 0, banded ? band_offset : 0};
+    std::vector<unsigned char> flags;
+    const int live = cull_blocks(camf, b, rec.n_planes, win, flags);
+    std::vector<uint64_t> m((size_t)live, ~0ull);
+    const bool on = U.on && live > 0 && live < (int)flags.size() &&
+                    unit_masks(camf, b, U.n, U.lo.data(), U.hi.data(), win, flags, m);
+    int64_t n_ids = 0;
+    for (int u = 0; u < U.n; u++) {
+        if (unit_first && u < kMaxUnits) unit_first[u] = (int32_t)n_ids;
+        for (int id : U.ids[(size_t)u]) {
+            if (n_ids < cap_ids) unit_ids[n_ids] = id;
+            n_ids++;
+        }
+        if (unit_box && u < kMaxUnits)
+            for (int k = 0; k < 3; k++) {
+                unit_box[6 * u + k] = U.lo[(size_t)u * 3 + k];
+                unit_box[6 * u + 3 + k] = U.hi[(size_t)u * 3 + k];
+            }
+    }
+    if (unit_first && U.n <= kMaxUnits) unit_first[U.n] = (int32_t)n_ids;
+    for (size_t i = 0; i < flags.size() && (int64_t)i < cap_blocks; i++) dead[i] = flags[i];
+    for (size_t i = 0; i < m.size() && (int64_t)i < cap_blocks; i++) masks[i] = m[i];
+    if (info) {
+        info[0] = (w + 7) / 8;
+        info[1] = (h + 7) / 8;
+        info[2] = live;
+        info[3] = on ? 1 : 0;
+        info[4] = (int32_t)std::min<int64_t>(n_ids, INT32_MAX);
+        std::memcpy(&info[5], &b.pad, 4);
+    }
+    return U.n;
+}
+
 int rt_debug_start_rows(int32_t kernel, const rt_camera* camera, int32_t w, int32_t h, int32_t spp, int32_t chunks,
                         int32_t grid_blocks, int32_t flags, int64_t* info)
 {
diff --git a/raytracercore_amd/csrc/block_cull.cpp b/raytracercore_amd/csrc/block_cull.cpp
--- a/raytracercore_amd/csrc/block_cull.cpp
+++ b/raytracercore_amd/csrc/block_cull.cpp
@@ -122,6 +122,68 @@
     return true;
 }
 
+int block_runs(const CullWindow& win, int by, int run_a[8], int run_b[8])
+{
+    int runs = 0;
+    for (int py = by * 8; py < std::min(win.h, by * 8 + 8); py++) {
+        int fy = win.y0 + py;
+        if (win.band > 0) fy = win.y0 + ((py / win.band) * win.band_stride + win.band_offset) * win.band + py % win.band;
+        if (runs > 0 && fy == run_b[runs - 1] + 1) run_b[runs - 1] = fy;
+        else {
+            run_a[runs] = run_b[runs] = fy;
+            runs++;
+        }
+    }
+    return runs;
+}
+
+bool block_misses(const Hull& hull, const CullWindow& win, int bx, int runs, const int run_a[8], const int run_b[8])
+{
+    const double xa = (double)(win.x0 + bx * 8) - kMargin;
+    const double xb = (double)(win.x0 + std::min(win.w, bx * 8 + 8)) + kMargin;
+    bool miss = true;
+    for (int r = 0; r < runs && miss; r++)
+        miss = separated(hull, xa, xb, (double)run_a[r] - kMargin, (double)(run_b[r] + 1) + kMargin);
+    return miss;
+}
+
+}
+
+bool unit_masks(const CameraF& cam, const SceneBound& bound, int n_units, const float* unit_lo, const float* unit_hi,
+                const CullWindow& win, const std::vector<unsigned char>& dead, std::vector<uint64_t>& masks)
+{
+    const int bxn = (win.w + 7) / 8, byn = (win.h + 7) / 8;
+    size_t n_live = 0;
+    for (unsigned char d : dead) n_live += d ? 0 : 1;
+    masks.assign(n_live, ~0ull);
+    Hull scene_hull;
+    if (n_units < 0 || n_units > 64 || bound.empty || !(bound.limit >= 0.0f) || dead.size() != (size_t)bxn * byn ||
+        !project_bound(cam, bound, (int)(2.0f * cam.w2), scene_hull))
+        return false;
+    std::vector<Hull> hulls((size_t)n_units);
+    uint64_t proven = 0;
+    for (int u = 0; u < n_units; u++) {
+        SceneBound ub = bound;
+        for (int k = 0; k < 3; k++) {
+            ub.lo[k] = unit_lo[3 * u + k];
+            ub.hi[k] = unit_hi[3 * u + k];
+        }
+        if (project_bound(cam, ub, (int)(2.0f * cam.w2), hulls[(size_t)u])) proven |= 1ull << u;
+    }
+    const uint64_t all = n_units == 64 ? ~0ull : (1ull << n_units) - 1ull;
+    size_t live = 0;
+    for (int by = 0; by < byn; by++) {
+        int run_a[8], run_b[8];
+        const int runs = block_runs(win, by, run_a, run_b);
+        for (int bx = 0; bx < bxn; bx++) {
+            if (dead[(size_t)by * bxn + bx]) continue;
+            uint64_t m = all;
+            for (int u = 0; u < n_units; u++)
+                if (((proven >> u) & 1ull) && block_misses(hulls[(size_t)u], win, bx, runs, run_a, run_b)) m &= ~(1ull << u);
+            masks[live++] = m;
+        }
+    }
+    return true;
 }
 
 int cull_blocks(const CameraF& cam, const SceneBound& bound, int n_planes, const CullWindow& win,
@@ -140,22 +202,10 @@
     if (!project_bound(cam, bound, (int)(2.0f * cam.w2), hull)) return n;
     int live = 0;
     for (int by = 0; by < byn; by++) {
-        int run_a[8], run_b[8], runs = 0;
-        for (int py = by * 8; py < std::min(win.h, by * 8 + 8); py++) {
-            int fy = win.y0 + py;
-            if (win.band > 0) fy = win.y0 + ((py / win.band) * win.band_stride + win.band_offset) * win.band + py % win.band;
-            if (runs > 0 && fy == run_b[runs - 1] + 1) run_b[runs - 1] = fy;
-            else {
-                run_a[runs] = run_b[runs] = fy;
-                runs++;
-            }
-        }
+        int run_a[8], run_b[8];
+        const int runs = block_runs(win, by, run_a, run_b);
         for (int bx = 0; bx < bxn; bx++) {
-            const double xa = (double)(win.x0 + bx * 8) - kMargin;
-            const double xb = (double)(win.x0 + std::min(win.w, bx * 8 + 8)) + kMargin;
-            bool is_dead = true;
-            for (int r = 0; r < runs && is_dead; r++)
-                is_dead = separated(hull, xa, xb, (double)run_a[r] - kMargin, (double)(run_b[r] + 1) + kMargin);
+            const bool is_dead = block_misses(hull, win, bx, runs, run_a, run_b);
             dead[(size_t)by * bxn + bx] = is_dead ? 1 : 0;
             live += is_dead ? 0 : 1;
         }
diff --git a/raytracercore_amd/csrc/block_cull.h b/raytracercore_amd/csrc/block_cull.h
--- a/raytracercore_amd/csrc/block_cull.h
+++ b/raytracercore_amd/csrc/block_cull.h
@@ -14,6 +14,9 @@
 int cull_blocks(const CameraF& cam, const SceneBound& bound, int n_planes, const CullWindow& win,
                 std::vector<unsigned char>& dead);
 
+bool unit_masks(const CameraF& cam, const SceneBound& bound, int n_units, const float* unit_lo, const float* unit_hi,
+                const CullWindow& win, const std::vector<unsigned char>& dead, std::vector<uint64_t>& masks);
+
 uint64_t dead_pixels(const CullWindow& win, const std::vector<unsigned char>& dead);
 
 }
diff --git a/raytracercore_amd/csrc/kernels_path.hip b/raytracercore_amd/csrc/kernels_path.hip
--- a/raytracercore_amd/csrc/kernels_path.hip
+++ b/raytracercore_amd/csrc/kernels_path.hip
@@ -367,6 +367,85 @@
         }
         if (ANY && CULL && !__any(b.sg < 0)) return;
     }
+}
+
+#ifdef RT_SCENE_CONST
+#define RT_UNROLL_UNITS _Pragma("unroll")
+#else
+#define RT_UNROLL_UNITS
+#endif
+template <class GroupP, class TestP, class RectP, class FrameP, class BoxP, class XfP>
+__device__ __forceinline__ void trace_units(GroupP groups, TestP tests, RectP rects, FrameP frames, BoxP boxes, XfP xf,
+                                            V3 o, V3 d, int prev, Best& b, unsigned long long mask)
+{
+    const V3 id = v3(slab_rcp_lean(d.x), slab_rcp_lean(d.y), slab_rcp_lean(d.z));
+    const V3 oi = o * id;
+    const GroupRec G = groups[0];
+    auto on = [&]() {
+        const bool t = (mask & 1ull) != 0ull;
+        mask >>= 1;
+        return t;
+    };
+    RectP r = rects + __float_as_int(G.lo.w);
+    RT_UNROLL_UNITS
+    for (int k = 0; k < G.n_rect[0]; k++)
+        if (on()) {
+            const RectRec r0 = r[k];
+            hit_rect<0>(r0, r0.sg, o, d, id, oi, prev, b);
+        }
+    r += G.n_rect[0];
+    RT_UNROLL_UNITS
+    for (int k = 0; k < G.n_rect[1]; k++)
+        if (on()) {
+            const RectRec r0 = r[k];
+            hit_rect<1>(r0, r0.sg, o, d, id, oi, prev, b);
+        }
+    r += G.n_rect[1];
+    RT_UNROLL_UNITS
+    for (int k = 0; k < G.n_rect[2]; k++)
+        if (on()) {
+            const RectRec r0 = r[k];
+            hit_rect<2>(r0, r0.sg, o, d, id, oi, prev, b);
+        }
+    RT_UNROLL_UNITS
+    for (int j = G.frame_first + G.n_frames; j < G.frame_first + G.n_frames + G.n_boxes; j++)
+        if (on()) {
+            const BoxRec B = boxes[j];
+            hit_box<false>(B, o, d, id, oi, prev, b);
+        }
+    RT_UNROLL_UNITS
+    for (int f = G.frame_first; f < G.frame_first + G.n_frames; f++)
+        if (on()) {
+            const FrameRec F = frames[f];
+            const V3 lo = v3(dot4(F.r0, o), dot4(F.r1, o), dot4(F.r2, o));
+            const V3 ld = v3(dot3(F.r0, d), dot3(F.r1, d), dot3(F.r2, d));
+            const V3 lid = v3(rcp(ld.x), rcp(ld.y), rcp(ld.z));
+            RectP fr = rects + F.rect_first;
+            rect_group<0, true>(fr, F.n_rect[0], lo, ld, lid, lo, prev, b);
+            fr += F.n_rect[0];
+            rect_group<1, true>(fr, F.n_rect[1], lo, ld, lid, lo, prev, b);
+            fr += F.n_rect[1];
+            rect_group<2, true>(fr, F.n_rect[2], lo, ld, lid, lo, prev, b);
+            if (F.box >= 0) {
+                const BoxRec B = boxes[F.box];
+                hit_box<true>(B, lo, ld, lid, lo, prev, b);
+            }
+        }
+    int i = __float_as_int(G.hi.w);
+    const int tri_end = i + (G.n_tri_sph & 0xFFFF);
+    RT_UNROLL_UNITS
+    for (; i < tri_end; i++)
+        if (on()) {
+            const TestRec cur = tests[i];
+            hit_tri<true>(cur, i, o, d, prev, b);
+        }
+    const int sph_end = i + (G.n_tri_sph >> 16);
+    RT_UNROLL_UNITS
+    for (; i < sph_end; i++)
+        if (on()) {
+            const TestRec cur = tests[i];
+            hit_sph<true, RT_SPH_WAVE_SKIP < 0 ? false : RT_SPH_WAVE_SKIP != 0>(cur, i, o, d, prev, xf, b);
+        }
 }
 
 template <bool SLOT = false, class XfP>
@@ -1434,6 +1513,7 @@
     const ShadeRecs R = stage_scene<LDS>(P0.scene, P0.prims, P0.mats, P0.xf, lds_scene);
     const int lane = threadIdx.x & 63;
     const unsigned total = (unsigned)P0.n_chunks * (unsigned)P0.n_pad;
+    constexpr bool FIRST = !STATS && !VN && !CULL && SRC == ITEMS_TILE;
     Lane L;
     lane_init(L);
     Sample S;
@@ -1441,7 +1521,7 @@
     S.bounce = 0;
     Counters cnt{};
     unsigned long long wave_rays = 0;
-    const unsigned long long bound_off = P0.scene_bound != 0 ? 0ull : ~0ull;
+    const unsigned long long bound_off = (P0.scene_bound & 1) != 0 ? 0ull : ~0ull;
 
     while (true) {
         unsigned long long t0 = 0, t1 = 0, t2 = 0;
@@ -1484,9 +1564,30 @@
             const auto vnormals = (const RT_AS_CONST float4*)pq->vnormals;
             Best b = query_start<VN>(sc, S.prev);
             bool query = true;
-            if (!STATS && (!CULL || RT_BOUND_GROUPED) &&
-                __builtin_expect((__ballot(L.live && S.bounce != 0) | bound_off) == 0ull, 0))
-                query = __any(L.live && scene_meets(sc, S.o, S.d));
+            if constexpr (FIRST) {
+                const bool camera_rays = __ballot(L.live && S.bounce != 0) == 0ull;
+                if (__builtin_expect(camera_rays, 0)) {
+                    const int fb = pq->scene_bound;
+                    if (fb & 1) query = __any(L.live && scene_meets(sc, S.o, S.d));
+                    if (query && (fb & kFirstMasks)) {
+                        const unsigned sh = 6u + (unsigned)pq->log2_chunks;
+                        const unsigned blk = (unsigned)__builtin_amdgcn_readfirstlane((int)L.item) >> sh;
+                        unsigned long long mask = ~0ull;
+                        if (__ballot(L.live && (L.item >> sh) != blk) == 0ull) {
+                            const unsigned n_live = (unsigned)pq->n_pad >> 6;
+                            const auto cw = (const RT_AS_CONST unsigned int*)pq->cull;
+                            const unsigned at = cull_masks_at(n_live, cw[3]) + 2u * blk;
+                            mask = (unsigned long long)cw[at] | (unsigned long long)cw[at + 1] << 32;
+                        }
+                        trace_units(groups, tests, rects, frames, boxes, xf, S.o, S.d, S.prev, b, mask);
+                        query = false;
+                    }
+                }
+            } else {
+                if (!STATS && (!CULL || RT_BOUND_GROUPED) &&
+                    __builtin_expect((__ballot(L.live && S.bounce != 0) | bound_off) == 0ull, 0))
+                    query = __any(L.live && scene_meets(sc, S.o, S.d));
+            }
             if (query)
                 trace_brute<CULL, STATS>(sc, groups, tests, rects, frames, boxes, xf, S.o, S.d, S.prev, b, cnt.tris,
                                          cnt.sphs, cnt.nodes);
diff --git a/raytracercore_amd/csrc/launch_params.cpp b/raytracercore_amd/csrc/launch_params.cpp
--- a/raytracercore_amd/csrc/launch_params.cpp
+++ b/raytracercore_amd/csrc/launch_params.cpp
@@ -93,6 +93,9 @@
     if (const char* e = getenv("RTCORE_ITEM_BATCH")) p.batch = std::max(0, std::min(64, atoi(e)));
     p.scene_bound = 1;
     if (const char* e = getenv("RTCORE_SCENE_BOUND")) p.scene_bound = atoi(e) != 0 ? 1 : 0;
+    bool first_bounce = true;
+    if (const char* e = getenv("RTCORE_FIRST_BOUNCE")) first_bounce = atoi(e) != 0;
+    if (first_bounce) p.scene_bound |= kFirstBounce;
     p.sample_rounds = 1;
     if (const char* e = getenv("RTCORE_SAMPLE_ROUNDS")) p.sample_rounds = std::max(0, std::min(2, atoi(e)));
     p.refill = 28;
diff --git a/raytracercore_amd/csrc/rt_kernels.h b/raytracercore_amd/csrc/rt_kernels.h
--- a/raytracercore_amd/csrc/rt_kernels.h
+++ b/raytracercore_amd/csrc/rt_kernels.h
@@ -89,6 +89,18 @@
                   __builtin_offsetof(PathParams, cull) == __builtin_offsetof(PathParams, scene_bound) + 8,
               "sample_rounds takes the padding after scene_bound");
 constexpr int kCullTable = 4;
+
+constexpr int kFirstBounce = 2, kFirstMasks = 4;
+constexpr int kMaxUnits = 64;
+template <class GroupT>
+__host__ __device__ inline int flat_unit_count(const GroupT& G)
+{
+    return G.n_rect[0] + G.n_rect[1] + G.n_rect[2] + G.n_boxes + G.n_frames + (G.n_tri_sph & 0xFFFF) + (G.n_tri_sph >> 16);
+}
+__host__ __device__ inline unsigned cull_masks_at(unsigned n_live, unsigned n_blocks)
+{
+    return ((unsigned)kCullTable + n_live + n_blocks + 1u) & ~1u;
+}
 constexpr int kRecRows = 6;
 
 template <class ParT>
diff --git a/raytracercore_amd/csrc/rt_scene.h b/raytracercore_amd/csrc/rt_scene.h
--- a/raytracercore_amd/csrc/rt_scene.h
+++ b/raytracercore_amd/csrc/rt_scene.h
@@ -205,6 +205,7 @@
         unsigned cam_gen = 0;
         CullWindow win{};
         int n_live = 0, n_blocks = 0;
+        bool masks = false;
         uint64_t dead_px = 0, used = 0;
         DevBuf<unsigned int> dev;
         HostBuf<unsigned int> host;
@@ -213,6 +214,7 @@
     static constexpr int kCullEntries = 4;
     std::array<CullEntry, kCullEntries> cull_cache;
     uint64_t cull_clock = 0;
+    FlatUnits units;
     unsigned cam_gen = 0;
     bool has_camera = false;
     bool flat_overflow = false;
diff --git a/raytracercore_amd/csrc/scene_records.cpp b/raytracercore_amd/csrc/scene_records.cpp
--- a/raytracercore_amd/csrc/scene_records.cpp
+++ b/raytracercore_amd/csrc/scene_records.cpp
@@ -1,4 +1,6 @@
 #include "scene_records.h"
+
+#include "rt_kernels.h"
 
 #include <algorithm>
 #include <array>
@@ -851,37 +853,65 @@
     return facts;
 }
 
+static bool prim_extent(const HostPrim& p, double lo[3], double hi[3])
+{
+    for (int k = 0; k < 3; k++) {
+        lo[k] = INFINITY;
+        hi[k] = -INFINITY;
+    }
+    if (p.kind == RT_PRIM_TRIANGLE) {
+        const Vec4d v3 = add(add(p.v[0], p.e01), p.e02);
+        const int nv = (p.flags & F_MIRROR) ? 4 : 3;
+        bool bad = false;
+        for (int j = 0; j < nv; j++) {
+            const Vec4d& v = j < 3 ? p.v[j] : v3;
+            const double c[3] = {v.x, v.y, v.z};
+            for (int k = 0; k < 3; k++) {
+                bad |= !std::isfinite(c[k]);
+                lo[k] = std::min(lo[k], c[k]);
+                hi[k] = std::max(hi[k], c[k]);
+            }
+        }
+        if (bad) lo[0] = hi[0] = NAN;
+        return true;
+    }
+    if (p.kind == RT_PRIM_SPHERE) {
+        const double c[3] = {p.center.x, p.center.y, p.center.z};
+        for (int k = 0; k < 3; k++) {
+            double mid = c[k], half = std::fabs(p.radius);
+            if (p.flags & F_TRANSFORMED) {
+                const double* m = p.to_obj + 4 * k;
+                mid = m[0] * c[0] + m[1] * c[1] + m[2] * c[2] + m[3];
+                half = std::fabs(p.radius) * std::sqrt(m[0] * m[0] + m[1] * m[1] + m[2] * m[2]);
+            }
+            lo[k] = mid - half;
+            hi[k] = mid + half;
+        }
+        return true;
+    }
+    return false;
+}
+static void pad_outward(double a, double c, double pad, float& lo, float& hi)
+{
+    a -= pad;
+    c += pad;
+    lo = (float)a;
+    if ((double)lo > a) lo = std::nextafterf(lo, -INFINITY);
+    hi = (float)c;
+    if ((double)hi < c) hi = std::nextafterf(hi, INFINITY);
+}
+
 SceneBound make_scene_bound(const std::vector<HostPrim>& H)
 {
     double lo[3] = {INFINITY, INFINITY, INFINITY}, hi[3] = {-INFINITY, -INFINITY, -INFINITY};
     bool any = false, bad = false;
-    auto grow = [&](int k, double a, double b) {
-        if (!(std::isfinite(a) && std::isfinite(b))) bad = true;
-        lo[k] = std::min(lo[k], a);
-        hi[k] = std::max(hi[k], b);
-    };
     for (const HostPrim& p : H) {
-        if (p.kind == RT_PRIM_TRIANGLE) {
-            const Vec4d v3 = add(add(p.v[0], p.e01), p.e02);
-            const int nv = (p.flags & F_MIRROR) ? 4 : 3;
-            for (int j = 0; j < nv; j++) {
-                const Vec4d& v = j < 3 ? p.v[j] : v3;
-                const double c[3] = {v.x, v.y, v.z};
-                for (int k = 0; k < 3; k++) grow(k, c[k], c[k]);
-            }
-        } else if (p.kind == RT_PRIM_SPHERE) {
-            const double c[3] = {p.center.x, p.center.y, p.center.z};
-            for (int k = 0; k < 3; k++) {
-                double mid = c[k], half = std::fabs(p.radius);
-                if (p.flags & F_TRANSFORMED) {
-                    const double* m = p.to_obj + 4 * k;
-                    mid = m[0] * c[0] + m[1] * c[1] + m[2] * c[2] + m[3];
-                    half = std::fabs(p.radius) * std::sqrt(m[0] * m[0] + m[1] * m[1] + m[2] * m[2]);
-                }
-                grow(k, mid - half, mid + half);
-            }
-        } else {
-            continue;
+        double a[3], c[3];
+        if (!prim_extent(p, a, c)) continue;
+        for (int k = 0; k < 3; k++) {
+            if (!(std::isfinite(a[k]) && std::isfinite(c[k]))) bad = true;
+            lo[k] = std::min(lo[k], a[k]);
+            hi[k] = std::max(hi[k], c[k]);
         }
         any = true;
     }
@@ -898,17 +928,72 @@
         b.limit = -1.0f;
         return b;
     }
-    for (int k = 0; k < 3; k++) {
-        const double a = lo[k] - pad, c = hi[k] + pad;
-        b.lo[k] = (float)a;
-        if ((double)b.lo[k] > a) b.lo[k] = std::nextafterf(b.lo[k], -INFINITY);
-        b.hi[k] = (float)c;
-        if ((double)b.hi[k] < c) b.hi[k] = std::nextafterf(b.hi[k], INFINITY);
-    }
+    for (int k = 0; k < 3; k++) pad_outward(lo[k], hi[k], pad, b.lo[k], b.hi[k]);
     b.limit = (float)limit;
     if ((double)b.limit > limit) b.limit = std::nextafterf(b.limit, 0.0f);
     b.pad = (float)pad;
     return b;
+}
+
+FlatUnits make_flat_units(const std::vector<HostPrim>& H, const BruteOrder& flat, const SceneBound& bound, int n_planes,
+                          int n_vn)
+{
+    FlatUnits U;
+    if (flat.groups.empty() || flat.overflow) return U;
+    const GroupRec& G = flat.groups[0];
+    auto slot_id = [&](int slot) {
+        int id;
+        std::memcpy(&id, &flat.prims[(size_t)slot].a.w, 4);
+        return id;
+    };
+    auto box_ids = [&](const FrameRec& R, std::vector<int>& out) {
+        BoxRec B;
+        std::memcpy(&B, &R, sizeof B);
+        for (int f = 0; f < 6; f++) out.push_back(slot_id((B.sg0 >> 1) + f));
+    };
+    int rect_first, tri_slot;
+    std::memcpy(&rect_first, &G.lo.w, 4);
+    std::memcpy(&tri_slot, &G.hi.w, 4);
+    const int n_rects = G.n_rect[0] + G.n_rect[1] + G.n_rect[2];
+    for (int k = 0; k < n_rects; k++) U.ids.push_back({slot_id(flat.rects[(size_t)(rect_first + k)].sg >> 1)});
+    for (int j = 0; j < G.n_boxes; j++) {
+        U.ids.emplace_back();
+        box_ids(flat.frames[(size_t)(G.frame_first + G.n_frames + j)], U.ids.back());
+    }
+    for (int f = 0; f < G.n_frames; f++) {
+        const FrameRec& F = flat.frames[(size_t)(G.frame_first + f)];
+        U.ids.emplace_back();
+        for (int k = 0; k < F.n_rect[0] + F.n_rect[1] + F.n_rect[2]; k++)
+            U.ids.back().push_back(slot_id(flat.rects[(size_t)(F.rect_first + k)].sg >> 1));
+        if (F.box >= 0) box_ids(flat.frames[(size_t)F.box], U.ids.back());
+    }
+    const int n_ts = (G.n_tri_sph & 0xFFFF) + (G.n_tri_sph >> 16);
+    for (int i = 0; i < n_ts; i++) U.ids.push_back({slot_id(tri_slot + i)});
+    U.n = (int)U.ids.size();
+    bool ok = U.n == flat_unit_count(G) && U.n <= kMaxUnits && n_planes == 0 && n_vn == 0 && !bound.empty &&
+              bound.limit >= 0.0f;
+    U.lo.assign((size_t)U.n * 3, -INFINITY);
+    U.hi.assign((size_t)U.n * 3, INFINITY);
+    for (int u = 0; u < U.n && ok; u++) {
+        double lo[3] = {INFINITY, INFINITY, INFINITY}, hi[3] = {-INFINITY, -INFINITY, -INFINITY};
+        for (int id : U.ids[(size_t)u]) {
+            double a[3], c[3];
+            if (id < 0 || id >= (int)H.size() || !prim_extent(H[(size_t)id], a, c)) {
+                ok = false;
+                break;
+            }
+            for (int k = 0; k < 3; k++) {
+                lo[k] = std::min(lo[k], a[k]);
+                hi[k] = std::max(hi[k], c[k]);
+            }
+        }
+        for (int k = 0; k < 3 && ok; k++) {
+            if (!(std::isfinite(lo[k]) && std::isfinite(hi[k]))) ok = false;
+            else pad_outward(lo[k], hi[k], (double)bound.pad, U.lo[(size_t)u * 3 + k], U.hi[(size_t)u * 3 + k]);
+        }
+    }
+    U.on = ok;
+    return U;
 }
 
 static constexpr int kOuterMax = 64;
diff --git a/raytracercore_amd/csrc/scene_records.h b/raytracercore_amd/csrc/scene_records.h
--- a/raytracercore_amd/csrc/scene_records.h
+++ b/raytracercore_amd/csrc/scene_records.h
@@ -64,6 +64,14 @@
 XformF make_xformf(const HostPrim& p);
 uint32_t scene_facts(const std::vector<HostPrim>& H);
 SceneBound make_scene_bound(const std::vector<HostPrim>& H);
+struct FlatUnits {
+    bool on = false;
+    int n = 0;
+    std::vector<std::vector<int>> ids;
+    std::vector<float> lo, hi;
+};
+FlatUnits make_flat_units(const std::vector<HostPrim>& H, const BruteOrder& flat, const SceneBound& bound, int n_planes,
+                          int n_vn);
 void select_outer(const std::vector<HostPrim>& H, std::vector<char>& out);
 
 }
diff --git a/raytracercore_amd/csrc/scene_upload.hip b/raytracercore_amd/csrc/scene_upload.hip
--- a/raytracercore_amd/csrc/scene_upload.hip
+++ b/raytracercore_amd/csrc/scene_upload.hip
@@ -336,6 +336,7 @@
     d.ambient = make_float3((float)a.r, (float)a.g, (float)a.b);
     d.ambient_miss = (a.r == -1 && a.g == -1 && a.b == -1) ? 1 : 0;
     d.bound = make_scene_bound(H);
+    s->units = make_flat_units(H, orders.flat, d.bound, np, rec.n_vn);
     return RT_OK;
 }
 
@@ -579,8 +580,14 @@
         c->dead_px = dead_pixels(win, dead);
         c->cam_gen = s->cam_gen;
         c->win = win;
+        c->masks = false;
         if (c->n_live < n_blocks) {
-            const size_t words = (size_t)kCullTable + (size_t)c->n_live + (size_t)n_blocks;
+            std::vector<uint64_t> masks;
+            c->masks = s->units.on && c->n_live > 0 &&
+                       unit_masks(s->camf, s->dev.bound, s->units.n, s->units.lo.data(), s->units.hi.data(), win, dead, masks);
+            const size_t masks_at = cull_masks_at((unsigned)c->n_live, (unsigned)n_blocks);
+            const size_t words = c->masks ? masks_at + 2 * (size_t)c->n_live
+                                          : (size_t)kCullTable + (size_t)c->n_live + (size_t)n_blocks;
             HIP_TRY(c->host.reserve(words));
             HIP_TRY(c->dev.reserve(words));
             unsigned int* h = c->host.p;
@@ -594,6 +601,13 @@
                 h[kCullTable + c->n_live + b] = dead[(size_t)b] ? 0xFFFFFFFFu : live;
                 live += dead[(size_t)b] ? 0u : 1u;
             }
+            if (c->masks) {
+                if (masks_at > (size_t)kCullTable + (size_t)c->n_live + (size_t)n_blocks) h[masks_at - 1] = 0;
+                for (size_t i = 0; i < (size_t)c->n_live; i++) {
+                    h[masks_at + 2 * i] = (unsigned)(masks[i] & 0xFFFFFFFFull);
+                    h[masks_at + 2 * i + 1] = (unsigned)(masks[i] >> 32);
+                }
+            }
             fresh = true;
         } else {
             c->valid = true;
@@ -614,6 +628,7 @@
     if (cull) {
         set_blocks(p, cull->n_live);
         p.cull = cull->dev.p;
+        if ((p.scene_bound & kFirstBounce) && cull->masks) p.scene_bound |= kFirstMasks;
     }
     const size_t need = (size_t)p.n_chunks * (size_t)p.n_pad;
     uint64_t tickets = 0;
@@ -634,7 +649,8 @@
     if (p.ray_log) s->ray_log = nullptr;
     if (s->any_op && stream != s->last_stream) HIP_TRY(hipStreamWaitEvent(stream, s->done_ev, 0));
     if (cull && cull_fresh) {
-        const size_t words = (size_t)kCullTable + (size_t)cull->n_live + (size_t)cull->n_blocks;
+        const size_t words = cull->masks ? cull_masks_at((unsigned)cull->n_live, (unsigned)cull->n_blocks) + 2 * (size_t)cull->n_live
+                                         : (size_t)kCullTable + (size_t)cull->n_live + (size_t)cull->n_blocks;
         HIP_TRY(hipMemcpyAsync(cull->dev.p, cull->host.p, words * sizeof(unsigned int), hipMemcpyHostToDevice, stream));
         HIP_TRY(hipEventRecord(cull->up, stream));
         cull->valid = true;
```

After: 134,000 Mrays/s (median of 6 runs). 1.02x the previous value.
